# MIT-SPARK/Kimera-Semantics

Hardware: AMD Instinct MI355X
Metric: Mvoxel-updates/s + frames/s, 640×480 @5cm voxels, 1/2/4/8 MI355X (higher is better)
Workload: dtype f32; 1 GPU; bag-replay stand-in: 640x480 depth+label trajectory (room), 'fast' integrator, 5 cm voxels, 5 m rays, trunc 0.2 m, p=0.8; pipeline_frames=12, parallelism=frame-sharded x1, points_per_frame=305657, rays_per_frame=85307, updates_per_frame=502687

## Files before the change

### include/ks_hip.h

```cpp
#ifndef KS_HIP_H_
#define KS_HIP_H_

#include <stddef.h>
#include <stdint.h>

#ifdef __cplusplus
extern "C" {
#endif

#define KS_NUM_LABELS 21

enum {
  KS_OK = 0,
  KS_ERR_INVALID_ARG = -1,
  KS_ERR_LABEL_RANGE = -2,
  KS_ERR_PROBABILITY = -3,
  KS_ERR_HIP = -4,
  KS_ERR_POOL_FULL = -5,
  KS_ERR_INDEX_RANGE = -6,
  KS_ERR_NO_DEVICE = -7,
  KS_ERR_UNSUPPORTED = -8,
  KS_ERR_PEER_FAILED = -9
};

// ... 3 lines not shown
enum { KS_BUNDLE_ORDER_REFERENCE = 0, KS_BUNDLE_ORDER_CANONICAL = 1 };
enum { KS_EARLY_OUT_EXACT = 1 };

typedef struct ks_config {
  float voxel_size;
  int32_t voxels_per_side;
  float truncation_distance;
  float max_weight;
  float min_ray_length_m;
  float max_ray_length_m;
  int32_t voxel_carving_enabled;
  int32_t use_const_weight;
  int32_t allow_clear;
  int32_t use_weight_dropoff;
  int32_t use_sparsity_compensation_factor;
  float sparsity_compensation_factor;
  int32_t enable_anti_grazing;
  float start_voxel_subsampling_factor;
  int32_t max_consecutive_ray_collisions;
  int32_t clear_checks_every_n_frames;
  int32_t integration_order_mode;
  int32_t integrator_threads;
  int32_t method;
  int32_t bundle_order;
  float semantic_measurement_probability;
  int32_t color_mode;
  int32_t n_dynamic_labels;
  uint8_t dynamic_labels[32];
  uint8_t label_rgba[256][4];
  int32_t early_out_phase_growth;
  int32_t device_id;
  uint32_t max_tiles;
  uint32_t max_points;
  int32_t pipeline_frames;
} ks_config;

typedef struct ks_frame_stats {
  uint64_t n_points;
  uint64_t n_valid_points;
  uint64_t n_rays_cast;
  uint64_t n_voxel_updates;
  uint64_t n_blocks_allocated;
} ks_frame_stats;

enum {
  KS_STAGE_POINTS = 0,
  KS_STAGE_SORT_POINTS,
  KS_STAGE_RAYS,
  KS_STAGE_MARCH,
  KS_STAGE_EMIT,
  KS_STAGE_SORT_PAIRS,
  KS_STAGE_APPLY,
  KS_STAGE_APPLY_LONG,
  KS_STAGE_COUNT
};
typedef struct ks_profile {
  double ms[KS_STAGE_COUNT];
  uint64_t launches[KS_STAGE_COUNT];
  uint64_t frames;
  uint64_t updates;
  uint64_t points;
  double apply_kernel_ms;
  uint64_t apply_kernel_launches;
  uint64_t apply_kernel_updates;
  double host_ms;
  double host_wait_ms;
} ks_profile;

typedef struct ks_ctx ks_ctx;

int ks_default_config(ks_config* cfg);
int ks_create(const ks_config* cfg, ks_ctx** out);
void ks_destroy(ks_ctx* ctx);
const char* ks_last_error(ks_ctx* ctx);

int ks_set_color_to_label(ks_ctx* ctx, const uint8_t* rgba_keys, const uint8_t* labels, size_t n);

int ks_integrate_points(ks_ctx* ctx, const float T_G_C[7], const float* xyz, const uint8_t* rgba,
                        const uint8_t* labels, size_t n, int freespace, ks_frame_stats* stats);
int ks_integrate_points_device(ks_ctx* ctx, const float T_G_C[7], const float* d_xyz, const uint8_t* d_rgba,
                               const uint8_t* d_labels, size_t n, int freespace, ks_frame_stats* stats);

int ks_integrate_depth(ks_ctx* ctx, const float T_G_C[7], const void* depth, int depth_fmt, const uint8_t* label_img,
                       const uint8_t* rgba_img, int width, int height, const float K[4], int freespace,
                       ks_frame_stats* stats);
int ks_integrate_depth_device(ks_ctx* ctx, const float T_G_C[7], const void* d_depth, int depth_fmt,
                              const uint8_t* d_label_img, const uint8_t* d_rgba_img, int width, int height,
                              const float K[4], int freespace, ks_frame_stats* stats);

int ks_num_blocks(ks_ctx* ctx, size_t* n);
int ks_get_block_indices(ks_ctx* ctx, int32_t* out_xyz, size_t cap, size_t* n);
int ks_get_updated_block_indices(ks_ctx* ctx, int32_t* out_xyz, size_t cap, size_t* n, int reset);
int ks_download_blocks(ks_ctx* ctx, const int32_t* idx_xyz, size_t n, void* tsdf_out, void* sem_out);
int ks_upload_blocks(ks_ctx* ctx, const int32_t* idx_xyz, size_t n, const void* tsdf_in, const void* sem_in);
#define KS_VOXEL_RECORD_BYTES 120
typedef struct ks_voxel_run {
  int32_t block[3];
  uint32_t first;
  uint32_t count;
} ks_voxel_run;
int ks_count_updated_voxels(ks_ctx* ctx, size_t* n_records, size_t* n_runs );
int ks_download_updated_voxels(ks_ctx* ctx, void* out, size_t cap_records, size_t* n_records, ks_voxel_run* runs,
                               size_t cap_runs, size_t* n_runs);
void* ks_host_alloc(size_t bytes);
void ks_host_free(void* p);

typedef struct ks_mesh_config { float min_weight; int32_t only_stale; } ks_mesh_config;
typedef struct ks_mesh_stats {
  uint64_t blocks_meshed, blocks_total, triangles_total, triangles_changed, degenerate_dropped;
} ks_mesh_stats;
typedef struct ks_mesh_block { int32_t block[3]; uint32_t first_vertex, n_vertices; } ks_mesh_block;
int ks_mesh_default_config(ks_mesh_config* cfg);
int ks_mesh_update(ks_ctx* ctx, const ks_mesh_config* cfg, ks_mesh_stats* stats );
int ks_mesh_size(ks_ctx* ctx, size_t* n_blocks, size_t* n_vertices);
int ks_mesh_download(ks_ctx* ctx, ks_mesh_block* blocks, size_t cap_blocks, float* xyz, float* normals, uint8_t* rgba,
                     uint8_t* labels, size_t cap_vertices);
int ks_mesh_changed_blocks(ks_ctx* ctx, int32_t* out_xyz, size_t cap, size_t* n);

typedef struct ks_esdf_config {
  float min_weight, min_distance_m, max_distance_m;
  int32_t use_region;
  int32_t region_min[3], region_max[3];
  uint64_t max_workspace_bytes;
} ks_esdf_config;
typedef struct ks_esdf_stats { uint64_t voxels_observed, voxels_fixed, voxels_clamped, box_voxels[3], workspace_bytes; } ks_esdf_stats;
#define KS_ESDF_RECORD_BYTES 8
int ks_esdf_default_config(ks_esdf_config* cfg);
int ks_esdf_update(ks_ctx* ctx, const ks_esdf_config* cfg, ks_esdf_stats* stats );
int ks_esdf_download_blocks(ks_ctx* ctx, const int32_t* idx_xyz, size_t n, void* out );
int ks_esdf_query(ks_ctx* ctx, const float* xyz , size_t n, float* distance, uint8_t* flags,
                  uint8_t* label );

#define KS_TILE_BYTES 65536
int ks_get_tile_keys(ks_ctx* ctx, uint64_t* out, size_t cap, size_t* n);
int ks_export_tiles_device(ks_ctx* ctx, const uint32_t* slots, size_t n, void* d_payload);
int ks_merge_tiles_device(ks_ctx* ctx, const uint64_t* keys, size_t n, const void* d_payload);
int ks_clear(ks_ctx* ctx);
int ks_clear_voxels(ks_ctx* ctx);
int ks_reset_tiles(ks_ctx* ctx, const uint32_t* slots, size_t n);
int ks_tile_owner(uint64_t tile_key, int world);
typedef struct ks_reduce_stats {
  uint64_t tiles_sent, tiles_received, tiles_local, bytes_sent;
} ks_reduce_stats;
int ks_reduce(ks_ctx* ctx, void* rccl_comm, int rank, int world, ks_reduce_stats* stats);

typedef struct ks_round_stats {
  uint64_t updates_marched, updates_applied, bytes_sent, origin_voxel_touched, rays_cast;
} ks_round_stats;
int ks_integrate_round_exact(ks_ctx* marcher, ks_ctx* owner, void* rccl_comm, int rank, int world, uint64_t first_frame,
                             const float T_G_C[7], const float* xyz, const uint8_t* rgba, const uint8_t* labels, size_t n,
                             int freespace_points, ks_round_stats* stats);

int ks_debug_radix_sort(ks_ctx* ctx, void* keys, uint32_t* vals, size_t n, int key_bits, unsigned end_bit);

int ks_synchronize(ks_ctx* ctx);
void* ks_stream(ks_ctx* ctx);
int ks_flush(ks_ctx* ctx, ks_frame_stats* stats);
int ks_profile_enable(ks_ctx* ctx, int level);
int ks_early_out_iterations(ks_ctx* ctx, uint64_t* frames, uint64_t* iterations);
int ks_early_out_stats(ks_ctx* ctx, uint64_t out[5]);
int ks_profile_get(ks_ctx* ctx, ks_profile* out, int reset);
int ks_update_stats(ks_ctx* ctx, uint64_t out[4]);
int ks_pipeline_shape(ks_ctx* ctx, int32_t out[4]);
int ks_stream_plan(ks_ctx* ctx, int32_t out[8]);
int ks_seed_launch_shape(int32_t integration_order_mode, int32_t early_out_phase_growth, uint64_t cap_points, uint32_t* out, int32_t max_phases);

#ifdef __cplusplus
}
#endif
#endif
```

### kimera_semantics_amd/binding.py

```python
from __future__ import annotations

import ctypes as C
import os
import subprocess

import numpy as np

_HERE = os.path.dirname(os.path.abspath(__file__))
LIB_PATH = os.environ.get("KS_HIP_LIB") or os.path.join(_HERE, "libks_hip.so")
NUM_LABELS = 21

KS_METHOD_FAST, KS_METHOD_MERGED = 0, 1
KS_COLOR_MODE_COLOR, KS_COLOR_MODE_SEMANTIC, KS_COLOR_MODE_SEMANTIC_PROBABILITY = 0, 1, 2
KS_ORDER_MIXED, KS_ORDER_SORTED, KS_ORDER_MIXED_1024_GROUPS = 0, 1, 2
KS_BUNDLE_ORDER_REFERENCE, KS_BUNDLE_ORDER_CANONICAL = 0, 1
KS_EARLY_OUT_EXACT = 1
KS_ERR_LABEL_RANGE, KS_ERR_PROBABILITY, KS_ERR_POOL_FULL, KS_ERR_NO_DEVICE, KS_ERR_UNSUPPORTED = -2, -3, -5, -7, -8
KS_ERR_INVALID_ARG, KS_ERR_PEER_FAILED = -1, -9

STAGES = ["points", "sort_points", "rays", "march", "emit", "sort_pairs", "apply", "apply_long"]

TSDF_DTYPE = np.dtype([("distance", "<f4"), ("weight", "<f4"), ("color", "u1", (4,))])
SEM_DTYPE = np.dtype([("label", "u1"), ("pad", "u1", (3,)), ("priors", "<f4", (NUM_LABELS,)),
                      ("color", "u1", (4,))])

ABI_SYMBOLS = [
    "ks_default_config", "ks_create", "ks_destroy", "ks_last_error", "ks_set_color_to_label",
    "ks_integrate_points", "ks_integrate_points_device", "ks_integrate_depth", "ks_integrate_depth_device", "ks_num_blocks", "ks_get_block_indices",
    "ks_get_updated_block_indices", "ks_count_updated_voxels", "ks_download_updated_voxels", "ks_download_blocks", "ks_upload_blocks", "ks_host_alloc", "ks_host_free", "ks_get_tile_keys", "ks_export_tiles_device", "ks_merge_tiles_device", "ks_clear", "ks_clear_voxels", "ks_reset_tiles", "ks_tile_owner", "ks_reduce",
    "ks_debug_radix_sort", "ks_synchronize", "ks_flush", "ks_stream",
    "ks_profile_enable", "ks_profile_get", "ks_early_out_iterations", "ks_early_out_stats", "ks_pipeline_shape", "ks_stream_plan", "ks_seed_launch_shape", "ks_update_stats", "ks_integrate_round_exact",
    "ks_mesh_default_config", "ks_mesh_update", "ks_mesh_size", "ks_mesh_download", "ks_mesh_changed_blocks",
    "ks_esdf_default_config", "ks_esdf_update", "ks_esdf_download_blocks", "ks_esdf_query",
]


class KsConfig(C.Structure):
    _fields_ = [
        ("voxel_size", C.c_float), ("voxels_per_side", C.c_int32),
        ("truncation_distance", C.c_float), ("max_weight", C.c_float),
        ("min_ray_length_m", C.c_float), ("max_ray_length_m", C.c_float),
        ("voxel_carving_enabled", C.c_int32), ("use_const_weight", C.c_int32),
        ("allow_clear", C.c_int32), ("use_weight_dropoff", C.c_int32),
        ("use_sparsity_compensation_factor", C.c_int32), ("sparsity_compensation_factor", C.c_float),
        ("enable_anti_grazing", C.c_int32), ("start_voxel_subsampling_factor", C.c_float),
        ("max_consecutive_ray_collisions", C.c_int32), ("clear_checks_every_n_frames", C.c_int32),
        ("integration_order_mode", C.c_int32), ("integrator_threads", C.c_int32),
        ("method", C.c_int32), ("bundle_order", C.c_int32),
        ("semantic_measurement_probability", C.c_float), ("color_mode", C.c_int32),
        ("n_dynamic_labels", C.c_int32), ("dynamic_labels", C.c_uint8 * 32),
        ("label_rgba", (C.c_uint8 * 4) * 256),
        ("early_out_phase_growth", C.c_int32),
        ("device_id", C.c_int32), ("max_tiles", C.c_uint32), ("max_points", C.c_uint32), ("pipeline_frames", C.c_int32),
    ]


class KsRoundStats(C.Structure):
    _fields_ = [("updates_marched", C.c_uint64), ("updates_applied", C.c_uint64), ("bytes_sent", C.c_uint64),
                ("origin_voxel_touched", C.c_uint64), ("rays_cast", C.c_uint64)]


class KsFrameStats(C.Structure):
    _fields_ = [("n_points", C.c_uint64), ("n_valid_points", C.c_uint64), ("n_rays_cast", C.c_uint64),
                ("n_voxel_updates", C.c_uint64), ("n_blocks_allocated", C.c_uint64)]


class KsReduceStats(C.Structure):
    _fields_ = [("tiles_sent", C.c_uint64), ("tiles_received", C.c_uint64), ("tiles_local", C.c_uint64),
                ("bytes_sent", C.c_uint64)]


class KsMeshConfig(C.Structure):
    _fields_ = [("min_weight", C.c_float), ("only_stale", C.c_int32)]


class KsMeshStats(C.Structure):
    _fields_ = [("blocks_meshed", C.c_uint64), ("blocks_total", C.c_uint64), ("triangles_total", C.c_uint64),
                ("triangles_changed", C.c_uint64), ("degenerate_dropped", C.c_uint64)]


MESH_BLOCK_DTYPE = np.dtype([("block", "<i4", (3,)), ("first_vertex", "<u4"), ("n_vertices", "<u4")])


class KsEsdfConfig(C.Structure):
    _fields_ = [("min_weight", C.c_float), ("min_distance_m", C.c_float), ("max_distance_m", C.c_float), ("use_region", C.c_int32),
                ("region_min", C.c_int32 * 3), ("region_max", C.c_int32 * 3), ("max_workspace_bytes", C.c_uint64)]


class KsEsdfStats(C.Structure):
    _fields_ = [("voxels_observed", C.c_uint64), ("voxels_fixed", C.c_uint64), ("voxels_clamped", C.c_uint64),
                ("box_voxels", C.c_uint64 * 3), ("workspace_bytes", C.c_uint64)]


ESDF_DTYPE = np.dtype([("distance", "<f4"), ("flags", "u1"), ("label", "u1"), ("pad", "u1", (2,))])


class KsProfile(C.Structure):
    _fields_ = [("ms", C.c_double * 8), ("launches", C.c_uint64 * 8), ("frames", C.c_uint64),
                ("updates", C.c_uint64), ("points", C.c_uint64), ("apply_kernel_ms", C.c_double),
                ("apply_kernel_launches", C.c_uint64), ("apply_kernel_updates", C.c_uint64),
                ("host_ms", C.c_double), ("host_wait_ms", C.c_double)]


def build(force: bool = False) -> str:
    src_dir = os.path.join(_HERE, "csrc")
    srcs = [os.path.join(src_dir, f) for f in ("ks_hip.hip", "ks_types.h", "ks_k_rays.h", "ks_k_bundle_order.h", "ks_k_march.h", "ks_k_exact.h", "ks_k_apply.h",
                                                "ks_k_apply_xl.h", "ks_k_shard.h", "ks_k_shard_merged.h", "ks_k_io.h", "ks_k_mesh.h", "ks_k_esdf.h", "ks_mc_tri_table.inc", "ks_device_math.h", "ks_radix_sort.h", "ks_owned.h")]
    srcs.append(os.path.join(_HERE, "..", "include", "ks_hip.h"))
    stale = (not os.path.exists(LIB_PATH)) or any(
        os.path.exists(s) and os.path.getmtime(s) > os.path.getmtime(LIB_PATH) for s in srcs)
    if force or stale:
        subprocess.check_call(["make", "-C", src_dir])
    return LIB_PATH


_lib = None


def lib():
    global _lib
    if _lib is None:
        if not os.path.exists(LIB_PATH):
            raise RuntimeError(f"{LIB_PATH} is missing: run `python -c 'import __graft_entry__ as g; g.build()'` "
                               "(the HIP path has no CPU fallback)")
        L = C.CDLL(LIB_PATH)
        vp = C.c_void_p
        L.ks_default_config.argtypes = [C.POINTER(KsConfig)]
        L.ks_create.argtypes = [C.POINTER(KsConfig), C.POINTER(vp)]
        L.ks_destroy.argtypes = [vp]
        L.ks_destroy.restype = None
        L.ks_last_error.argtypes = [vp]
        L.ks_last_error.restype = C.c_char_p
        L.ks_set_color_to_label.argtypes = [vp, vp, vp, C.c_size_t]
        L.ks_integrate_points.argtypes = [vp, vp, vp, vp, vp, C.c_size_t, C.c_int, C.POINTER(KsFrameStats)]
        L.ks_integrate_points_device.argtypes = [vp, vp, vp, vp, vp, C.c_size_t, C.c_int, C.POINTER(KsFrameStats)]
        L.ks_integrate_depth.argtypes = [vp, vp, vp, C.c_int, vp, vp, C.c_int, C.c_int, vp, C.c_int, C.POINTER(KsFrameStats)]
        L.ks_integrate_depth_device.argtypes = [vp, vp, vp, C.c_int, vp, vp, C.c_int, C.c_int, vp, C.c_int, C.POINTER(KsFrameStats)]
        L.ks_num_blocks.argtypes = [vp, C.POINTER(C.c_size_t)]
        L.ks_get_block_indices.argtypes = [vp, vp, C.c_size_t, C.POINTER(C.c_size_t)]
        L.ks_get_updated_block_indices.argtypes = [vp, vp, C.c_size_t, C.POINTER(C.c_size_t), C.c_int]
        L.ks_download_blocks.argtypes = [vp, vp, C.c_size_t, vp, vp]
        L.ks_count_updated_voxels.argtypes = [vp, C.POINTER(C.c_size_t), C.POINTER(C.c_size_t)]
        L.ks_download_updated_voxels.argtypes = [vp, vp, C.c_size_t, C.POINTER(C.c_size_t), vp, C.c_size_t, C.POINTER(C.c_size_t)]
        L.ks_upload_blocks.argtypes = [vp, vp, C.c_size_t, vp, vp]
        L.ks_host_alloc.argtypes = [C.c_size_t]
        L.ks_host_alloc.restype = C.c_void_p
        L.ks_host_free.argtypes = [vp]
        L.ks_host_free.restype = None
        L.ks_get_tile_keys.argtypes = [vp, vp, C.c_size_t, C.POINTER(C.c_size_t)]
        L.ks_export_tiles_device.argtypes = [vp, vp, C.c_size_t, vp]
        L.ks_merge_tiles_device.argtypes = [vp, vp, C.c_size_t, vp]
        L.ks_clear.argtypes = [vp]
        L.ks_clear_voxels.argtypes = [vp]
        L.ks_reset_tiles.argtypes = [vp, vp, C.c_size_t]
        L.ks_tile_owner.argtypes = [C.c_uint64, C.c_int]
        L.ks_reduce.argtypes = [vp, vp, C.c_int, C.c_int, C.POINTER(KsReduceStats)]
        L.ks_debug_radix_sort.argtypes = [vp, vp, vp, C.c_size_t, C.c_int, C.c_uint]
        L.ks_synchronize.argtypes = [vp]
        L.ks_flush.argtypes = [vp, C.POINTER(KsFrameStats)]
        L.ks_stream.argtypes = [vp]
        L.ks_stream.restype = vp
        L.ks_profile_enable.argtypes = [vp, C.c_int]
        L.ks_profile_get.argtypes = [vp, C.POINTER(KsProfile), C.c_int]
        L.ks_early_out_iterations.argtypes = [vp, C.POINTER(C.c_uint64), C.POINTER(C.c_uint64)]
        L.ks_early_out_stats.argtypes = [vp, C.POINTER(C.c_uint64)]
        L.ks_pipeline_shape.argtypes = [vp, C.POINTER(C.c_int32)]
        L.ks_stream_plan.argtypes = [vp, C.POINTER(C.c_int32)]
        L.ks_seed_launch_shape.argtypes = [C.c_int32, C.c_int32, C.c_uint64, C.POINTER(C.c_uint32), C.c_int32]
        L.ks_update_stats.argtypes = [vp, C.POINTER(C.c_uint64)]
        L.ks_integrate_round_exact.argtypes = [vp, vp, vp, C.c_int, C.c_int, C.c_uint64, vp, vp, vp, vp, C.c_size_t, C.c_int, C.POINTER(KsRoundStats)]
        L.ks_mesh_default_config.argtypes = [C.POINTER(KsMeshConfig)]
        L.ks_mesh_update.argtypes = [vp, C.POINTER(KsMeshConfig), C.POINTER(KsMeshStats)]
        L.ks_mesh_size.argtypes = [vp, C.POINTER(C.c_size_t), C.POINTER(C.c_size_t)]
        L.ks_mesh_download.argtypes = [vp, vp, C.c_size_t, vp, vp, vp, vp, C.c_size_t]
        L.ks_mesh_changed_blocks.argtypes = [vp, vp, C.c_size_t, C.POINTER(C.c_size_t)]
        L.ks_esdf_default_config.argtypes = [C.POINTER(KsEsdfConfig)]
        L.ks_esdf_update.argtypes = [vp, C.POINTER(KsEsdfConfig), C.POINTER(KsEsdfStats)]
        L.ks_esdf_download_blocks.argtypes = [vp, vp, C.c_size_t, vp]
        L.ks_esdf_query.argtypes = [vp, vp, C.c_size_t, vp, vp, vp]
        _lib = L
    return _lib


def default_config(**overrides) -> KsConfig:
    cfg = KsConfig()
    lib().ks_default_config(C.byref(cfg))
    apply_overrides(cfg, **overrides)
    return cfg


def apply_overrides(cfg, **overrides):
    for k, v in overrides.items():
        if k == "dynamic_labels":
            cfg.n_dynamic_labels = len(v)
            for i, lab in enumerate(v):
                cfg.dynamic_labels[i] = int(lab)
        elif k == "label_rgba":
            arr = np.ascontiguousarray(np.asarray(v, dtype=np.uint8).reshape(256, 4))
            C.memmove(cfg.label_rgba, arr.ctypes.data, 1024)
        else:
            if not hasattr(cfg, k):
                raise AttributeError(k)
            setattr(cfg, k, v)
    return cfg


class KsError(RuntimeError):
    def __init__(self, code, msg):
        super().__init__(f"ks error {code}: {msg}")
        self.code = code


def _ptr(a):
    return None if a is None else a.ctypes.data


class HipIntegrator:

    def __init__(self, cfg: KsConfig):
        self.cfg = cfg
        self.vps = cfg.voxels_per_side
        self._h = C.c_void_p()
        rc = lib().ks_create(C.byref(cfg), C.byref(self._h))
        if rc != 0:
            raise KsError(rc, lib().ks_last_error(None).decode())

    def _chk(self, rc):
        if rc != 0:
            raise KsError(rc, lib().ks_last_error(self._h).decode())

    def close(self):
        if getattr(self, "_h", None):
            lib().ks_destroy(self._h)
            self._h = C.c_void_p()

    def __del__(self):
        try:
            self.close()
        except Exception:
            pass

    def set_color_to_label(self, rgba_keys, labels):
        k = np.ascontiguousarray(rgba_keys, dtype=np.uint8).reshape(-1, 4)
        l = np.ascontiguousarray(labels, dtype=np.uint8)
        self._chk(lib().ks_set_color_to_label(self._h, _ptr(k), _ptr(l), len(l)))

    def integrate(self, T_G_C, xyz, rgba, labels, freespace=False) -> KsFrameStats:
        T = np.ascontiguousarray(T_G_C, dtype=np.float32)
        xyz = np.ascontiguousarray(xyz, dtype=np.float32)
        labels = None if labels is None else np.ascontiguousarray(labels, dtype=np.uint8)
        rgba = None if rgba is None else np.ascontiguousarray(rgba, dtype=np.uint8)
        st = KsFrameStats()
        self._chk(lib().ks_integrate_points(self._h, _ptr(T), _ptr(xyz), _ptr(rgba), _ptr(labels), xyz.shape[0],
                                            int(freespace), C.byref(st)))
        return st

    def integrate_depth(self, T_G_C, depth, K, label_img=None, rgba_img=None, freespace=False) -> KsFrameStats:
        T = np.ascontiguousarray(T_G_C, dtype=np.float32)
        depth = np.ascontiguousarray(depth)
        fmt = 0 if depth.dtype == np.float32 else 1
        assert depth.dtype in (np.float32, np.uint16)
        Kc = np.ascontiguousarray(K, dtype=np.float32)
        lab = None if label_img is None else np.ascontiguousarray(label_img, dtype=np.uint8)
        col = None if rgba_img is None else np.ascontiguousarray(rgba_img, dtype=np.uint8)
        st = KsFrameStats()
        self._chk(lib().ks_integrate_depth(self._h, _ptr(T), _ptr(depth), fmt, _ptr(lab), _ptr(col), depth.shape[1],
                                           depth.shape[0], _ptr(Kc), int(freespace), C.byref(st)))
        return st

    def integrate_depth_device(self, T_G_C, d_depth: int, fmt: int, d_label_img: int, d_rgba_img: int, width: int,
                               height: int, K, freespace=False) -> KsFrameStats:
        T = np.ascontiguousarray(T_G_C, dtype=np.float32)
        Kc = np.ascontiguousarray(K, dtype=np.float32)
        st = KsFrameStats()
        self._chk(lib().ks_integrate_depth_device(self._h, _ptr(T), d_depth or None, fmt, d_label_img or None,
                                                  d_rgba_img or None, width, height, _ptr(Kc), int(freespace), C.byref(st)))
        return st

    def integrate_device(self, T_G_C, d_xyz: int, d_rgba: int, d_labels: int, n: int, freespace=False) -> KsFrameStats:
        T = np.ascontiguousarray(T_G_C, dtype=np.float32)
        st = KsFrameStats()
        self._chk(lib().ks_integrate_points_device(self._h, _ptr(T), d_xyz or None, d_rgba or None, d_labels or None, n,
                                                   int(freespace), C.byref(st)))
        return st

    def block_indices(self) -> np.ndarray:
        n = C.c_size_t()
        self._chk(lib().ks_get_block_indices(self._h, None, 0, C.byref(n)))
        out = np.zeros((n.value, 3), dtype=np.int32)
        if n.value:
            self._chk(lib().ks_get_block_indices(self._h, _ptr(out), n.value, C.byref(n)))
        return out

    def updated_block_indices(self, reset=True) -> np.ndarray:
        n = C.c_size_t()
        self._chk(lib().ks_get_updated_block_indices(self._h, None, 0, C.byref(n), 0))
        out = np.zeros((n.value, 3), dtype=np.int32)
        self._chk(lib().ks_get_updated_block_indices(self._h, _ptr(out), n.value, C.byref(n), int(reset)))
        return out

    def download(self, indices=None):
        if indices is None:
            indices = self.block_indices()
        indices = np.ascontiguousarray(indices, dtype=np.int32).reshape(-1, 3)
        nv = self.vps ** 3
        t = np.zeros((len(indices), nv), dtype=TSDF_DTYPE)
        s = np.zeros((len(indices), nv), dtype=SEM_DTYPE)
        if len(indices):
            self._chk(lib().ks_download_blocks(self._h, _ptr(indices), len(indices), _ptr(t), _ptr(s)))
        return indices, t, s

    def upload(self, indices, tsdf=None, sem=None):
        indices = np.ascontiguousarray(indices, dtype=np.int32).reshape(-1, 3)
        nv = self.vps ** 3
        tp = sp = None
        if tsdf is not None:
            tsdf = np.ascontiguousarray(tsdf, dtype=TSDF_DTYPE).reshape(len(indices), nv)
            tp = _ptr(tsdf)
        if sem is not None:
            sem = np.ascontiguousarray(sem, dtype=SEM_DTYPE).reshape(len(indices), nv)
            sp = _ptr(sem)
        self._chk(lib().ks_upload_blocks(self._h, _ptr(indices), len(indices), tp, sp))

    def mesh(self, only_stale=False, min_weight=1e-4):
        from .mesh import Mesh
        mc, st = KsMeshConfig(float(min_weight), int(bool(only_stale))), KsMeshStats()
        self._chk(lib().ks_mesh_update(self._h, C.byref(mc), C.byref(st)))
        nb, nv = C.c_size_t(), C.c_size_t()
        self._chk(lib().ks_mesh_size(self._h, C.byref(nb), C.byref(nv)))
        blocks = np.zeros(nb.value, dtype=MESH_BLOCK_DTYPE)
        xyz, normals = np.zeros((nv.value, 3), np.float32), np.zeros((nv.value, 3), np.float32)
        rgba, labels = np.zeros((nv.value, 4), np.uint8), np.zeros(nv.value, np.uint8)
        self._chk(lib().ks_mesh_download(self._h, _ptr(blocks), nb.value, _ptr(xyz), _ptr(normals), _ptr(rgba), _ptr(labels), nv.value))
        return Mesh(blocks, xyz, normals, rgba, labels, {k: int(getattr(st, k)) for k, _ in KsMeshStats._fields_})

    def mesh_changed_blocks(self) -> np.ndarray:
        n = C.c_size_t()
        self._chk(lib().ks_mesh_changed_blocks(self._h, None, 0, C.byref(n)))
        out = np.zeros((n.value, 3), dtype=np.int32)
        if n.value:
            self._chk(lib().ks_mesh_changed_blocks(self._h, _ptr(out), n.value, C.byref(n)))
        return out

    def esdf_update(self, region=None, **cfg) -> dict:
        ec, st = KsEsdfConfig(), KsEsdfStats()
        lib().ks_esdf_default_config(C.byref(ec))
        for k, v in cfg.items():
            if k not in ("min_weight", "min_distance_m", "max_distance_m", "max_workspace_bytes"):
                raise AttributeError(k)
            setattr(ec, k, v)
        if region is not None:
            ec.use_region = 1
            for a in range(3):
                ec.region_min[a], ec.region_max[a] = int(region[0][a]), int(region[1][a])
        rc = lib().ks_esdf_update(self._h, C.byref(ec), C.byref(st))
        stats = {k: ([int(v) for v in getattr(st, k)] if k == "box_voxels" else int(getattr(st, k))) for k, _ in KsEsdfStats._fields_}
        if rc != 0:
            err = KsError(rc, lib().ks_last_error(self._h).decode())
            err.stats = stats
            raise err
        return stats

    def esdf(self, region=None, **cfg):
        stats = self.esdf_update(region=region, **cfg)
        idx = self.block_indices()
        return idx, self.esdf_blocks(idx), stats

    def esdf_blocks(self, indices) -> np.ndarray:
        indices = np.ascontiguousarray(indices, dtype=np.int32).reshape(-1, 3)
        out = np.zeros((len(indices), self.vps ** 3), dtype=ESDF_DTYPE)
        self._chk(lib().ks_esdf_download_blocks(self._h, _ptr(indices), len(indices), _ptr(out)))
        return out

    def esdf_query(self, xyz) -> np.ndarray:
        xyz = np.ascontiguousarray(xyz, dtype=np.float32).reshape(-1, 3)
        n = len(xyz)
        d, f, l = np.zeros(n, np.float32), np.zeros(n, np.uint8), np.zeros(n, np.uint8)
        self._chk(lib().ks_esdf_query(self._h, _ptr(xyz), n, _ptr(d), _ptr(f), _ptr(l)))
        out = np.zeros(n, dtype=ESDF_DTYPE)
        out["distance"], out["flags"], out["label"] = d, f, l
        return out

    TILE_BYTES = 65536

    def tile_keys(self) -> np.ndarray:
        n = C.c_size_t()
        self._chk(lib().ks_get_tile_keys(self._h, None, 0, C.byref(n)))
        out = np.zeros(n.value, dtype=np.uint64)
        if n.value:
            self._chk(lib().ks_get_tile_keys(self._h, _ptr(out), n.value, C.byref(n)))
        return out

    def export_tiles(self, slots: np.ndarray, d_payload: int):
        s = np.ascontiguousarray(slots, dtype=np.uint32)
        self._chk(lib().ks_export_tiles_device(self._h, _ptr(s), len(s), d_payload or None))

    def merge_tiles(self, keys: np.ndarray, d_payload: int):
        k = np.ascontiguousarray(keys, dtype=np.uint64)
        self._chk(lib().ks_merge_tiles_device(self._h, _ptr(k), len(k), d_payload or None))

    def download_updated_voxels(self):
        n, nr = C.c_size_t(), C.c_size_t()
        self._chk(lib().ks_count_updated_voxels(self._h, C.byref(n), C.byref(nr)))
        dt = np.dtype([("block", "<i4", (3,)), ("linear", "<u4"), ("tsdf", TSDF_DTYPE), ("sem", SEM_DTYPE)])
        rdt = np.dtype([("block", "<i4", (3,)), ("first", "<u4"), ("count", "<u4")])
        assert dt.itemsize == 120 and rdt.itemsize == 20
        out = np.zeros(n.value, dtype=dt)
        runs = np.zeros(nr.value, dtype=rdt)
        if n.value:
            m, mr = C.c_size_t(), C.c_size_t()
            self._chk(lib().ks_download_updated_voxels(self._h, _ptr(out), n.value, C.byref(m), _ptr(runs), nr.value, C.byref(mr)))
            assert m.value == n.value and mr.value == nr.value
            assert int(runs["count"].sum()) == n.value
            for r in runs[:: max(1, len(runs) // 16)]:
                if r["count"]:
                    assert (out["block"][r["first"]:r["first"] + r["count"]] == r["block"]).all()
        return out

    def clear(self):
        self._chk(lib().ks_clear(self._h))

    def clear_voxels(self):
        self._chk(lib().ks_clear_voxels(self._h))

    def reset_tiles(self, slots: np.ndarray):
        s = np.ascontiguousarray(slots, dtype=np.uint32)
        self._chk(lib().ks_reset_tiles(self._h, _ptr(s), len(s)))

    def reduce(self, rccl_comm, rank: int, world: int) -> dict:
        st = KsReduceStats()
        self._chk(lib().ks_reduce(self._h, C.c_void_p(rccl_comm) if rccl_comm else None, rank, world, C.byref(st)))
        return {"tiles_sent": st.tiles_sent, "tiles_received": st.tiles_received, "tiles_local": st.tiles_local,
                "bytes_sent": st.bytes_sent}

    def debug_radix_sort(self, keys: np.ndarray, vals=None, end_bit=None):
        keys = np.ascontiguousarray(keys).copy()
        bits = keys.dtype.itemsize * 8
        vals = None if vals is None else np.ascontiguousarray(vals, dtype=np.uint32).copy()
        self._chk(lib().ks_debug_radix_sort(self._h, _ptr(keys), _ptr(vals), keys.shape[0], bits,
                                            bits if end_bit is None else end_bit))
        return keys, vals

    def synchronize(self):
        self._chk(lib().ks_synchronize(self._h))

    @property
    def stream(self) -> int:
        return lib().ks_stream(self._h) or 0

    def profile_enable(self, level=1):
        self._chk(lib().ks_profile_enable(self._h, int(level)))

    def early_out_stats(self):
        out = (C.c_uint64 * 5)()
        self._chk(lib().ks_early_out_stats(self._h, out))
        return dict(frames=int(out[0]), rounds=int(out[1]), fallbacks=int(out[2]), event_driven=bool(out[3]), pipelined=bool(out[4]))

    def integrate_round_exact(self, marcher: "HipIntegrator", rccl_comm, rank: int, world: int, first_frame: int, T_G_C, xyz, rgba, labels,
                              freespace=False) -> dict:
        T = np.ascontiguousarray(T_G_C, dtype=np.float32)
        n = 0 if xyz is None else len(xyz)
        x = None if xyz is None else np.ascontiguousarray(xyz, dtype=np.float32)
        c = None if rgba is None else np.ascontiguousarray(rgba, dtype=np.uint8)
        l = None if labels is None else np.ascontiguousarray(labels, dtype=np.uint8)
        st = KsRoundStats()
        self._chk(lib().ks_integrate_round_exact(marcher._h, self._h, rccl_comm, int(rank), int(world), int(first_frame), _ptr(T),
                                                 _ptr(x) if x is not None else None, _ptr(c) if c is not None else None,
                                                 _ptr(l) if l is not None else None, n, int(bool(freespace)), C.byref(st)))
        return dict(updates_marched=int(st.updates_marched), updates_applied=int(st.updates_applied), bytes_sent=int(st.bytes_sent),
                    origin_voxel_touched=bool(st.origin_voxel_touched), rays_cast=int(st.rays_cast))

    def update_stats(self):
        out = (C.c_uint64 * 4)()
        self._chk(lib().ks_update_stats(self._h, out))
        return dict(walked=int(out[0]), serial=int(out[1]), chunks=int(out[2]), replayed=int(out[3]))

    def pipeline_shape(self):
        out = (C.c_int32 * 4)()
        self._chk(lib().ks_pipeline_shape(self._h, out))
        return dict(lag=int(out[0]), slots=int(out[1]), batch=int(out[2]), march_streams=int(out[3]))

    def stream_plan(self):
        out = (C.c_int32 * 8)()
        self._chk(lib().ks_stream_plan(self._h, out))
        side = {1: "own", 0: "tail", -1: "none"}
        return dict(budget=int(out[0]), streams=int(out[1]), march_streams=int(out[2]), long=side[int(out[3])], xlong=side[int(out[4])],
                    march="own" if out[5] else "A", tail="own" if out[6] else "A", streams_held=int(out[7]))

    def early_out_iterations(self):
        f, it = C.c_uint64(), C.c_uint64()
        self._chk(lib().ks_early_out_iterations(self._h, C.byref(f), C.byref(it)))
        return f.value, it.value

    def flush(self) -> KsFrameStats:
        st = KsFrameStats()
        self._chk(lib().ks_flush(self._h, C.byref(st)))
        return st

    def profile(self, reset=False) -> dict:
        p = KsProfile()
        self._chk(lib().ks_profile_get(self._h, C.byref(p), int(reset)))
        return {"ms": {STAGES[i]: p.ms[i] for i in range(8)}, "launches": {STAGES[i]: p.launches[i] for i in range(8)},
                "frames": p.frames, "updates": p.updates, "points": p.points,
                "apply_kernel_ms": p.apply_kernel_ms, "apply_kernel_launches": p.apply_kernel_launches,
                "apply_kernel_updates": p.apply_kernel_updates, "host_ms": p.host_ms, "host_wait_ms": p.host_wait_ms}
```

### kimera_semantics_amd/csrc/ks_hip.hip

```cpp

#include <atomic>
#include <chrono>
#include <condition_variable>
#include <mutex>
#include <thread>
#include <cstring>
#include <string.h>

#include <dlfcn.h>
#include <hip/hip_runtime.h>
#include <hip/hip_ext.h>
#include <rccl/rccl.h>

#include <algorithm>
#include <iterator>
#include <cmath>
#include <cstdio>
#include <cstring>
#include <set>
#include <string>
#include <tuple>
#include <unordered_map>
#include <vector>

#include "../../include/ks_hip.h"
#include "ks_device_math.h"
#include "ks_owned.h"
#include "ks_radix_sort.h"

using namespace ksd;

#include "ks_types.h"
#include "ks_k_bundle_order.h"
#include "ks_k_rays.h"
#include "ks_k_march.h"
#include "ks_k_exact.h"
#include "ks_k_apply.h"
#include "ks_k_apply_xl.h"
#include "ks_k_shard.h"
#include "ks_k_shard_merged.h"
#include "ks_k_io.h"
#include "ks_k_mesh.h"
#include "ks_k_esdf.h"

using namespace ksk;

namespace {

std::string g_create_error;

const char* dbg_env(const char* name) {
  const char* g = getenv("KS_DEBUG");
  return (g && g[0] == '1') ? getenv(name) : nullptr;
}

}

constexpr int kMaxLag = 16;
constexpr int kSlots = kMaxLag + 8;
constexpr int kMarchStreams = 8;
constexpr int kObsTables = 16;
struct HostSnap {
  Counters c;
  uint32_t n_tiles;
  uint32_t pad[7];
};
struct FrameSlot {
  int index = 0;
  DevBuf<RayDesc> d_rays;
  DevBuf<float> d_deltas;
  DevBuf<uint64_t> d_pairs;
  DevBuf<uint32_t> d_cnt;
  DevBuf<uint32_t> d_lp;
  DevBuf<unsigned long long> d_bt;
  DevBuf<uint8_t> d_live;
  DevBuf<uint32_t> d_seed_gen, d_seed_items, d_seed_n;
  bool wide = false;
  DevBuf<FrameParams> d_F;
  DevBuf<uint64_t> d_gkeys, d_rkeys;
  struct GraphSet {
    hipGraphExec_t g1 = nullptr, g2 = nullptr, g3 = nullptr;
    uint64_t key = 0;
    GraphSet() = default;
    GraphSet(const GraphSet&) = delete;
    GraphSet& operator=(const GraphSet&) = delete;
    ~GraphSet() { reset(); }
    void reset() {
      for (hipGraphExec_t* g : {&g1, &g2, &g3}) {
        if (*g) (void)hipGraphExecDestroy(*g);
        *g = nullptr;
      }
      key = 0;
    }
  } b_graphs[2];
  DevBuf<uint64_t> d_eo_keys[2];
  DevBuf<uint32_t> d_eo_vals[2];
  size_t eo_cap_marks = 0;
  DevBuf<uint4> d_eo_tab;
  DevBuf<unsigned long long> d_eo_xnode;
  DevBuf<uint32_t> d_eo_cnt_b, d_eo_ux, d_eo_dirty, d_eo_list[2], d_eo_chg, d_eo_consulted, d_eo_lp;
  DevBuf<unsigned long long> d_eo_bt;
  DevBuf<EoCtl> d_eo_ctl;
  DevBuf<uint32_t> d_eo_sort_ws;
  DevBuf<uint32_t> d_eo_hseq, d_eo_where;
  DevBuf<uint4> d_eo_rinfo, d_eo_ckpt;
  DevBuf<uint8_t> d_eo_hitb;
  DevBuf<unsigned long long> d_eo_bits_a, d_eo_bits_b;
  DevBuf<unsigned long long> d_eo_btp;
  Event eo_committed;
  Counters* d_counters = nullptr;
  DevBuf<uint32_t> d_ray_list;
  PinnedBuf<HostSnap> h_snap;
  Event a_done;
  Event ready;
  Event tail_done;
  Event fork, join;
  Event join_x;
  Event found;
  bool tail_recorded = false;
  bool join_recorded = false;
  bool b_launched = false;
  size_t steps_max = 0;
  uint64_t frame_no = 0;
  FrameParams F{};
  size_t n = 0;
  int prof_set = -1;
  bool pending = false;
  const Counters& counters() const { return h_snap->c; }
  uint32_t n_tiles() const { return h_snap->n_tiles; }
};

constexpr int kProfSets = 32;
constexpr int kStageEvents = KS_STAGE_COUNT + 3;
struct ProfSet {
  Event ev[kStageEvents];
  Event k0, k1;
  bool used = false, complete = false, stages = false, apply = false, applied = false;
  uint64_t n_pairs = 0, n_points = 0;
};

struct StreamPlanIn {
  bool uses_early_out = false;
  bool exact_early_out = false;
  bool frames_independent = true;
  int pipeline_frames = 0;
  int batch = 1;
  bool xlong = true;
  int budget = 4;
};
struct StreamPlan {
  int budget = 4;
  int n_march = 1;
  bool march_own = false;
  bool tail_own = false;
  bool long_own = true;
  bool xlong_own = true;
  int distinct = 1;
};
inline StreamPlan stream_plan(const StreamPlanIn& in) {
  StreamPlan p;
  p.budget = in.budget;
  if (in.pipeline_frames) {
    p.n_march = (!in.frames_independent || in.batch > 1) ? 1 : std::min(kMarchStreams, std::max(4, in.pipeline_frames));
    if (in.exact_early_out && p.n_march > 4) p.n_march = 4;
    if (in.exact_early_out && in.batch > 1) p.n_march = 2;
    if (!in.uses_early_out) p.n_march = 1;
    p.march_own = in.uses_early_out;
    p.tail_own = true;
  }
  p.long_own = true;
  p.xlong_own = in.xlong;
  auto count = [&p] { return 1 + (p.march_own ? p.n_march : 0) + (p.tail_own ? 1 : 0) + (p.long_own ? 1 : 0) + (p.xlong_own ? 1 : 0); };
  if (p.budget < 8 && count() > p.budget) p.xlong_own = false;
  if (p.budget < 8 && count() > p.budget) p.long_own = false;
  p.distinct = count();
  return p;
}
inline int hw_queue_budget() {
  auto number = [](const char* s, int* out) {
    if (!s) return false;
    char* end = nullptr;
    const long v = strtol(s, &end, 10);
    if (end == s) return false;
    *out = (int)std::min<long>(32, std::max<long>(1, v));
    return true;
  };
  int b = 4;
  number(getenv("GPU_MAX_HW_QUEUES"), &b);
  number(dbg_env("KS_HW_QUEUES"), &b);
  return b;
}

struct ks_ctx {
  Stream streams[kMarchStreams + 4];
  int n_streams = 0;
  ks_config cfg{};
  std::string err;
  hipStream_t stream = nullptr;
  hipStream_t stream_march_[kMarchStreams] = {};
  int n_march = 1;
  int batch = 1;
  std::vector<FrameSlot*> batch_slots;
  hipStream_t prof_march_stream = nullptr;
  hipStream_t stream_tail = nullptr;
  hipStream_t stream_long = nullptr;
  hipStream_t stream_xlong = nullptr;
  StreamPlan plan;
  bool xlong = true;
  float voxel_size_inv = 0.f, log_match = 0.f, log_non_match = 0.f;
  int vps_shift = 1;

  TileTable table{};
  Pool pool{};
  DevBuf<TileEntry> table_ent;
  DevBuf<uint64_t> table_slot_keys;
  DevBuf<uint4> pool_vox;
  DevBuf<uint8_t> pool_updated, pool_dirty;
  DevBuf<uint64_t> d_start_set;
  DevBuf<uint64_t> d_observed_[kObsTables];
  int n_obs = 1;
  uint64_t start_offset = 0, observed_offset = 0;
  int64_t reset_counter = 0;
  uint32_t obs_tag = 0, obs_tag_lo = 1;
  DevBuf<Counters> d_retry_counters;
  std::atomic<size_t> pairs_hint{0};
  bool uses_early_out = false;
  std::vector<SeedPhase> seed_phases;
  DevBuf<SeedPhase> d_seed_phases;
  size_t seed_cap_items = 0;
  std::thread tail_thread;
  std::mutex tail_mu;
  std::mutex capture_mu;
  std::condition_variable tail_cv;
  FrameSlot* tail_job = nullptr;
  bool tail_busy = false, tail_quit = false;
  int tail_rc = KS_OK;
  bool use_tail_thread = false;
  bool use_graphs = true;
  bool test_overlap = true;
  std::atomic<uint64_t> buffers_epoch{1};
  DevBuf<uint8_t> d_color_lut;
  DevBuf<uint32_t> d_label_lut;
  uint32_t tiles_initialised = 0;

  size_t cap_points = 0;
  DevBuf<float> d_xyz;
  DevBuf<uint8_t> d_rgba;
  DevBuf<uint8_t> d_labels;
  DevBuf<uint32_t> d_hash;
  DevBuf<uint32_t> d_skeys32, d_skeys32b;
  DevBuf<float4> d_gpw;
  DevBuf<uint64_t> d_ray_keys;
  DevBuf<uint2> d_glc;
  DevBuf<unsigned long long> d_long_list_[2];
  DevBuf<uint32_t> d_blong;
  std::atomic<uint32_t> bo_hint{~0u};
  bool bo_hint_fixed = false;
  DevBuf<uint64_t> d_key_overflow;
  uint32_t key_overflow_mask = 0;
  uint32_t key_bits = 0;
  DevBuf<uint64_t> d_pkeys, d_pkeys2;
  DevBuf<uint32_t> d_pvals, d_pvals2;
  DevBuf<uint32_t> d_order;
  DevBuf<uint32_t> d_inv_order;
  DevBuf<uint32_t> d_okeys, d_okeys2, d_ovals;
  size_t cap_pairs = 0;
  DevBuf<uint64_t> d_pairs2_[2];
  hipEvent_t pending_join = nullptr;
  ksrs::Workspace sort_ws, sort_ws_tail;
  bool exact_early_out = false;
  DevBuf<uint64_t> d_eo_keys[2];
  DevBuf<uint32_t> d_eo_vals[2];
  size_t cap_marks = 0;
  DevBuf<uint2> d_eo_range;
  DevBuf<uint64_t> d_eo_plain;
  DevBuf<uint32_t> d_eo_lp;
  DevBuf<unsigned long long> d_eo_bt;
  DevBuf<EoState> d_eo_state;
  PinnedBuf<EoState> h_eo_state;
  uint64_t eo_iterations = 0, eo_frames = 0;
  bool eo_device = false;
  int eo_bulk_rounds = 6;
  static constexpr int eo_sweeps = 12;
  int eo_sweep_chunks = 16;
  std::atomic<int> eo_want_bulk{0};
  DevBuf<uint32_t> d_eo_committed;
  uint32_t eo_frame_no = 0;
  hipEvent_t eo_last_commit = nullptr;
  std::atomic<size_t> eo_want_marks{0}, eo_want_x{0};
  size_t eo_cap_marks = 0, eo_cap_x = 0;
  std::atomic<uint64_t> eo_fallbacks{0};
  uint64_t eo_fallbacks_seen = 0;
  std::atomic<int> eo_hopeless{0};
  bool eo_device_off = false;
  bool use_bundle_rank = false;
  BoCtx bo{};
  BoSchedule bo_sched{};
  DevBuf<uint8_t> d_bo_slab;
  int bo_epochs = 0;
  DevBuf<int32_t> d_rx_counts;
  DevBuf<uint64_t> d_tx_keys, d_rx_keys;
  DevBuf<uint32_t> d_tx_slots;
  DevBuf<uint8_t> d_tx_payload, d_rx_payload;
  size_t cap_tx = 0, cap_rx = 0;
  DevBuf<uint32_t> d_xchg_u32;
  DevBuf<uint64_t> d_xchg_u64;
  DevBuf<uint8_t> d_state;
  FrameSlot slot[kSlots];
  int n_slots = 1;
  uint64_t frame_no = 0;
  ks_frame_stats owed{};
  DevBuf<int32_t> d_block_idx;
  DevBuf<uint8_t> d_tsdf_out, d_sem_out;
  DevBuf<uint8_t> d_vox_out;
  size_t cap_out_blocks = 0;

  DevBuf<uint32_t> d_depth_blocks;
  DevBuf<uint8_t> d_img_depth;
  DevBuf<uint8_t> d_img_aux;

  int profiling = 0;
  unsigned long long apply_runs_min_pairs = 1ull << 20;
  bool xl_parallel = true;
  unsigned long long xl_min_pairs = 1ull << 23;
  DevBuf<XlRun> d_xl_runs;
  DevBuf<XlHeader> d_xl_hdr;
  DevBuf<XlChunk> d_xl_chunks;
  DevBuf<uint32_t> d_xl_idx;
  bool shard_export = false;
  int shard_world = 1;
  uint64_t shard_frames_seen = 0;
  DevBuf<uint64_t> d_sh_okey[2];
  DevBuf<uint64_t> d_sh_gkey[2];
  DevBuf<uint32_t> d_sh_seq[2];
  DevBuf<float> d_sh_sdf[2];
  DevBuf<float> d_sh_uw[2];
  DevBuf<uint32_t> d_sh_counts;
  size_t cap_sh = 0;
  uint32_t sh_counts[65] = {0};
  uint64_t sh_exported = 0;
  DevBuf<uint64_t> d_sh_tk;
  DevBuf<uint64_t> d_sh_pairs[2];
  DevBuf<uint32_t> d_sh_vals[2];
  size_t cap_sh_rx = 0;
  DevBuf<uint32_t> d_shm_bno;
  DevBuf<float2> d_shm_btab;
  DevBuf<uint32_t> d_shm_mpos;
  DevBuf<uint32_t> d_shm_cnt;
  size_t cap_shm_n = 0;
  DevBuf<float> d_shm_mixed;
  uint32_t shm_counts[2] = {0, 0};
  DevBuf<float2> d_shm_rx_btab;
  DevBuf<float> d_shm_rx_mixed;
  DevBuf<float4> d_shm_ops;
  DevBuf<uint32_t> d_shm_long;
  size_t cap_shm_ops = 0;
  bool long_lanes = true;
  unsigned long long long_lanes_min_pairs = 1ull << 24;
  DevBuf<unsigned long long> d_long_sorted_[2];
  DevBuf<LongHdr> d_long_hdr_[2];
  DevBuf<unsigned long long> d_xl_fb;
  uint32_t cap_xl_chunks = 1u << 17;
  MeshArena mesh_arena[2] = {};
  DevBuf<float> mesh_xyz[2], mesh_nrm[2];
  DevBuf<uint32_t> mesh_rgba[2];
  DevBuf<uint8_t> mesh_label[2];
  size_t mesh_cap[2] = {0, 0};
  int mesh_cur = 0;
  bool mesh_valid = false;
  float mesh_min_weight = 0.f;
  std::vector<uint64_t> mesh_blocks;
  uint32_t mesh_tiles_seen = 0;
  std::vector<ks_mesh_block> mesh_dir;
  std::vector<int32_t> mesh_changed;
  DevBuf<uint8_t> d_mesh_buf[10];
  DevBuf<EsdfRecord> esdf_store;
  DevBuf<uint64_t> esdf_keys[2];
  DevBuf<uint32_t> esdf_slots;
  DevBuf<unsigned long long> esdf_counters;
  DevBuf<EsdfRecord> esdf_out;
  DevBuf<int32_t> esdf_idx;
  DevBuf<float> esdf_xyz;
  bool esdf_valid = false;
  uint32_t esdf_tiles = 0;
  ks_profile prof{};
  ProfSet pset[kProfSets];
  bool fatal = false;
};

#define HIPCHK(ctx, expr)                                                                         \
  do {                                                                                            \
    hipError_t e_ = (expr);                                                                       \
    if (e_ != hipSuccess) {                                                                       \
      (ctx)->err = std::string(#expr) + ": " + hipGetErrorString(e_);                             \
      return KS_ERR_HIP;                                                                          \
    }                                                                                             \
  } while (0)

int ks_hip_failed(ks_ctx* ctx, const char* what, hipError_t e) {
  ctx->err = std::string(what) + ": " + hipGetErrorString(e);
  return KS_ERR_HIP;
}

namespace {

inline hipStream_t march_stream(ks_ctx* c, uint64_t frame_no) { return c->stream_march_[frame_no % (uint64_t)c->n_march]; }
inline uint64_t* observed_table(ks_ctx* c, uint64_t frame_no) { return c->d_observed_[frame_no % (uint64_t)c->n_obs]; }
int sync_march(ks_ctx* c) {
  for (int i = 0; i < c->n_march; ++i)
    if (c->stream_march_[i] != c->stream) HIPCHK(c, hipStreamSynchronize(c->stream_march_[i]));
  return KS_OK;
}

void probe_rehash_schedule(size_t n_max, BoSchedule* out) {
  static std::mutex mu;
  static std::vector<uint32_t> t, b;
  static size_t probed = 0;
  std::lock_guard<std::mutex> lk(mu);
  if (probed < n_max) {
    t.clear();
    b.clear();
    std::unordered_map<uint32_t, char> m;
    size_t bc = m.bucket_count();
    for (uint32_t i = 0; i < n_max; ++i) {
      m.emplace(i, 0);
      if (m.bucket_count() != bc) {
        bc = m.bucket_count();
        t.push_back(i);
        b.push_back((uint32_t)bc);
      }
    }
    probed = n_max;
  }
  *out = BoSchedule{};
  uint32_t off = 0;
  int e = 0;
  for (; e < (int)t.size() && e < kBoMaxEpochs && t[e] < n_max; ++e) {
    out->t[e] = t[e];
    out->b[e] = b[e];
    out->head_off[e] = off;
    off += b[e];
  }
  out->n_epochs = (uint32_t)e;
  out->t[e] = UINT32_MAX;
}

int ensure_bundle_order(ks_ctx* c, size_t cap) {
  probe_rehash_schedule(cap, &c->bo_sched);
  const BoSchedule& S = c->bo_sched;
  {
    static const uint32_t kLibstdcxxBuckets[] = {13, 29, 59, 127, 257, 541, 1109, 2357, 5087, 10273, 20753, 42043, 85229, 172933};
    for (uint32_t e = 0; e < S.n_epochs && e < sizeof(kLibstdcxxBuckets) / sizeof(uint32_t); ++e)
      if (S.b[e] != kLibstdcxxBuckets[e] || (e > 0 && S.t[e] != kLibstdcxxBuckets[e - 1])) {
        c->err = "bundle_order = KS_BUNDLE_ORDER_REFERENCE needs libstdc++'s unordered_map rehash schedule (13, 29, 59, ...): this build's standard "
                 "library differs; use KS_BUNDLE_ORDER_CANONICAL";
        return KS_ERR_UNSUPPORTED;
      }
  }
  c->bo_epochs = (int)S.n_epochs;
  size_t heads = 0;
  for (uint32_t e = 0; e < S.n_epochs; ++e) heads += S.b[e];
  const size_t nbt = cap / kBoBlock + 2, nfbt = 2 * cap / kBoBlock + 2;
  auto al = [](size_t words) { return (words * 4 + 255) & ~(size_t)255; };
  const size_t per_map = 11 * al(cap) + al(nbt) + al(heads);
  const size_t total = 2 * per_map + al(2) + al((sizeof(BoSchedule) + 3) / 4) + 2 * al(2 * cap) + al(nfbt) + al(cap);
  if (int rc = c->d_bo_slab.alloc(c, total)) return rc;
  uint8_t* p = c->d_bo_slab;
  auto take = [&](size_t words) { uint32_t* r = (uint32_t*)p; p += al(words); return r; };
  for (int m = 0; m < 2; ++m) {
    BoMap& M = c->bo.m[m];
    M.H = take(cap); M.rank = take(cap);
    M.next[0] = take(cap); M.next[1] = take(cap);
    M.idj[0] = take(cap); M.idj[1] = take(cap);
    M.kj[0] = take(cap); M.kj[1] = take(cap);
    M.lp = take(cap); M.gm = take(cap); M.cj = take(cap);
    M.bt = take(nbt);
    M.head = take(heads);
    HIPCHK(c, hipMemsetAsync(M.head, 0xff, heads * 4, c->stream));
  }
  c->bo.B = take(2);
  BoSchedule* d_sched = (BoSchedule*)take((sizeof(BoSchedule) + 3) / 4);
  c->bo.sched = d_sched;
  c->bo.flag = take(2 * cap);
  c->bo.flag_lp = take(2 * cap);
  c->bo.flag_bt = take(nfbt);
  c->bo.t_of_head = take(cap);
  HIPCHK(c, hipMemcpyAsync(d_sched, &c->bo_sched, sizeof(BoSchedule), hipMemcpyHostToDevice, c->stream));
  HIPCHK(c, hipStreamSynchronize(c->stream));
  return KS_OK;
}

inline uint32_t order_chains(int order_mode, size_t n) {
  const size_t q = n / kOrderStep;
  return (order_mode == KS_ORDER_MIXED && q >= 1) ? (uint32_t)q : kOrderStep;
}
inline uint32_t order_chains_cap(int order_mode, size_t cap) { return std::max(order_chains(order_mode, cap), order_mode == KS_ORDER_MIXED ? kOrderStep : 0u); }
inline uint32_t order_generations_cap(int order_mode, size_t cap) {
  if (order_mode == KS_ORDER_MIXED) return cap >= kOrderStep ? 2u * kOrderStep - 1u : 1u;
  return (uint32_t)((cap + kOrderStep - 1) / kOrderStep);
}
std::vector<uint32_t> phase_bounds(uint32_t n_gen, int growth) {
  std::vector<uint32_t> b{0};
  for (;;) {
    const uint64_t inc = std::max<uint64_t>(1, (uint64_t)b.back() * (uint64_t)(growth - 16) / 16);
    if (b.back() + inc >= n_gen) break;
    b.push_back((uint32_t)(b.back() + inc));
  }
  return b;
}
inline uint64_t seed_items_of(int order_mode, size_t n, uint32_t g0, uint32_t g1) {
  if (n == 0) return 0;
  const uint64_t chains = order_chains(order_mode, n), full = n / chains, part = n % chains;
  auto subs = [&](uint64_t gens) -> uint64_t {
    const uint64_t hi = std::min<uint64_t>(g1, gens);
    return hi > g0 ? (hi - g0 + kSubRun - 1) / kSubRun : 0;
  };
  return (chains - part) * subs(full) + part * subs(full + 1);
}
std::vector<SeedPhase> seed_launch_shape(int order_mode, int growth, size_t cap) {
  const uint32_t n_gen = order_generations_cap(order_mode, cap);
  const std::vector<uint32_t> B = phase_bounds(n_gen, growth);
  std::vector<SeedPhase> out;
  uint64_t off = 0;
  for (size_t j = 0; j < B.size(); ++j) {
    const uint32_t g0 = B[j], g1 = (j + 1 < B.size()) ? B[j + 1] : n_gen;
    uint64_t m = 0;
    if (order_mode == KS_ORDER_MIXED) {
      m = seed_items_of(order_mode, std::min<size_t>(cap, kOrderStep - 1), g0, g1);
      for (size_t q = 1; q <= cap / kOrderStep; ++q) m = std::max(m, seed_items_of(order_mode, std::min<size_t>(cap, q * kOrderStep + kOrderStep - 1), g0, g1));
    } else {
      m = seed_items_of(order_mode, cap, g0, g1);
    }
    out.push_back(SeedPhase{g0, g1, (uint32_t)off, (uint32_t)m});
    off += m;
  }
  return out;
}

size_t steps_max_of(const ks_config& cfg, float voxel_size_inv) {
  const double max_len = (double)cfg.max_ray_length_m + 2.0 * (double)cfg.truncation_distance;
  return (size_t)std::ceil(1.7321 * max_len * (double)voxel_size_inv) + 8;
}
int ensure_exact_points(ks_ctx* c, size_t cap);
int ensure_points(ks_ctx* c, size_t n) {
  if (n <= c->cap_points) return KS_OK;
  const size_t cap = std::max<size_t>(c->cap_points ? n + n / 8 : n, 1024);
  c->cap_points = 0;
  int rc;
  if ((rc = c->d_xyz.alloc(c, cap * 3))) return rc;
  if ((rc = c->d_rgba.alloc(c, cap * 4))) return rc;
  if ((rc = c->d_labels.alloc(c, cap))) return rc;
  ++c->buffers_epoch;
  const size_t scan_cap = (c->cfg.method == KS_METHOD_MERGED ? 2 : 1) * cap;
  size_t seed_items = 0;
  if (c->uses_early_out) {
    c->seed_phases = seed_launch_shape(c->cfg.integration_order_mode, c->cfg.early_out_phase_growth, cap);
    uint32_t off = 0;
    for (SeedPhase& P : c->seed_phases) {
      if ((P.g1 - P.g0 + kSubRun - 1) / kSubRun > (1u << kSeedSubBits) || order_chains_cap(c->cfg.integration_order_mode, cap) > (1u << kSeedChainBits)) {
        c->err = "point cloud too large for the early-out's work list";
        return KS_ERR_INVALID_ARG;
      }
      if (c->seed_cap_items) P.item_cap = (uint32_t)std::min<size_t>(P.item_cap, c->seed_cap_items);
      P.item_off = off;
      off += P.item_cap;
    }
    seed_items = off;
    if ((rc = c->d_seed_phases.alloc(c, c->seed_phases.size()))) return rc;
    HIPCHK(c, hipMemcpyAsync(c->d_seed_phases, c->seed_phases.data(), c->seed_phases.size() * sizeof(SeedPhase), hipMemcpyHostToDevice, c->stream));
    HIPCHK(c, hipStreamSynchronize(c->stream));
  }
  for (int i = 0; i < (c->cfg.pipeline_frames ? c->n_slots : 1); ++i) {
    if (c->uses_early_out) {
      if ((rc = c->slot[i].d_seed_gen.alloc(c, cap + order_chains_cap(c->cfg.integration_order_mode, cap)))) return rc;
      if ((rc = c->slot[i].d_seed_items.alloc(c, seed_items))) return rc;
      if ((rc = c->slot[i].d_seed_n.alloc(c, c->seed_phases.size()))) return rc;
    }
    if ((rc = c->slot[i].d_rays.alloc(c, cap))) return rc;
    if ((rc = c->slot[i].d_ray_list.alloc(c, cap))) return rc;
    if ((rc = c->slot[i].d_cnt.alloc(c, scan_cap))) return rc;
    if ((rc = c->slot[i].d_lp.alloc(c, scan_cap))) return rc;
    if ((rc = c->slot[i].d_bt.alloc(c, scan_cap / kScanBlock + 2))) return rc;
    if (c->cfg.method == KS_METHOD_FAST && (rc = c->slot[i].d_live.alloc(c, cap))) return rc;
    if (c->cfg.enable_anti_grazing && c->cfg.method == KS_METHOD_MERGED) {
      if ((rc = c->slot[i].d_gkeys.alloc(c, cap))) return rc;
      if ((rc = c->slot[i].d_rkeys.alloc(c, cap))) return rc;
    }
    if (c->cfg.method == KS_METHOD_MERGED && (rc = c->slot[i].d_deltas.alloc(c, cap * kNumLabels))) return rc;
  }
  if ((rc = c->d_hash.alloc(c, cap))) return rc;
  if ((rc = c->d_skeys32.alloc(c, cap))) return rc;
  if ((rc = c->d_skeys32b.alloc(c, cap))) return rc;
  if ((rc = c->d_pkeys.alloc(c, cap))) return rc;
  if ((rc = c->d_pkeys2.alloc(c, cap))) return rc;
  if ((rc = c->d_pvals.alloc(c, cap))) return rc;
  if ((rc = c->d_pvals2.alloc(c, cap))) return rc;
  if ((rc = c->d_order.alloc(c, cap))) return rc;
  if ((rc = c->d_inv_order.alloc(c, cap))) return rc;
  if ((rc = c->d_okeys.alloc(c, cap))) return rc;
  if ((rc = c->d_okeys2.alloc(c, cap))) return rc;
  if ((rc = c->d_ovals.alloc(c, cap))) return rc;
  if (c->cfg.method == KS_METHOD_MERGED) {
    if ((rc = c->d_gpw.alloc(c, cap))) return rc;
    if ((rc = c->d_glc.alloc(c, cap))) return rc;
    if ((rc = c->d_ray_keys.alloc(c, cap))) return rc;
    if ((rc = c->d_blong.alloc(c, cap / kLongRun + 64))) return rc;
    if (c->key_bits) {
      size_t slots = 1024;
      while (slots < 2 * cap) slots <<= 1;
      if ((rc = c->d_key_overflow.alloc(c, slots))) return rc;
      HIPCHK(c, hipMemsetAsync(c->d_key_overflow, 0, slots * sizeof(uint64_t), c->stream));
      c->key_overflow_mask = (uint32_t)(slots - 1);
    }
  }
  if (c->use_bundle_rank && (rc = ensure_bundle_order(c, cap))) return rc;
  if (c->exact_early_out) {
    if ((rc = c->d_eo_lp.alloc(c, cap))) return rc;
    if ((rc = c->d_eo_bt.alloc(c, cap / kScanBlock + 2))) return rc;
    if ((rc = ensure_exact_points(c, cap))) return rc;
  }
  c->cap_points = cap;
  return KS_OK;
}

int ensure_pairs_in(ks_ctx* c, FrameSlot& S, size_t bound) {
  if (bound <= S.d_pairs.size()) return KS_OK;
  if (int rc = S.d_pairs.alloc(c, std::max<size_t>(bound, 1 << 20))) return rc;
  ++c->buffers_epoch;
  return KS_OK;
}
int ensure_pairs_out(ks_ctx* c, size_t n) {
  if (n <= c->cap_pairs) return KS_OK;
  const size_t cap = std::max<size_t>(n + n / 4, 1 << 20);
  c->cap_pairs = 0;
  int rc;
  HIPCHK(c, hipStreamSynchronize(c->stream_long));
  if (c->stream_xlong) HIPCHK(c, hipStreamSynchronize(c->stream_xlong));
  if (c->stream_tail) HIPCHK(c, hipStreamSynchronize(c->stream_tail));
  for (int b = 0; b < 2; ++b) {
    if ((rc = c->d_pairs2_[b].alloc(c, cap))) return rc;
    if ((rc = c->d_long_list_[b].alloc(c, cap / kLongRunLanes + 64 + cap / kXLongRun + 64))) return rc;
    if (c->long_lanes && (rc = c->d_long_sorted_[b].alloc(c, cap / kLongRunLanes + 64))) return rc;
  }
  if (c->d_xl_hdr && (rc = c->d_xl_fb.alloc(c, cap / kXLongRun + 64))) return rc;
  c->cap_pairs = cap;
  return KS_OK;
}

template <typename K>
int sort_keys(ks_ctx* c, K* a, K* b, size_t n, unsigned end_bit, K** result, unsigned begin_bit = 0, bool tail = false) {
  HIPCHK(c, (ksrs::sort<K, false>(tail ? c->sort_ws_tail : c->sort_ws, a, b, nullptr, nullptr, n, end_bit,
                                  tail ? c->stream_tail : c->stream, result, nullptr, begin_bit)));
  return KS_OK;
}
template <typename K>
int sort_pairs(ks_ctx* c, K* ka, K* kb, uint32_t* va, uint32_t* vb, size_t n, unsigned end_bit, K** kres,
               uint32_t** vres) {
  HIPCHK(c, (ksrs::sort<K, true>(c->sort_ws, ka, kb, va, vb, n, end_bit, c->stream, kres, vres)));
  return KS_OK;
}

inline unsigned bits_for(uint64_t n) {
  unsigned b = 1;
  while (b < 64 && (1ull << b) < n) ++b;
  return b;
}

int launch_batch(ks_ctx* c);
int quiesce(ks_ctx* c);
int reset_set(ks_ctx* c, uint64_t* d_set0, uint64_t* offset, bool observed) {
  const bool full = ++(*offset) >= kFullResetThreshold;
  const bool retag = observed && !full && c->obs_tag + (uint32_t)c->cfg.clear_checks_every_n_frames + 2u >= kObsMaxTag;
  if (full || retag) {
    if (int rc = launch_batch(c)) return rc;
    if (full && c->exact_early_out) {
      if (int rc = quiesce(c)) return rc;
    }
    if (int rc = sync_march(c)) return rc;
    if (full) *offset = 0;
    for (int t = 0; t < (observed ? c->n_obs : 1); ++t) {
      uint64_t* d_set = observed ? c->d_observed_[t] : d_set0;
      if (full) {
        HIPCHK(c, hipMemsetAsync(d_set, 0, (observed ? 2 : 1) * (sizeof(uint64_t) << kSetBits), c->stream));
        const uint64_t poison = observed ? kObsPoison : ~0ull;
        HIPCHK(c, hipMemcpyAsync(d_set, &poison, sizeof(poison), hipMemcpyHostToDevice, c->stream));
      } else {
        hipLaunchKernelGGL(k_obs_retag, dim3((2u << kSetBits) / 256), dim3(256), 0, c->stream, d_set);
      }
    }
    if (observed && full && c->d_eo_plain) {
      HIPCHK(c, hipMemsetAsync(c->d_eo_plain, 0, sizeof(uint64_t) << kSetBits, c->stream));
      const uint64_t poison = ~0ull;
      HIPCHK(c, hipMemcpyAsync(c->d_eo_plain, &poison, sizeof(poison), hipMemcpyHostToDevice, c->stream));
    }
    HIPCHK(c, hipStreamSynchronize(c->stream));
    if (observed) c->obs_tag = 0;
  }
  if (observed) c->obs_tag_lo = c->obs_tag + 1;
  return KS_OK;
}

inline void stage_mark(ks_ctx* c, int set, int ev) {
  if (set >= 0 && c->pset[set].stages)
    (void)hipEventRecord(c->pset[set].ev[ev], ev <= 3 ? c->stream : ev <= 5 ? c->prof_march_stream : c->stream_tail);
}

void resolve_prof(ks_ctx* c, int set) {
  ProfSet& P = c->pset[set];
  if (!P.used || !P.complete) return;
  (void)hipEventSynchronize(P.ev[kStageEvents - 1]);
  if (P.stages) {
    for (int s = 0; s < KS_STAGE_COUNT; ++s) {
      float ms = 0.f;
      const int a = s < 3 ? s : s == 3 ? 4 : s + 2;
      if (hipEventElapsedTime(&ms, P.ev[a], P.ev[a + 1]) == hipSuccess) {
        c->prof.ms[s] += ms;
        c->prof.launches[s] += 1;
      }
    }
  }
  if (P.applied) {
    float kms = 0.f;
    if (hipEventElapsedTime(&kms, P.k0, P.k1) == hipSuccess) {
      c->prof.apply_kernel_ms += kms;
      c->prof.apply_kernel_launches += 1;
      c->prof.apply_kernel_updates += P.n_pairs;
    }
  }
  c->prof.frames += 1;
  c->prof.updates += P.n_pairs;
  c->prof.points += P.n_points;
  P.used = P.complete = P.applied = false;
}

SlotView slot_view(const FrameSlot& S, Counters* counters = nullptr) {
  SlotView v{};
  v.F = S.d_F;
  v.rays = S.d_rays;
  v.cnt = S.d_cnt;
  v.lp = S.d_lp;
  v.bt = S.d_bt;
  v.ray_list = S.d_ray_list;
  v.pairs = S.d_pairs;
  v.pairs_cap = (unsigned long long)S.d_pairs.size();
  v.C = counters ? counters : S.d_counters;
  v.host_snap = (uint32_t*)S.h_snap.get();
  v.eo_stats = S.d_eo_ctl ? &S.d_eo_ctl->n_x : nullptr;
  v.seed_gen = S.d_seed_gen;
  v.seed_items = S.d_seed_items;
  v.seed_n = S.d_seed_n;
  return v;
}

void launch_emit(ks_ctx* c, const BatchView& V, uint32_t nb, bool wide, hipStream_t st) {
  const size_t n = c->cap_points;
  const size_t lds = ((2 * n + kScanBlock - 1) / kScanBlock) * sizeof(unsigned long long);
  if (!(c->cfg.method == KS_METHOD_MERGED && c->cfg.enable_anti_grazing)) {
    if (wide || c->cfg.method == KS_METHOD_MERGED || !c->uses_early_out) {
      hipLaunchKernelGGL(k_emit_lane<8>, dim3((uint32_t)((n + 31) / 32), nb), dim3(256), lds, st, V, c->table, c->pool);
    } else {
      hipLaunchKernelGGL(k_emit_lane<16>, dim3((uint32_t)((n + 63) / 64), nb), dim3(256), lds, st, V, c->table, c->pool);
    }
  } else if (wide) {
    hipLaunchKernelGGL(k_emit<64>, dim3((uint32_t)((n + 3) / 4), nb), dim3(256), lds, st, V, c->table, c->pool);
  } else {
    hipLaunchKernelGGL(k_emit<16>, dim3((uint32_t)((n + 15) / 16), nb), dim3(256), lds, st, V, c->table, c->pool);
  }
}

void enqueue_stage_b(ks_ctx* c, const BatchView& V, uint32_t nb, bool wide, hipStream_t sm, size_t steps_max, int part = 0) {
  const ks_config& cfg = c->cfg;
  const size_t n = c->cap_points;
  if (c->uses_early_out && part != 2) {
    for (size_t j = 0; j < c->seed_phases.size(); ++j) {
      const SeedPhase& P = c->seed_phases[j];
      if (P.item_cap == 0) continue;
      const uint32_t steps_cap = (uint32_t)((steps_max + 3) & ~(size_t)3);
      const size_t lds_wave = (size_t)test_lds_words64(steps_cap) * sizeof(unsigned long long);
      const uint32_t wpb = lds_wave * 4 <= 60 * 1024 ? 4u : lds_wave * 2 <= 60 * 1024 ? 2u : 1u;
      const dim3 grid((P.item_cap + wpb - 1) / wpb, nb), block(64 * wpb);
      if (c->test_overlap) hipLaunchKernelGGL(k_test<true>, grid, block, lds_wave * wpb, sm, V, P.g0, P.g1, (uint32_t)j, P.item_off, P.item_cap, steps_cap);
      else hipLaunchKernelGGL(k_test<false>, grid, block, lds_wave * wpb, sm, V, P.g0, P.g1, (uint32_t)j, P.item_off, P.item_cap, steps_cap);
    }
  }
  if (part == 1) return;
  if (cfg.method == KS_METHOD_MERGED && cfg.enable_anti_grazing)
    hipLaunchKernelGGL(k_count_grazing<16>, dim3((uint32_t)((n + 15) / 16), nb), dim3(256), 0, sm, V);
  hipLaunchKernelGGL(k_scan_local, dim3((uint32_t)(((cfg.method == KS_METHOD_MERGED ? 2 : 1) * n + kScanBlock - 1) / kScanBlock), nb),
                     dim3(1024), 0, sm, V);
  launch_emit(c, V, nb, wide, sm);
  hipLaunchKernelGGL(k_publish, dim3(nb), dim3(64), 0, sm, V, (const uint32_t*)c->table.n_tiles);
}

int ensure_marks(ks_ctx* c, size_t n) {
  if (n <= c->cap_marks) return KS_OK;
  const size_t cap = std::max<size_t>(n + n / 4, 1 << 20);
  c->cap_marks = 0;
  int rc;
  for (int b = 0; b < 2; ++b) {
    if ((rc = c->d_eo_keys[b].alloc(c, cap))) return rc;
    if ((rc = c->d_eo_vals[b].alloc(c, cap))) return rc;
  }
  c->cap_marks = cap;
  return KS_OK;
}
constexpr int kEoMaxIterations = 4096;
int exact_early_out(ks_ctx* c, FrameSlot& S, hipStream_t st, Counters* counters = nullptr) {
  const size_t n = S.n;
  Counters* const d_counters = counters ? counters : S.d_counters;
  const FrameParams* dF = S.d_F;
  EoState* hs = c->h_eo_state;
  HIPCHK(c, hipMemsetAsync(c->d_eo_state, 0, sizeof(EoState), st));
  hipLaunchKernelGGL(k_eo_total, dim3((uint32_t)std::min<size_t>((n + 255) / 256, 1024)), dim3(256), 0, st, dF,
                     (const uint32_t*)S.d_cnt, c->d_eo_state);
  HIPCHK(c, hipMemcpyAsync(hs, c->d_eo_state, sizeof(EoState), hipMemcpyDeviceToHost, st));
  HIPCHK(c, hipStreamSynchronize(st));
  const uint32_t nb4k = (uint32_t)((n + kScanBlock - 1) / kScanBlock);
  const size_t lds = (size_t)nb4k * sizeof(unsigned long long);
  uint64_t* kres = nullptr;
  uint32_t* vres = nullptr;
  unsigned long long n_marks = hs->n_marks_next;
  bool converged = n_marks == 0;
  int it = 0;
  for (; !converged && it < kEoMaxIterations; ++it) {
    int rc;
    if ((rc = ensure_marks(c, n_marks))) return rc;
    HIPCHK(c, hipMemsetAsync(c->d_eo_range, 0, sizeof(uint2) << kSetBits, st));
    hipLaunchKernelGGL(k_eo_scan, dim3(nb4k), dim3(1024), 0, st, dF, (const uint32_t*)S.d_cnt, c->d_eo_lp, c->d_eo_bt, c->d_eo_state);
    if (S.wide)
      hipLaunchKernelGGL(k_eo_emit<8>, dim3((uint32_t)((n + 31) / 32)), dim3(256), lds, st, dF, S.d_ray_list, S.d_rays, S.d_cnt,
                         c->d_eo_lp, c->d_eo_bt, c->d_eo_keys[0], c->d_eo_vals[0], (unsigned long long)c->cap_marks, d_counters,
                         c->d_eo_state);
    else
      hipLaunchKernelGGL(k_eo_emit<64>, dim3((uint32_t)((n + 255) / 256)), dim3(256), lds, st, dF, S.d_ray_list, S.d_rays, S.d_cnt,
                         c->d_eo_lp, c->d_eo_bt, c->d_eo_keys[0], c->d_eo_vals[0], (unsigned long long)c->cap_marks, d_counters,
                         c->d_eo_state);
    HIPCHK(c, (ksrs::sort<uint64_t, true>(counters ? c->sort_ws_tail : c->sort_ws, c->d_eo_keys[0], c->d_eo_keys[1], c->d_eo_vals[0], c->d_eo_vals[1],
                                          (size_t)n_marks, 64, st, &kres, &vres, 44)));
    hipLaunchKernelGGL(k_eo_index, dim3((uint32_t)((n_marks + 255) / 256)), dim3(256), 0, st, n_marks, (const uint64_t*)kres,
                       c->d_eo_range);
    EoBuf E{kres, vres, c->d_eo_range, c->d_eo_plain};
    if (S.wide)
      hipLaunchKernelGGL(k_eo_eval<8>, dim3((uint32_t)((n + 31) / 32)), dim3(256), 0, st, dF, S.d_ray_list, S.d_rays, S.d_cnt, E,
                         d_counters, c->d_eo_state);
    else
      hipLaunchKernelGGL(k_eo_eval<16>, dim3((uint32_t)((n + 63) / 64)), dim3(256), 0, st, dF, S.d_ray_list, S.d_rays, S.d_cnt, E,
                         d_counters, c->d_eo_state);
    HIPCHK(c, hipMemcpyAsync(hs, c->d_eo_state, sizeof(EoState), hipMemcpyDeviceToHost, st));
    HIPCHK(c, hipStreamSynchronize(st));
    if (hs->n_marks != n_marks) {
      c->err = "exact early-out: mark count mismatch";
      return KS_ERR_HIP;
    }
    if (hs->changed == 0) converged = true;
    else n_marks = hs->n_marks_next;
  }
  if (!converged) {
    c->err = "exact early-out: no fixed point within the iteration limit";
    return KS_ERR_UNSUPPORTED;
  }
  c->eo_iterations += (uint64_t)it;
  if (!counters) c->eo_frames += 1;
  if (n_marks)
    hipLaunchKernelGGL(k_eo_commit, dim3((uint32_t)((n_marks + 255) / 256)), dim3(256), 0, st, n_marks, (const uint64_t*)kres,
                       (const uint32_t*)vres, c->d_eo_plain);
  return KS_OK;
}

int ensure_exact_slots(ks_ctx* c, size_t cap_marks, size_t cap_x) {
  if (!c->eo_device) return KS_OK;
  int rc;
  const int n_slots = c->cfg.pipeline_frames ? c->n_slots : 1;
  for (int i = 0; i < n_slots; ++i) {
    FrameSlot& S = c->slot[i];
    if (!S.d_eo_ctl) {
      if ((rc = S.d_eo_ctl.alloc(c, 1))) return rc;
      if ((rc = S.d_eo_tab.alloc(c, (size_t)1 << kSetBits))) return rc;
      HIPCHK(c, hipMemsetAsync(S.d_eo_tab, 0, sizeof(uint4) << kSetBits, c->stream));
      if ((rc = S.eo_committed.create(c, hipEventDisableTiming))) return rc;
    }
    if (S.eo_cap_marks < cap_marks) {
      S.eo_cap_marks = 0;
      for (int b = 0; b < 2; ++b) {
        if ((rc = S.d_eo_keys[b].alloc(c, cap_marks))) return rc;
        if ((rc = S.d_eo_vals[b].alloc(c, cap_marks))) return rc;
      }
      if ((rc = S.d_eo_sort_ws.alloc(c, ksrs::ws_words_dev(cap_marks, 3)))) return rc;
      if ((rc = S.d_eo_hitb.alloc(c, cap_marks))) return rc;
      if ((rc = S.d_eo_hseq.alloc(c, cap_marks))) return rc;
      if ((rc = S.d_eo_where.alloc(c, cap_marks))) return rc;
      if ((rc = S.d_eo_bits_a.alloc(c, cap_marks / 64 + 2))) return rc;
      if ((rc = S.d_eo_bits_b.alloc(c, cap_marks / 64 + 2))) return rc;
      S.eo_cap_marks = cap_marks;
    }
    if ((rc = S.d_eo_xnode.reserve(c, 2 * cap_x, 2 * cap_x))) return rc;
  }
  c->eo_cap_marks = cap_marks;
  c->eo_cap_x = cap_x;
  ++c->buffers_epoch;
  HIPCHK(c, hipStreamSynchronize(c->stream));
  return KS_OK;
}
int ensure_exact_points(ks_ctx* c, size_t cap) {
  if (!c->eo_device) return KS_OK;
  int rc;
  for (int i = 0; i < (c->cfg.pipeline_frames ? c->n_slots : 1); ++i) {
    FrameSlot& S = c->slot[i];
    for (DevBuf<uint32_t>* p : {&S.d_eo_cnt_b, &S.d_eo_ux, &S.d_eo_dirty, &S.d_eo_list[0], &S.d_eo_list[1], &S.d_eo_chg, &S.d_eo_consulted, &S.d_eo_lp})
      if ((rc = p->alloc(c, cap))) return rc;
    if ((rc = S.d_eo_bt.alloc(c, cap / kScanBlock + 2))) return rc;
    if ((rc = S.d_eo_btp.alloc(c, cap / kScanBlock + 2))) return rc;
    if ((rc = S.d_eo_rinfo.alloc(c, cap))) return rc;
    if ((rc = S.d_eo_ckpt.alloc(c, 3 * cap))) return rc;
  }
  return KS_OK;
}
EoView eo_view(ks_ctx* c, const FrameSlot& S) {
  EoView E{};
  E.F = S.d_F;
  E.ray_list = S.d_ray_list;
  E.rays = S.d_rays;
  E.C = S.d_counters;
  E.cnt_a = S.d_cnt;
  E.cnt_b = S.d_eo_cnt_b;
  E.ux = S.d_eo_ux;
  E.dirty = S.d_eo_dirty;
  E.keys = S.d_eo_keys[1];
  E.vals = S.d_eo_vals[1];
  E.bits_a = S.d_eo_bits_a;
  E.bits_b = S.d_eo_bits_b;
  E.lp = S.d_eo_lp;
  E.bt = S.d_eo_bt;
  E.btp = S.d_eo_btp;
  E.keys0 = S.d_eo_keys[0];
  E.vals0 = S.d_eo_vals[0];
  E.cap_marks = (unsigned long long)S.eo_cap_marks;
  E.hitb = S.d_eo_hitb;
  E.hseq_w = S.d_eo_hseq;
  E.wide = S.wide ? 1u : 0u;
  E.live = S.d_live;
  E.hseq = S.d_eo_hseq;
  E.where = S.d_eo_where;
  E.rinfo = S.d_eo_rinfo;
  E.ckpt = S.d_eo_ckpt;
  E.tab = S.d_eo_tab;
  E.xnode = S.d_eo_xnode;
  E.cap_x = (uint32_t)(S.d_eo_xnode.size() / 2);
  E.list[0] = S.d_eo_list[0];
  E.list[1] = S.d_eo_list[1];
  E.chg = S.d_eo_chg;
  E.consulted = S.d_eo_consulted;
  E.plain = c->d_eo_plain;
  E.committed = c->d_eo_committed;
  E.ctl = S.d_eo_ctl;
  return E;
}
void enqueue_sweeps(ks_ctx* c, const EoBatch& Bt, uint32_t nb, int count, hipStream_t st) {
  const size_t n = c->cap_points;
  const size_t waves = (size_t)order_chains_cap(c->cfg.integration_order_mode, n) *
                       ((order_generations_cap(c->cfg.integration_order_mode, n) + kEoSweepSegment - 1) / kEoSweepSegment);
  const uint32_t grid = (uint32_t)std::min<size_t>((waves + 3) / 4, 1 << 16);
  for (int i = 0; i < count; ++i) {
    hipLaunchKernelGGL(k_eo2_sweep, dim3(grid, nb), dim3(256), 0, st, Bt);
    hipLaunchKernelGGL(k_eo2_sweep_next, dim3(nb), dim3(64), 0, st, Bt);
  }
}
int enqueue_exact_rounds(ks_ctx* c, FrameSlot* const* slots, uint32_t nb, hipStream_t st) {
  const size_t n = c->cap_points;
  const uint32_t nb4k = (uint32_t)((n + kScanBlock - 1) / kScanBlock);
  const size_t lds = (size_t)nb4k * sizeof(unsigned long long);
  EoBatch Bt{};
  ksrs::DevBatch<uint64_t> Rs{};
  const FrameSlot& S0 = *slots[0];
  for (uint32_t k = 0; k < nb; ++k) {
    const FrameSlot& S = *slots[k];
    Bt.v[k] = eo_view(c, S);
    Rs.keys_a[k] = S.d_eo_keys[0];
    Rs.keys_b[k] = S.d_eo_keys[1];
    Rs.vals_a[k] = S.d_eo_vals[0];
    Rs.vals_b[k] = S.d_eo_vals[1];
    Rs.n_dev[k] = (const unsigned long long*)&S.d_eo_ctl->st.n_marks;
    Rs.ws[k] = S.d_eo_sort_ws;
  }
  hipLaunchKernelGGL(k_eo2_begin, dim3(nb), dim3(64), 0, st, Bt);
  const uint32_t gm = (uint32_t)std::min<size_t>((S0.eo_cap_marks + 255) / 256, 2048);
  const uint32_t gn = (uint32_t)std::min<size_t>((n + 255) / 256, 2048);
  if (S0.wide) {
    hipLaunchKernelGGL(k_eo2_full, dim3(gn, nb), dim3(256), 0, st, Bt);
    hipLaunchKernelGGL(k_eo2_scan, dim3(nb4k, nb), dim3(1024), 0, st, Bt);
    hipLaunchKernelGGL(k_eo2_emit<8>, dim3((uint32_t)((n + 31) / 32), nb), dim3(256), lds, st, Bt);
    HIPCHK(c, ksrs::sort_dev_batch<uint64_t>(Rs, (int)nb, S0.d_eo_sort_ws.size(), S0.eo_cap_marks, 44, 64, st));
    hipLaunchKernelGGL(k_eo2_bits, dim3(gm, nb), dim3(256), 0, st, Bt, 0u);
    hipLaunchKernelGGL(k_eo2_where, dim3(gm, nb), dim3(256), 0, st, Bt);
    enqueue_sweeps(c, Bt, nb, c->eo_sweeps, st);
    return KS_OK;
  } else {
    hipLaunchKernelGGL(k_eo2_scan, dim3(nb4k, nb), dim3(1024), 0, st, Bt);
    hipLaunchKernelGGL(k_eo2_emit<64>, dim3((uint32_t)((n + 255) / 256), nb), dim3(256), lds, st, Bt);
    HIPCHK(c, ksrs::sort_dev_batch<uint64_t>(Rs, (int)nb, S0.d_eo_sort_ws.size(), S0.eo_cap_marks, 44, 64, st));
    hipLaunchKernelGGL(k_eo2_hits, dim3(gm, nb), dim3(256), 0, st, Bt);
    hipLaunchKernelGGL(k_eo2_stop0, dim3(gn, nb), dim3(256), 0, st, Bt);
    hipLaunchKernelGGL(k_eo2_bits, dim3(gm, nb), dim3(256), 0, st, Bt, 1u);
  }
  const uint32_t gr = (uint32_t)std::min<size_t>((n + 3) / 4, 2048);
  for (int r = 1; r <= c->eo_bulk_rounds; ++r) {
    const uint32_t g = S0.wide ? gr : std::min(gr, r == 1 ? 2048u : r == 2 ? 1024u : r <= 4 ? 512u : 256u);
    hipLaunchKernelGGL(k_eo2_eval, dim3(g, nb), dim3(256), 0, st, Bt, (uint32_t)r);
    hipLaunchKernelGGL(k_eo2_propagate, dim3(g, nb), dim3(256), 0, st, Bt, (uint32_t)r);
  }
  return KS_OK;
}
void enqueue_exact_finish(ks_ctx* c, FrameSlot& S, hipStream_t st) {
  const EoView E = eo_view(c, S);
  hipLaunchKernelGGL(k_eo2_finish, dim3(1), dim3(kEoFinishThreads), 0, st, E, (uint32_t)c->eo_bulk_rounds + 1u, 1u);
  hipLaunchKernelGGL(k_eo2_commit, dim3(1024), dim3(256), 0, st, E);
}

template <typename Enqueue> hipGraphExec_t capture_graph(hipStream_t sm, Enqueue enqueue) {
  hipGraph_t g = nullptr;
  hipGraphExec_t out = nullptr;
  bool ok = hipStreamBeginCapture(sm, hipStreamCaptureModeRelaxed) == hipSuccess;
  if (ok) {
    const int rc = enqueue();
    ok = hipStreamEndCapture(sm, &g) == hipSuccess && g != nullptr && rc == KS_OK;
  }
  if (ok) ok = hipGraphInstantiate(&out, g, nullptr, nullptr, 0) == hipSuccess;
  if (g) (void)hipGraphDestroy(g);
  return ok ? out : nullptr;
}
struct BatchLaunch {
  ks_ctx* c;
  FrameSlot* const* slots;
  uint32_t nb;
  FrameSlot& S0;
  hipStream_t sm;
  const BatchView& V;
  size_t steps_max;
  uint64_t key;
  FrameSlot::GraphSet& G;
  int sweeps_host_driven() const {
    EoBatch Bt{};
    for (uint32_t k = 0; k < nb; ++k) Bt.v[k] = eo_view(c, *slots[k]);
    for (int chunk = 1;; ++chunk) {
      bool going = false;
      for (uint32_t k = 0; k < nb; ++k) {
        uint32_t w[2] = {0u, 0u};
        HIPCHK(c, hipMemcpyAsync(&w[0], &slots[k]->d_eo_ctl->sw_prev, sizeof(uint32_t), hipMemcpyDeviceToHost, sm));
        HIPCHK(c, hipMemcpyAsync(&w[1], &slots[k]->d_eo_ctl->fail, sizeof(uint32_t), hipMemcpyDeviceToHost, sm));
        HIPCHK(c, hipStreamSynchronize(sm));
        going = going || (w[0] != 0u && w[1] == 0u);
      }
      if (!going || chunk >= c->eo_sweep_chunks) break;
      enqueue_sweeps(c, Bt, nb, c->eo_sweeps, sm);
    }
    hipLaunchKernelGGL(k_eo2_sweep_done, dim3(nb), dim3(64), 0, sm, Bt);
    return KS_OK;
  }
  int exact_device() const {
    int rc;
    auto seed_and_rounds = [&] {
      enqueue_stage_b(c, V, nb, S0.wide, sm, steps_max, 1);
      return enqueue_exact_rounds(c, slots, nb, sm);
    };
    auto finish = [&] {
      for (uint32_t k = 0; k < nb; ++k) enqueue_exact_finish(c, *slots[k], sm);
      return KS_OK;
    };
    auto emission = [&] { return enqueue_stage_b(c, V, nb, S0.wide, sm, steps_max, 2), KS_OK; };
    bool graphs = c->use_graphs && !S0.wide;
    if (graphs && (G.key != key || !G.g1 || !G.g2 || !G.g3)) {
      std::lock_guard<std::mutex> cap(c->capture_mu);
      G.reset();
      if ((G.g1 = capture_graph(sm, seed_and_rounds)) && (G.g2 = capture_graph(sm, finish)) && (G.g3 = capture_graph(sm, emission))) {
        G.key = key;
      } else {
        (void)hipGetLastError();
        G.reset();
        c->use_graphs = graphs = false;
      }
    }
    if (graphs) HIPCHK(c, hipGraphLaunch(G.g1, sm));
    else if ((rc = seed_and_rounds()) || (S0.wide && (rc = sweeps_host_driven()))) return rc;
    if (c->eo_last_commit && c->eo_last_commit != S0.eo_committed) HIPCHK(c, hipStreamWaitEvent(sm, c->eo_last_commit, 0));
    if (graphs) HIPCHK(c, hipGraphLaunch(G.g2, sm));
    else finish();
    HIPCHK(c, hipEventRecord(S0.eo_committed, sm));
    c->eo_last_commit = S0.eo_committed;
    if (graphs) HIPCHK(c, hipGraphLaunch(G.g3, sm));
    else emission();
    return KS_OK;
  }
  int exact_host() const {
    enqueue_stage_b(c, V, nb, S0.wide, sm, steps_max, 1);
    if (int rc = exact_early_out(c, S0, sm)) return rc;
    enqueue_stage_b(c, V, nb, S0.wide, sm, steps_max, 2);
    return KS_OK;
  }
  int plain_or_replayed() const {
    if (c->use_graphs && (G.key != key || !G.g1)) {
      std::lock_guard<std::mutex> cap(c->capture_mu);
      G.reset();
      if ((G.g1 = capture_graph(sm, [&] { return enqueue_stage_b(c, V, nb, S0.wide, sm, steps_max), KS_OK; }))) {
        G.key = key;
      } else {
        (void)hipGetLastError();
        c->use_graphs = false;
      }
    }
    if (c->use_graphs && G.g1) HIPCHK(c, hipGraphLaunch(G.g1, sm));
    else enqueue_stage_b(c, V, nb, S0.wide, sm, steps_max);
    return KS_OK;
  }
};

int launch_batch(ks_ctx* c) {
  if (c->batch_slots.empty()) return KS_OK;
  std::vector<FrameSlot*> slots;
  slots.swap(c->batch_slots);
  const uint32_t nb = (uint32_t)slots.size();
  FrameSlot& S0 = *slots[0];
  hipStream_t sm = c->batch > 1 ? c->stream_march_[(S0.frame_no / (uint64_t)c->batch) % (uint64_t)c->n_march] : march_stream(c, S0.frame_no);
  c->prof_march_stream = sm;
  if (sm != c->stream) HIPCHK(c, hipStreamWaitEvent(sm, slots[nb - 1]->a_done, 0));
  const bool stage_events = nb == 1 && S0.prof_set >= 0 && c->pset[S0.prof_set].stages;
  if (stage_events) (void)hipEventRecord(c->pset[S0.prof_set].ev[4], sm);
  BatchView V{};
  size_t steps_max = 0;
  ParamsBatch PB{};
  for (uint32_t k = 0; k < nb; ++k) {
    FrameSlot& S = *slots[k];
    S.F.observed = observed_table(c, S.frame_no);
    if (c->exact_early_out) S.F.eo_frame = c->eo_frame_no++;
    PB.F[k] = S.F;
    PB.out[k] = S.d_F;
    V.s[k] = slot_view(S);
    steps_max = std::max(steps_max, S.steps_max);
  }
  if (nb == 1) hipLaunchKernelGGL(k_set_params, dim3(1), dim3(64), 0, sm, slots[0]->F, slots[0]->d_F);
  else hipLaunchKernelGGL(k_set_params_batch, dim3(nb), dim3(64), 0, sm, PB);
  const uint64_t key = ((uint64_t)c->cap_points << 24) ^ (c->buffers_epoch.load() << 4) ^ (S0.wide ? 1u : 0u) ^ ((uint64_t)nb << 1);
  const BatchLaunch B{c, slots.data(), nb, S0, sm, V, steps_max, key, S0.b_graphs[nb == (uint32_t)c->batch ? 0 : 1]};
  if (int rc = !c->exact_early_out ? B.plain_or_replayed() : c->eo_device && !c->eo_device_off ? B.exact_device() : B.exact_host()) return rc;
  for (uint32_t k = 0; k < nb; ++k) {
    HIPCHK(c, hipEventRecord(slots[k]->ready, sm));
    slots[k]->b_launched = true;
  }
  if (stage_events) (void)hipEventRecord(c->pset[S0.prof_set].ev[5], sm);
  return KS_OK;
}

void fill_frame_params(ks_ctx* c, FrameParams& F, const float Tq[7], size_t n, int freespace) {
  const ks_config& cfg = c->cfg;
  F = FrameParams{};
  F.T.w = Tq[0];
  F.T.v = {Tq[1], Tq[2], Tq[3]};
  F.T.t = {Tq[4], Tq[5], Tq[6]};
  F.voxel_size_inv = c->voxel_size_inv;
  F.min_ray = cfg.min_ray_length_m;
  F.max_ray = cfg.max_ray_length_m;
  F.trunc = cfg.truncation_distance;
  F.start_inv = cfg.start_voxel_subsampling_factor * c->voxel_size_inv;
  F.log_match = c->log_match;
  F.log_non_match = c->log_non_match;
  F.tsdf.voxel_size = cfg.voxel_size;
  F.tsdf.trunc = cfg.truncation_distance;
  F.tsdf.max_weight = cfg.max_weight;
  F.tsdf.dropoff_denominator = cfg.truncation_distance - cfg.voxel_size;
  F.tsdf.sparsity_factor = cfg.sparsity_compensation_factor;
  F.tsdf.use_dropoff = cfg.use_weight_dropoff;
  F.tsdf.use_sparsity = cfg.use_sparsity_compensation_factor;
  F.start_offset = c->start_offset;
  F.observed_offset = c->observed_offset;
  F.obs_tag = c->obs_tag;
  F.obs_tag_lo = c->obs_tag_lo;
  F.max_collisions = cfg.max_consecutive_ray_collisions;
  F.n = (uint32_t)n;
  const uint32_t q = (uint32_t)(n / kOrderStep);
  const bool by_1024 = cfg.integration_order_mode == KS_ORDER_MIXED_1024_GROUPS;
  F.order_groups = q == 0 ? 1u : by_1024 ? kOrderStep : q;
  F.order_per = q == 0 ? 0u : by_1024 ? q : kOrderStep;
  F.chains = order_chains(cfg.integration_order_mode, n);
  F.carving = cfg.voxel_carving_enabled;
  F.allow_clear = cfg.allow_clear;
  F.freespace = freespace;
  F.use_const_weight = cfg.use_const_weight;
  F.method = cfg.method;
  F.color_mode = cfg.color_mode;
  F.sorted_order = cfg.integration_order_mode == KS_ORDER_SORTED;
  F.n_dynamic = cfg.n_dynamic_labels;
  const unsigned pb = bits_for(n);
  F.point_mask = (1u << pb) - 1u;
  F.clear_bit = (cfg.method == KS_METHOD_MERGED) ? (1u << pb) : 0u;
  F.seq_bits = pb + (cfg.method == KS_METHOD_MERGED ? 1u : 0u);
  F.inv_order = F.sorted_order ? c->d_inv_order : nullptr;
  std::memcpy(F.dynamic_labels, cfg.dynamic_labels, 32);
  F.early_out = c->uses_early_out;
}
void begin_prof_set(ks_ctx* c, FrameSlot& S, size_t n) {
  const int set = (int)(c->frame_no % kProfSets);
  resolve_prof(c, set);
  ProfSet& P = c->pset[set];
  P.used = true;
  P.complete = P.applied = false;
  P.stages = c->profiling == 1;
  P.apply = c->profiling == 1 || (c->frame_no % 4) == 0;
  P.n_points = n;
  P.n_pairs = 0;
  S.prof_set = set;
}
int stage_a_fast(ks_ctx* c, FrameSlot& S, const float* d_xyz, const uint8_t* d_rgba, const uint8_t* d_labels, size_t n) {
  const FrameParams& F = S.F;
  hipStream_t st = c->stream;
  const uint32_t nb1k = (uint32_t)((n + 1023) / 1024);
  hipLaunchKernelGGL(k_points_fast, dim3(nb1k), dim3(1024), 0, st, F, d_xyz, d_rgba, d_labels, c->d_color_lut,
                     S.d_rays, c->d_hash, c->d_skeys32, c->d_pvals, S.d_cnt, S.d_live, S.d_counters);
  stage_mark(c, S.prof_set, 1);
  uint32_t *sk = nullptr, *sv = nullptr;
  if (int rc = sort_pairs(c, c->d_skeys32.get(), c->d_skeys32b.get(), c->d_pvals.get(), c->d_pvals2.get(), n, kSetBits + 1, &sk, &sv)) return rc;
  stage_mark(c, S.prof_set, 2);
  hipLaunchKernelGGL(k_dedup, dim3(nb1k), dim3(1024), 0, st, F, sk, sv, c->d_hash, c->d_start_set, S.d_ray_list, S.d_rays, S.d_cnt, S.d_live, S.d_counters);
  if (c->uses_early_out && n > 0) {
    const uint32_t n_gen = (uint32_t)((n + F.chains - 1) / F.chains);
    uint32_t n_ph = 0;
    while (n_ph < c->seed_phases.size() && c->seed_phases[n_ph].g0 < n_gen) ++n_ph;
    HIPCHK(c, hipMemsetAsync(S.d_seed_n, 0, c->seed_phases.size() * sizeof(uint32_t), st));
    hipLaunchKernelGGL(k_seed_list, dim3((F.chains + 63u) / 64u, n_ph), dim3(64 * kSeedSegs), 0, st, F, (const SeedPhase*)c->d_seed_phases,
                       (const uint8_t*)S.d_live, S.d_seed_gen, S.d_seed_items, S.d_seed_n, S.d_counters);
  }
  hipLaunchKernelGGL(k_dedup_commit, dim3(nb1k), dim3(1024), 0, st, F, sk, sv, c->d_hash, c->d_start_set, S.d_counters);
  return KS_OK;
}
void enqueue_bundle_order(ks_ctx* c, hipStream_t st, size_t n, const uint64_t* sk, const uint32_t* sv) {
  const uint32_t capb = (uint32_t)((c->cap_points + kBoBlock - 1) / kBoBlock);
  const size_t lds_f = (2 * c->cap_points / kBoBlock + 3) * sizeof(uint32_t), lds_e = ((size_t)capb + 2) * sizeof(uint32_t);
  hipLaunchKernelGGL(k_bo_scan_flags, dim3((uint32_t)((2 * n + kBoBlock - 1) / kBoBlock)), dim3(kBoBlock), 0, st, (uint32_t)n, c->bo);
  hipLaunchKernelGGL(k_bo_init, dim3((uint32_t)((n + kBoBlock - 1) / kBoBlock)), dim3(kBoBlock), lds_f, st, (uint32_t)n, sk, sv, c->bo);
  const uint32_t nbb = (uint32_t)((n + kBoBlock - 1) / kBoBlock);
  int e_small = 0;
  while (e_small < c->bo_epochs && c->bo_sched.b[e_small] <= kBoSmallBuckets) ++e_small;
  if (e_small > 0) hipLaunchKernelGGL(k_bo_small, dim3(2), dim3(kBoBlock), 0, st, c->bo, e_small);
  const size_t nh_floor = c->bo_hint_fixed ? (e_small > 0 ? (size_t)c->bo_sched.t[e_small - 1] + 1 : 1) : 2 * (size_t)kBoSmallBuckets;
  const size_t nh = std::min<size_t>(n, std::max<size_t>(c->bo_hint.load(std::memory_order_relaxed), nh_floor));
  int e_last = -1;
  for (int e = e_small; e <= c->bo_epochs; ++e) {
    if (e > 0 && c->bo_sched.t[e - 1] >= nh) break;
    hipLaunchKernelGGL(k_bo_link, dim3(nbb, 2), dim3(kBoBlock), lds_e, st, c->bo, e, (e == e_small && e_small > 0) ? 1 : 0);
    if (e < c->bo_epochs && c->bo_sched.t[e] < nh)
      hipLaunchKernelGGL(k_bo_walk, dim3(nbb, 2), dim3(kBoBlock), 0, st, c->bo, e);
    else
      e_last = e;
  }
  if (nh < n && e_last >= 0 && e_last < c->bo_epochs) hipLaunchKernelGGL(k_bo_rest, dim3(2), dim3(kBoBlock), lds_e, st, c->bo, e_last);
}
int stage_a_merged(ks_ctx* c, FrameSlot& S, const float* d_xyz, const uint8_t* d_rgba, const uint8_t* d_labels, size_t n, const uint32_t* order_ptr) {
  const ks_config& cfg = c->cfg;
  FrameParams& F = S.F;
  hipStream_t st = c->stream;
  const uint32_t nb = (uint32_t)((n + 255) / 256);
  const uint32_t nb1k = (uint32_t)((n + 1023) / 1024);
  if (c->key_bits) {
    const float reach = cfg.max_ray_length_m + 2.0f * cfg.voxel_size;
    const float tq[3] = {F.T.t.x, F.T.t.y, F.T.t.z};
    for (int a = 0; a < 3; ++a) {
      const float lo = std::floor((tq[a] - reach) * c->voxel_size_inv) - 2.0f;
      F.key_base[a] = (int32_t)std::min(std::max(lo, -2.0e9f), 2.0e9f);
    }
    F.key_bits = c->key_bits;
  }
  hipLaunchKernelGGL(k_points_merged, dim3(nb1k), dim3(1024), 0, st, F, d_xyz, d_rgba, d_labels, c->d_color_lut, c->d_pkeys, c->d_skeys32, c->d_pvals,
                     S.d_cnt, c->use_bundle_rank ? c->bo.flag : nullptr, c->d_key_overflow, c->key_overflow_mask, S.d_counters);
  stage_mark(c, S.prof_set, 1);
  uint64_t* sk = nullptr;
  uint32_t *sk32 = nullptr, *sv = nullptr;
  if (c->key_bits) {
    if (int rc = sort_pairs(c, c->d_skeys32.get(), c->d_skeys32b.get(), c->d_pvals.get(), c->d_pvals2.get(), n, 32, &sk32, &sv)) return rc;
    sk = c->d_pkeys;
  } else {
    if (int rc = sort_pairs(c, c->d_pkeys.get(), c->d_pkeys2.get(), c->d_pvals.get(), c->d_pvals2.get(), n, 64, &sk, &sv)) return rc;
  }
  stage_mark(c, S.prof_set, 2);
  hipLaunchKernelGGL(k_gather_sorted, dim3(nb), dim3(256), 0, st, F, d_xyz, d_rgba, d_labels, c->d_color_lut,
                     order_ptr, (const uint64_t*)sk, (const uint32_t*)sk32, sk, sv, c->d_gpw, c->d_glc, c->use_bundle_rank ? c->bo.flag : nullptr, c->d_blong,
                     c->d_key_overflow, S.d_counters);
  if (c->use_bundle_rank) enqueue_bundle_order(c, st, n, sk, sv);
  uint64_t* ray_keys = cfg.enable_anti_grazing ? S.d_rkeys : nullptr;
  if (cfg.enable_anti_grazing) HIPCHK(c, hipMemcpyAsync(S.d_gkeys, sk, n * sizeof(uint64_t), hipMemcpyDeviceToDevice, st));
  const uint32_t n_long_blocks = (uint32_t)std::min<size_t>(n / kLongRun + 1, 512);
  hipLaunchKernelGGL(k_bundles_all, dim3(n_long_blocks + (uint32_t)((n + 127) / 128)), dim3(128), 0, st, F, sk, sv, c->d_gpw, c->d_glc, c->d_blong,
                     S.d_rays, S.d_deltas, S.d_ray_list, ray_keys, S.d_cnt, c->bo, c->use_bundle_rank, S.d_counters, n_long_blocks);
  if (cfg.enable_anti_grazing) {
    F.grazing_keys = S.d_gkeys;
    F.ray_keys = S.d_rkeys;
  }
  return KS_OK;
}
int frame_front(ks_ctx* c, FrameSlot& S, const float Tq[7], const float* d_xyz, const uint8_t* d_rgba, const uint8_t* d_labels, size_t n, int freespace) {
  int rc;
  FrameParams& F = S.F;
  fill_frame_params(c, F, Tq, n, freespace);
  const size_t steps_max = steps_max_of(c->cfg, c->voxel_size_inv);
  S.wide = steps_max > 400;
  const size_t hint = c->pairs_hint.load(std::memory_order_relaxed);
  if ((rc = ensure_pairs_in(c, S, std::max<size_t>(hint + hint / 4, 1 << 20)))) return rc;
  hipStream_t st = c->stream;
  if (S.tail_recorded && c->stream_tail != c->stream) HIPCHK(c, hipStreamWaitEvent(st, S.tail_done, 0));
  if (S.join_recorded) HIPCHK(c, hipStreamWaitEvent(st, S.join, 0));
  S.n = n;
  S.prof_set = -1;
  if (c->profiling) begin_prof_set(c, S, n);
  S.frame_no = c->frame_no++;
  const uint32_t nb = (uint32_t)((n + 255) / 256);
  const uint32_t* order_ptr = nullptr;
  stage_mark(c, S.prof_set, 0);
  if (F.sorted_order) {
    hipLaunchKernelGGL(k_sqnorm, dim3(nb), dim3(256), 0, st, (uint32_t)n, d_xyz, c->d_okeys, c->d_ovals);
    uint32_t *ok = nullptr, *ov = nullptr;
    if ((rc = sort_pairs(c, c->d_okeys.get(), c->d_okeys2.get(), c->d_ovals.get(), c->d_order.get(), n, 32, &ok, &ov))) return rc;
    order_ptr = ov;
    hipLaunchKernelGGL(k_invert, dim3(nb), dim3(256), 0, st, (uint32_t)n, order_ptr, c->d_inv_order);
    F.order = order_ptr;
  }
  if ((rc = c->cfg.method == KS_METHOD_FAST ? stage_a_fast(c, S, d_xyz, d_rgba, d_labels, n) : stage_a_merged(c, S, d_xyz, d_rgba, d_labels, n, order_ptr)))
    return rc;
  stage_mark(c, S.prof_set, 3);
  if (c->stream_march_[0] != st) HIPCHK(c, hipEventRecord(S.a_done, st));
  S.steps_max = steps_max;
  S.b_launched = false;
  S.pending = true;
  c->batch_slots.push_back(&S);
  if ((int)c->batch_slots.size() >= c->batch || c->profiling == 1) return launch_batch(c);
  return KS_OK;
}

int shard_export_frame(ks_ctx* c, FrameSlot& S, unsigned long long n_pairs, hipStream_t st) {
  const int world = c->shard_world;
  int rc;
  if (n_pairs > c->cap_sh) {
    const size_t cap = std::max<size_t>(n_pairs + n_pairs / 4, 1 << 20);
    c->cap_sh = 0;
    for (int b = 0; b < 2; ++b) {
      if ((rc = c->d_sh_okey[b].alloc(c, cap))) return rc;
      if ((rc = c->d_sh_gkey[b].alloc(c, cap))) return rc;
      if ((rc = c->d_sh_seq[b].alloc(c, cap))) return rc;
      if ((rc = c->d_sh_sdf[b].alloc(c, cap))) return rc;
      if ((rc = c->d_sh_uw[b].alloc(c, cap))) return rc;
    }
    c->cap_sh = cap;
  }
  if (!c->d_sh_counts && (rc = c->d_sh_counts.alloc(c, 128))) return rc;
  const bool merged = c->cfg.method == KS_METHOD_MERGED;
  c->shm_counts[0] = c->shm_counts[1] = 0;
  if (merged && (S.n > c->cap_shm_n || !c->d_shm_cnt)) {
    const size_t cap = std::max<size_t>(S.n, 1 << 16);
    c->cap_shm_n = 0;
    if ((rc = c->d_shm_bno.alloc(c, cap))) return rc;
    if ((rc = c->d_shm_btab.alloc(c, cap))) return rc;
    if ((rc = c->d_shm_mpos.alloc(c, cap))) return rc;
    if ((rc = c->d_shm_cnt.alloc(c, 2))) return rc;
    c->cap_shm_n = cap;
  }
  HIPCHK(c, hipMemsetAsync(c->d_sh_counts, 0, 128 * sizeof(uint32_t), st));
  std::memset(c->sh_counts, 0, sizeof(c->sh_counts));
  c->sh_exported = n_pairs;
  if (n_pairs) {
    const uint32_t nb = (uint32_t)((n_pairs + 255) / 256);
    hipLaunchKernelGGL(k_shard_export, dim3(nb), dim3(256), 0, st, S.F, n_pairs, (const uint64_t*)S.d_pairs, (const RayDesc*)S.d_rays,
                       (const uint64_t*)c->table.slot_keys, (uint32_t)world, c->d_sh_okey[0], c->d_sh_gkey[0], c->d_sh_seq[0],
                       c->d_sh_sdf[0], c->d_sh_uw[0], c->d_sh_counts);
    uint64_t* sorted = nullptr;
    HIPCHK(c, (ksrs::sort<uint64_t, false>(c->sort_ws_tail, c->d_sh_okey[0], c->d_sh_okey[1], nullptr, nullptr, (size_t)n_pairs, 64, st,
                                           &sorted, nullptr, 56)));
    if (merged) {
      HIPCHK(c, hipMemsetAsync(c->d_shm_bno, 0, (size_t)S.n * sizeof(uint32_t), st));
      HIPCHK(c, hipMemsetAsync(c->d_shm_cnt, 0, 2 * sizeof(uint32_t), st));
      hipLaunchKernelGGL(k_shard_mark_bundles, dim3(nb), dim3(256), 0, st, n_pairs, (const uint32_t*)c->d_sh_seq[0], c->d_shm_bno);
      hipLaunchKernelGGL(k_shard_bundle_table, dim3((uint32_t)((S.n + 255) / 256)), dim3(256), 0, st, (uint32_t)S.n, (const RayDesc*)S.d_rays,
                         c->d_shm_bno, c->d_shm_btab, c->d_shm_mpos, c->d_shm_cnt);
      hipLaunchKernelGGL(k_shard_gather_merged, dim3(nb), dim3(256), 0, st, n_pairs, (const uint64_t*)sorted, (const uint64_t*)c->d_sh_gkey[0],
                         (const uint32_t*)c->d_sh_seq[0], (const float*)c->d_sh_sdf[0], (const float*)c->d_sh_uw[0], (const uint32_t*)c->d_shm_bno,
                         c->d_sh_gkey[1], c->d_sh_seq[1], c->d_sh_sdf[1], c->d_sh_uw[1]);
      HIPCHK(c, hipMemcpyAsync(c->shm_counts, c->d_shm_cnt, 2 * sizeof(uint32_t), hipMemcpyDeviceToHost, st));
    } else {
      hipLaunchKernelGGL(k_shard_gather, dim3(nb), dim3(256), 0, st, n_pairs, (const uint64_t*)sorted, (const uint64_t*)c->d_sh_gkey[0],
                         (const uint32_t*)c->d_sh_seq[0], (const float*)c->d_sh_sdf[0], (const float*)c->d_sh_uw[0], c->d_sh_gkey[1],
                         c->d_sh_seq[1], c->d_sh_sdf[1], c->d_sh_uw[1]);
    }
    HIPCHK(c, hipMemcpyAsync(c->sh_counts, c->d_sh_counts, 65 * sizeof(uint32_t), hipMemcpyDeviceToHost, st));
  }
  HIPCHK(c, hipStreamSynchronize(st));
  if (merged && c->shm_counts[1]) {
    const size_t nm = c->shm_counts[1];
    if ((rc = c->d_shm_mixed.reserve(c, nm * kNumLabels, std::max<size_t>(nm + nm / 2, 1024) * kNumLabels))) return rc;
    hipLaunchKernelGGL(k_shard_mixed_rows, dim3((uint32_t)((nm * kNumLabels + 255) / 256)), dim3(256), 0, st, (uint32_t)nm,
                       (const uint32_t*)c->d_shm_mpos, (const float*)S.d_deltas, c->d_shm_mixed);
    HIPCHK(c, hipStreamSynchronize(st));
  }
  return KS_OK;
}

inline void skip_update_stages(ks_ctx* c, int set) {
  for (int e = 7; e < kStageEvents - 1; ++e) stage_mark(c, set, e);
}
inline void finish_prof(ks_ctx* c, int set, hipStream_t st, uint64_t n_pairs) {
  if (set < 0) return;
  ProfSet& P = c->pset[set];
  P.n_pairs = n_pairs;
  (void)hipEventRecord(P.ev[kStageEvents - 1], st);
  P.complete = true;
}
inline void owe_stats(ks_ctx* c, const FrameSlot& S, const Counters& cnt, unsigned long long n_pairs, uint32_t n_blocks) {
  c->owed.n_points += S.n;
  c->owed.n_valid_points += cnt.n_valid;
  c->owed.n_rays_cast += cnt.n_rays;
  c->owed.n_voxel_updates += n_pairs;
  c->owed.n_blocks_allocated += n_blocks;
}
void eo_grow_after_fallback(ks_ctx* c, const EoCtl& hctl) {
  auto want_at_least = [](auto& w, auto v) {
    auto cur = w.load(std::memory_order_relaxed);
    while (cur < v && !w.compare_exchange_weak(cur, v, std::memory_order_relaxed)) {}
  };
  if (hctl.fail & kEoFailMarks) want_at_least(c->eo_want_marks, std::max<size_t>(2 * c->eo_cap_marks, (size_t)hctl.st.n_marks + (size_t)hctl.st.n_marks / 4));
  const bool x_dense = (hctl.fail & kEoFailX) && (size_t)hctl.n_x > (size_t)hctl.st.n_marks / 8;
  const bool more_bulk = (hctl.fail & kEoFailRounds) && !x_dense && c->eo_bulk_rounds < (int)kEoBulkMax;
  if (more_bulk) want_at_least(c->eo_want_bulk, std::min((int)kEoBulkMax, c->eo_bulk_rounds + std::max(4, c->eo_bulk_rounds / 2)));
  const bool dense = x_dense || ((hctl.fail & kEoFailRounds) && !more_bulk);
  if ((hctl.fail & kEoFailX) && !dense) want_at_least(c->eo_want_x, std::max<size_t>(16 * c->eo_cap_x, 8 * (size_t)hctl.n_x));
  if (dense) c->eo_hopeless.fetch_add(1, std::memory_order_relaxed);
  else if (!(hctl.fail & kEoFailChain)) c->eo_hopeless.store(0, std::memory_order_relaxed);
}
int repeat_emission(ks_ctx* c, FrameSlot& S, hipStream_t st, bool fix_point_first, Counters* cnt, uint32_t* new_tiles) {
  Counters rcnt{};
  rcnt.n_rays = cnt->n_rays;
  HIPCHK(c, hipMemcpyAsync(c->d_retry_counters, &rcnt, sizeof(rcnt), hipMemcpyHostToDevice, st));
  BatchView V{};
  V.s[0] = slot_view(S, c->d_retry_counters);
  if (fix_point_first) {
    if (int rc = exact_early_out(c, S, st, c->d_retry_counters)) return rc;
    HIPCHK(c, hipMemsetD32Async((hipDeviceptr_t)c->d_eo_committed, (int)(S.F.eo_frame + 1u), 1, st));
    hipLaunchKernelGGL(k_scan_local, dim3((uint32_t)((c->cap_points + kScanBlock - 1) / kScanBlock), 1), dim3(1024), 0, st, V);
  }
  launch_emit(c, V, 1, S.wide, st);
  HIPCHK(c, hipMemcpyAsync(&rcnt, c->d_retry_counters, sizeof(rcnt), hipMemcpyDeviceToHost, st));
  uint32_t nt = 0;
  HIPCHK(c, hipMemcpyAsync(&nt, c->table.n_tiles, sizeof(nt), hipMemcpyDeviceToHost, st));
  HIPCHK(c, hipStreamSynchronize(st));
  cnt->err = rcnt.err;
  cnt->n_pairs = rcnt.n_pairs;
  *new_tiles = std::min(nt, c->cfg.max_tiles);
  return KS_OK;
}
int repair_after_fallback(ks_ctx* c, FrameSlot& S, hipStream_t st, Counters* cnt, uint32_t* new_tiles) {
  HIPCHK(c, hipStreamSynchronize(st));
  EoCtl hctl;
  HIPCHK(c, hipMemcpy(&hctl, S.d_eo_ctl, sizeof(hctl), hipMemcpyDeviceToHost));
  eo_grow_after_fallback(c, hctl);
  c->eo_fallbacks.fetch_add(1, std::memory_order_relaxed);
  return repeat_emission(c, S, st, true, cnt, new_tiles);
}
int repair_after_overflow(ks_ctx* c, FrameSlot& S, hipStream_t st, Counters* cnt, uint32_t* new_tiles) {
  HIPCHK(c, hipStreamSynchronize(st));
  if (int rc = ensure_pairs_in(c, S, (size_t)cnt->n_pairs + (size_t)cnt->n_pairs / 4)) return rc;
  return repeat_emission(c, S, st, false, cnt, new_tiles);
}
int take_error_exits(ks_ctx* c, int set, hipStream_t st, uint32_t err) {
  skip_update_stages(c, set);
  finish_prof(c, set, st, 0);
  if (err & kErrLabel) {
    c->err = "semantic label >= 21 (CHECK_LT in the reference)";
    return KS_ERR_LABEL_RANGE;
  }
  c->fatal = true;
  c->err = (err & kErrPool) ? "voxel tile pool exhausted: raise ks_config.max_tiles" : "voxel index out of the packed range / tile table full";
  return (err & kErrPool) ? KS_ERR_POOL_FULL : KS_ERR_INDEX_RANGE;
}
#define KS_LAUNCH_TIMED_IF(timed, ev0, ev1, kernel, grid, block, stream, ...)                 \
  if (timed) hipExtLaunchKernelGGL(kernel, grid, block, 0, stream, ev0, ev1, 0, __VA_ARGS__); \
  else hipLaunchKernelGGL(kernel, grid, block, 0, stream, __VA_ARGS__)
// ... 1395 lines not shown
  if ((rc = c->esdf_out.reserve(c, m_max * nv, m_max * nv))) return rc;
  if ((rc = c->esdf_idx.reserve(c, m_max * 3, m_max * 3))) return rc;
  for (size_t off = 0; off < n; off += m_max) {
    const size_t m = std::min(m_max, n - off);
    HIPCHK(c, hipMemcpyAsync(c->esdf_idx, idx + 3 * off, m * 3 * sizeof(int32_t), hipMemcpyHostToDevice, c->stream));
    hipLaunchKernelGGL(k_esdf_download, dim3((uint32_t)((nv + 255) / 256), (uint32_t)m), dim3(256), 0, c->stream, c->table,
                       (const EsdfRecord*)c->esdf_store.get(), c->esdf_tiles, (const int32_t*)c->esdf_idx.get(), vps, c->esdf_out.get());
    HIPCHK(c, hipMemcpyAsync((uint8_t*)out + off * nv * sizeof(EsdfRecord), c->esdf_out, m * nv * sizeof(EsdfRecord), hipMemcpyDeviceToHost, c->stream));
    HIPCHK(c, hipStreamSynchronize(c->stream));
  }
  HIPCHK(c, hipGetLastError());
  return KS_OK;
}

int ks_esdf_query(ks_ctx* c, const float* xyz, size_t n, float* distance, uint8_t* flags, uint8_t* label) {
  if (!c || (n && !xyz)) return KS_ERR_INVALID_ARG;
  if (int rc = esdf_ready(c, "ks_esdf_query")) return rc;
  if (n == 0) return KS_OK;
  if (int rc = quiesce(c)) return rc;
  const size_t chunk = size_t(1) << 22;
  const size_t m_max = std::min(chunk, n);
  int rc;
  if ((rc = c->esdf_out.reserve(c, m_max, m_max))) return rc;
  if ((rc = c->esdf_xyz.reserve(c, m_max * 3, m_max * 3))) return rc;
  std::vector<EsdfRecord> rec(m_max);
  for (size_t off = 0; off < n; off += m_max) {
    const size_t m = std::min(m_max, n - off);
    HIPCHK(c, hipMemcpyAsync(c->esdf_xyz, xyz + 3 * off, m * 3 * sizeof(float), hipMemcpyHostToDevice, c->stream));
    hipLaunchKernelGGL(k_esdf_query, dim3((uint32_t)((m + 255) / 256)), dim3(256), 0, c->stream, c->table, (const EsdfRecord*)c->esdf_store.get(),
                       c->esdf_tiles, (const float*)c->esdf_xyz.get(), m, c->voxel_size_inv, c->esdf_out.get());
    HIPCHK(c, hipMemcpyAsync(rec.data(), c->esdf_out, m * sizeof(EsdfRecord), hipMemcpyDeviceToHost, c->stream));
    HIPCHK(c, hipStreamSynchronize(c->stream));
    for (size_t i = 0; i < m; ++i) {
      if (distance) distance[off + i] = rec[i].distance;
      if (flags) flags[off + i] = (uint8_t)(rec[i].tail & 0xffu);
      if (label) label[off + i] = (uint8_t)((rec[i].tail >> 8) & 0xffu);
    }
  }
  HIPCHK(c, hipGetLastError());
  return KS_OK;
}

static void* device_view_of_pinned(void* p) {
  hipPointerAttribute_t a;
  if (hipPointerGetAttributes(&a, p) != hipSuccess) {
    (void)hipGetLastError();
    return nullptr;
  }
  return a.type == hipMemoryTypeHost ? a.devicePointer : nullptr;
}

static int updated_voxels_impl(ks_ctx* c, void* out, size_t cap, size_t* n, bool count_only, ks_voxel_run* runs, size_t cap_runs,
                               size_t* n_runs) {
  if (!c || !n) return KS_ERR_INVALID_ARG;
  *n = 0;
  if (n_runs) *n_runs = 0;
  if (int rc = quiesce(c)) return rc;
  const uint32_t nt = c->tiles_initialised;
  if (nt == 0) return KS_OK;
  int rc;
  if ((rc = ensure_exchange(c, (size_t)nt + 8))) return rc;
  uint32_t* d_cnt = c->d_xchg_u32;
  uint32_t* d_list = c->d_xchg_u32 + 8;
  hipStream_t st = c->stream;
  HIPCHK(c, hipMemsetAsync(d_cnt, 0, 8 * sizeof(uint32_t), st));
  hipLaunchKernelGGL(k_list_updated_tiles, dim3((nt + 255) / 256), dim3(256), 0, st, c->pool, nt, d_list, d_cnt);
  uint32_t h_cnt[2] = {0, 0};
  HIPCHK(c, hipMemcpyAsync(h_cnt, d_cnt, sizeof(uint32_t), hipMemcpyDeviceToHost, st));
  HIPCHK(c, hipStreamSynchronize(st));
  const uint32_t n_list = h_cnt[0];
  if (n_list == 0) return KS_OK;
  if (n_runs) *n_runs = n_list;
  hipLaunchKernelGGL(k_export_dirty, dim3(n_list), dim3(512), 0, st, c->table, c->pool, (const uint32_t*)d_list,
                     (const uint32_t*)c->d_label_lut, c->vps_shift, 1, d_cnt, (uint8_t*)nullptr, (uint32_t*)nullptr);
  HIPCHK(c, hipMemcpyAsync(h_cnt, d_cnt, 2 * sizeof(uint32_t), hipMemcpyDeviceToHost, st));
  HIPCHK(c, hipStreamSynchronize(st));
  *n = h_cnt[1];
  if (count_only || h_cnt[1] == 0) return KS_OK;
  if ((size_t)h_cnt[1] > cap) {
    c->err = "ks_download_updated_voxels: output buffer too small (call ks_count_updated_voxels first)";
    return KS_ERR_INVALID_ARG;
  }
  if (runs && (size_t)n_list > cap_runs) {
    c->err = "ks_download_updated_voxels: run buffer too small";
    return KS_ERR_INVALID_ARG;
  }
  uint8_t* rec_direct = (uint8_t*)device_view_of_pinned(out);
  uint32_t* run_direct = runs ? (uint32_t*)device_view_of_pinned(runs) : nullptr;
  const size_t bytes = (size_t)h_cnt[1] * kVoxRecBytes;
  const size_t run_bytes = (size_t)n_list * sizeof(ks_voxel_run);
  const size_t need = (rec_direct ? 0 : bytes + bytes / 4) + (run_direct ? 0 : 2 * run_bytes) + 64;
  if ((!rec_direct || (runs && !run_direct)) && (rc = c->d_vox_out.reserve(c, need, need))) return rc;
  uint8_t* d_rec = rec_direct ? rec_direct : c->d_vox_out;
  uint32_t* d_runs = run_direct ? run_direct : (uint32_t*)(c->d_vox_out.get() + (rec_direct ? 0 : ((bytes + 15) & ~(size_t)15)));
  HIPCHK(c, hipMemsetAsync(d_cnt + 1, 0, sizeof(uint32_t), st));
  hipLaunchKernelGGL(k_export_dirty, dim3(n_list), dim3(512), 0, st, c->table, c->pool, (const uint32_t*)d_list,
                     (const uint32_t*)c->d_label_lut, c->vps_shift, 0, d_cnt, d_rec, runs ? d_runs : (uint32_t*)nullptr);
  if (!rec_direct) HIPCHK(c, hipMemcpyAsync(out, c->d_vox_out, bytes, hipMemcpyDeviceToHost, st));
  if (runs && !run_direct) HIPCHK(c, hipMemcpyAsync(runs, d_runs, run_bytes, hipMemcpyDeviceToHost, st));
  HIPCHK(c, hipStreamSynchronize(st));
  HIPCHK(c, hipGetLastError());
  return KS_OK;
}

int ks_count_updated_voxels(ks_ctx* c, size_t* n, size_t* n_runs) {
  return updated_voxels_impl(c, nullptr, 0, n, true, nullptr, 0, n_runs);
}
int ks_download_updated_voxels(ks_ctx* c, void* out, size_t cap, size_t* n, ks_voxel_run* runs, size_t cap_runs, size_t* n_runs) {
  if (!out && cap) return KS_ERR_INVALID_ARG;
  static_assert(sizeof(ks_voxel_run) == 20, "run record layout");
  return updated_voxels_impl(c, out, cap, n, false, runs, cap_runs, n_runs);
}

void* ks_host_alloc(size_t bytes) {
  void* p = nullptr;
  if (hipHostMalloc(&p, std::max<size_t>(bytes, 1), hipHostMallocDefault) != hipSuccess) return nullptr;
  return p;
}

void ks_host_free(void* p) {
  if (p) (void)hipHostFree(p);
}

int ks_debug_radix_sort(ks_ctx* c, void* keys, uint32_t* vals, size_t n, int key_bits, unsigned end_bit) {
  if (!c || (n && !keys) || (key_bits != 32 && key_bits != 64)) return KS_ERR_INVALID_ARG;
  if (n == 0) return KS_OK;
  const size_t kb = key_bits / 8;
  DevBuf<uint8_t> ka, kbuf;
  DevBuf<uint32_t> va, vb;
  int rc;
  if ((rc = ka.alloc(c, n * kb)) || (rc = kbuf.alloc(c, n * kb))) return rc;
  HIPCHK(c, hipMemcpy(ka, keys, n * kb, hipMemcpyHostToDevice));
  if (vals) {
    if ((rc = va.alloc(c, n)) || (rc = vb.alloc(c, n))) return rc;
    HIPCHK(c, hipMemcpy(va, vals, n * 4, hipMemcpyHostToDevice));
  }
  void* kres = nullptr;
  uint32_t* vres = nullptr;
  if (key_bits == 32) {
    uint32_t* r = nullptr;
    rc = vals ? sort_pairs(c, (uint32_t*)ka.get(), (uint32_t*)kbuf.get(), va.get(), vb.get(), n, end_bit, &r, &vres)
              : sort_keys(c, (uint32_t*)ka.get(), (uint32_t*)kbuf.get(), n, end_bit, &r);
    kres = r;
  } else {
    uint64_t* r = nullptr;
    rc = vals ? sort_pairs(c, (uint64_t*)ka.get(), (uint64_t*)kbuf.get(), va.get(), vb.get(), n, end_bit, &r, &vres)
              : sort_keys(c, (uint64_t*)ka.get(), (uint64_t*)kbuf.get(), n, end_bit, &r);
    kres = r;
  }
  if (rc) return rc;
  HIPCHK(c, hipStreamSynchronize(c->stream));
  HIPCHK(c, hipMemcpy(keys, kres, n * kb, hipMemcpyDeviceToHost));
  if (vals) HIPCHK(c, hipMemcpy(vals, vres, n * 4, hipMemcpyDeviceToHost));
  return KS_OK;
}

int ks_get_tile_keys(ks_ctx* c, uint64_t* out, size_t cap, size_t* n) {
  if (!c || !n) return KS_ERR_INVALID_ARG;
  if (int rc = quiesce(c)) return rc;
  HIPCHK(c, hipStreamSynchronize(c->stream));
  *n = c->tiles_initialised;
  const size_t m = std::min<size_t>(cap, *n);
  if (out && m) HIPCHK(c, hipMemcpy(out, c->table.slot_keys, m * sizeof(uint64_t), hipMemcpyDeviceToHost));
  return KS_OK;
}

int ks_export_tiles_device(ks_ctx* c, const uint32_t* slots, size_t n, void* d_payload) {
  if (!c || (n && (!slots || !d_payload))) return KS_ERR_INVALID_ARG;
  if (n == 0) return KS_OK;
  if (int rc = quiesce(c)) return rc;
  for (size_t i = 0; i < n; ++i)
    if (slots[i] >= c->tiles_initialised) return KS_ERR_INVALID_ARG;
  if (int rc = ensure_exchange(c, n)) return rc;
  HIPCHK(c, hipMemcpyAsync(c->d_xchg_u32, slots, n * sizeof(uint32_t), hipMemcpyHostToDevice, c->stream));
  hipLaunchKernelGGL(k_export_tiles, dim3((uint32_t)n), dim3(512), 0, c->stream, c->pool, c->d_xchg_u32, (uint4*)d_payload);
  HIPCHK(c, hipStreamSynchronize(c->stream));
  return KS_OK;
}

int ks_merge_tiles_device(ks_ctx* c, const uint64_t* keys, size_t n, const void* d_payload) {
  if (!c || (n && (!keys || !d_payload))) return KS_ERR_INVALID_ARG;
  if (n == 0) return KS_OK;
  if (c->fatal) return KS_ERR_INVALID_ARG;
  std::vector<uint32_t> order(n);
  for (size_t i = 0; i < n; ++i) order[i] = (uint32_t)i;
  std::stable_sort(order.begin(), order.end(), [&](uint32_t a, uint32_t b) { return keys[a] < keys[b]; });
  std::vector<uint64_t> ukeys;
  std::vector<uint32_t> offs;
  for (size_t i = 0; i < n; ++i) {
    if (i == 0 || keys[order[i]] != keys[order[i - 1]]) {
      ukeys.push_back(keys[order[i]]);
      offs.push_back((uint32_t)i);
    }
  }
  offs.push_back((uint32_t)n);
  const size_t nu = ukeys.size();
  int rc;
  if ((rc = quiesce(c))) return rc;
  if ((rc = ensure_exchange(c, n + 1))) return rc;
  uint32_t* d_offs = c->d_xchg_u32;
  uint32_t* d_idx = c->d_xchg_u32 + (nu + 1);
  HIPCHK(c, hipMemcpyAsync(c->d_xchg_u64, ukeys.data(), nu * sizeof(uint64_t), hipMemcpyHostToDevice, c->stream));
  HIPCHK(c, hipMemcpyAsync(d_offs, offs.data(), (nu + 1) * sizeof(uint32_t), hipMemcpyHostToDevice, c->stream));
  HIPCHK(c, hipMemcpyAsync(d_idx, order.data(), n * sizeof(uint32_t), hipMemcpyHostToDevice, c->stream));
  if ((rc = insert_tiles(c, c->d_xchg_u64, nu))) return rc;
  switch (c->cfg.color_mode) {
    case KS_COLOR_MODE_COLOR:
      hipLaunchKernelGGL(k_merge_tiles<KS_COLOR_MODE_COLOR>, dim3((uint32_t)nu), dim3(512), 0, c->stream, c->table, c->pool,
                         c->d_xchg_u64, d_offs, d_idx, (const uint4*)d_payload, c->cfg.max_weight, c->d_label_lut);
      break;
    case KS_COLOR_MODE_SEMANTIC:
      hipLaunchKernelGGL(k_merge_tiles<KS_COLOR_MODE_SEMANTIC>, dim3((uint32_t)nu), dim3(512), 0, c->stream, c->table,
                         c->pool, c->d_xchg_u64, d_offs, d_idx, (const uint4*)d_payload, c->cfg.max_weight, c->d_label_lut);
      break;
    default:
      hipLaunchKernelGGL(k_merge_tiles<KS_COLOR_MODE_SEMANTIC_PROBABILITY>, dim3((uint32_t)nu), dim3(512), 0, c->stream,
                         c->table, c->pool, c->d_xchg_u64, d_offs, d_idx, (const uint4*)d_payload, c->cfg.max_weight,
                         c->d_label_lut);
      break;
  }
  HIPCHK(c, hipStreamSynchronize(c->stream));
  HIPCHK(c, hipGetLastError());
  return KS_OK;
}

int ks_reset_tiles(ks_ctx* c, const uint32_t* slots, size_t n) {
  if (!c || (n && !slots)) return KS_ERR_INVALID_ARG;
  if (n == 0) return KS_OK;
  if (int rc = quiesce(c)) return rc;
  for (size_t i = 0; i < n; ++i)
    if (slots[i] >= c->tiles_initialised) return KS_ERR_INVALID_ARG;
  if (int rc = ensure_exchange(c, n)) return rc;
  HIPCHK(c, hipMemcpyAsync(c->d_xchg_u32, slots, n * sizeof(uint32_t), hipMemcpyHostToDevice, c->stream));
  hipLaunchKernelGGL(k_reset_tiles, dim3((uint32_t)n), dim3(512), 0, c->stream, c->pool, c->d_xchg_u32);
  HIPCHK(c, hipStreamSynchronize(c->stream));
  return KS_OK;
}

namespace {
struct RcclApi {
  void* h = nullptr;
  decltype(&ncclAllGather) all_gather = nullptr;
  decltype(&ncclSend) send = nullptr;
  decltype(&ncclRecv) recv = nullptr;
  decltype(&ncclGroupStart) group_start = nullptr;
  decltype(&ncclGroupEnd) group_end = nullptr;
  decltype(&ncclGetErrorString) err_string = nullptr;
  bool load(std::string* why) {
    if (h) return true;
    const char* env = getenv("KS_RCCL_LIB");
    const char* names[] = {env, "librccl.so.1", "librccl.so", "/opt/rocm/lib/librccl.so.1"};
    for (const char* nm : names) {
      if (!nm) continue;
      h = dlopen(nm, RTLD_NOW | RTLD_LOCAL);
      if (h) break;
    }
    if (!h) { *why = "librccl not found (set KS_RCCL_LIB)"; return false; }
    all_gather = (decltype(all_gather))dlsym(h, "ncclAllGather");
    send = (decltype(send))dlsym(h, "ncclSend");
    recv = (decltype(recv))dlsym(h, "ncclRecv");
    group_start = (decltype(group_start))dlsym(h, "ncclGroupStart");
    group_end = (decltype(group_end))dlsym(h, "ncclGroupEnd");
    err_string = (decltype(err_string))dlsym(h, "ncclGetErrorString");
    if (!all_gather || !send || !recv || !group_start || !group_end) { *why = "librccl lacks a required symbol"; h = nullptr; return false; }
    return true;
  }
};
RcclApi g_rccl;

inline uint64_t splitmix64(uint64_t x) {
  x += 0x9E3779B97F4A7C15ull;
  x = (x ^ (x >> 30)) * 0xBF58476D1CE4E5B9ull;
  x = (x ^ (x >> 27)) * 0x94D049BB133111EBull;
  return x ^ (x >> 31);
}
}

#define NCCLCHK(ctx, expr)                                                                                    \
  do {                                                                                                        \
    ncclResult_t r_ = (expr);                                                                                 \
    if (r_ != ncclSuccess) {                                                                                  \
      (ctx)->err = std::string(#expr) + ": " + (g_rccl.err_string ? g_rccl.err_string(r_) : "rccl error");    \
      return KS_ERR_HIP;                                                                                      \
    }                                                                                                         \
  } while (0)

int ks_tile_owner(uint64_t tile_key, int world) { return world > 0 ? (int)(splitmix64(tile_key) % (uint64_t)world) : 0; }

static int ensure_reduce_scratch(ks_ctx* c, size_t n_send, size_t n_recv, int world) {
  int rc;
  if ((rc = c->d_rx_counts.reserve(c, (size_t)(world + 3) * world, (size_t)(world + 3) * world))) return rc;
  if (n_send > c->cap_tx) {
    const size_t cap = std::max<size_t>(n_send + n_send / 2, 64);
    c->cap_tx = 0;
    if ((rc = c->d_tx_keys.alloc(c, cap))) return rc;
    if ((rc = c->d_tx_slots.alloc(c, cap))) return rc;
    if ((rc = c->d_tx_payload.alloc(c, cap * (size_t)KS_TILE_BYTES))) return rc;
    c->cap_tx = cap;
  }
  if (n_recv > c->cap_rx) {
    const size_t cap = std::max<size_t>(n_recv + n_recv / 2, 64);
    c->cap_rx = 0;
    if ((rc = c->d_rx_keys.alloc(c, cap))) return rc;
    if ((rc = c->d_rx_payload.alloc(c, cap * (size_t)KS_TILE_BYTES))) return rc;
    c->cap_rx = cap;
  }
// ... 553 lines not shown
```

### kimera_semantics_amd/csrc/ks_k_march.h

```cpp
#pragma once
#include "ks_types.h"

namespace ksk {

constexpr uint64_t kObsPoison = 0x00000000ffffffffull;
constexpr uint64_t kObsRetired = 0x00000000fffffffeull;
constexpr uint32_t kObsMaxTag = 1023;
constexpr uint32_t kObsMaxPoints = (1u << 22) - 2;

__device__ __forceinline__ uint64_t obs_entry(uint32_t tag, uint32_t pos, uint32_t hash) {
  return ((uint64_t)tag << 54) | ((uint64_t)(pos + 1u) << 32) | (uint64_t)hash;
}
__device__ __forceinline__ bool obs_match(uint64_t e, uint32_t h, uint32_t tag_lo, uint32_t tag) {
  const uint32_t posf = (uint32_t)(e >> 32) & 0x3fffffu, t = (uint32_t)(e >> 54);
  return posf != 0u && t >= tag_lo && t <= tag && (uint32_t)e == h;
}

__global__ void __launch_bounds__(256) k_obs_retag(uint64_t* __restrict__ set) {
  const uint32_t i = blockIdx.x * blockDim.x + threadIdx.x;
  if (i < (2u << kSetBits)) {
    const uint64_t e = set[i];
    if (e != 0ull) set[i] = kObsRetired;
  }
}
// ... 38 lines not shown
  return d.sx != 0 && d.sy != 0 && d.sz != 0 && isfinite(d.tx) && isfinite(d.ty) && isfinite(d.tz) && isfinite(d.dx) &&
         isfinite(d.dy) && isfinite(d.dz);
}
template <bool LE>
__device__ __forceinline__ int sorted_count(const float* e, float v) {
  int base = 0;
#pragma unroll
  for (int h = 32; h >= 1; h >>= 1) {
    const float x = e[base + h - 1];
    base += (LE ? (x <= v) : (x < v)) ? h : 0;
  }
  const float x = e[base];
  return base + ((LE ? (x <= v) : (x < v)) ? 1 : 0);
}
template <typename Visit>
__device__ __forceinline__ void dda_round64(Dda& st, float* E, uint32_t lane, Visit&& visit) {
  float tx0 = st.tx, ty0 = st.ty, tz0 = st.tz, dx0 = st.dx, dy0 = st.dy, dz0 = st.dz;
  KS_VALUE_BARRIER(tx0); KS_VALUE_BARRIER(ty0); KS_VALUE_BARRIER(tz0);
  KS_VALUE_BARRIER(dx0); KS_VALUE_BARRIER(dy0); KS_VALUE_BARRIER(dz0);
  if (lane < 3) {
    float t = lane == 0 ? tx0 : lane == 1 ? ty0 : tz0;
    const float d = lane == 0 ? dx0 : lane == 1 ? dy0 : dz0;
    float* e = E + lane * kES;
    for (int i = 0; i < 65; ++i) {
      e[i] = t;
      t = t + d;
    }
  }
  KS_WAVE_LDS_ORDER();
  const float *Ex = E, *Ey = E + kES, *Ez = E + 2 * kES;
  const float ex = Ex[lane], ey = Ey[lane], ez = Ez[lane];
  const int cyx = sorted_count<false>(Ey, ex), czx = sorted_count<false>(Ez, ex);
  const int cxy = sorted_count<true>(Ex, ey), czy = sorted_count<false>(Ez, ey);
  const int cxz = sorted_count<true>(Ex, ez), cyz = sorted_count<true>(Ey, ez);
  const int rx = (int)lane + cyx + czx, ry = (int)lane + cxy + czy, rz = (int)lane + cxz + cyz;
  if (rx < 64) visit((uint32_t)rx, st.cx + st.sx * (int)lane, st.cy + st.sy * cyx, st.cz + st.sz * czx);
  if (ry < 64) visit((uint32_t)ry, st.cx + st.sx * cxy, st.cy + st.sy * (int)lane, st.cz + st.sz * czy);
  if (rz < 64) visit((uint32_t)rz, st.cx + st.sx * cxz, st.cy + st.sy * cyz, st.cz + st.sz * (int)lane);
  const int nx = (int)__popcll(__ballot(rx < 64)), ny = (int)__popcll(__ballot(ry < 64)), nz = (int)__popcll(__ballot(rz < 64));
  const float ntx = Ex[nx], nty = Ey[ny], ntz = Ez[nz];
  st.cx += st.sx * nx;
  st.cy += st.sy * ny;
  st.cz += st.sz * nz;
  st.tx = ntx;
  st.ty = nty;
  st.tz = ntz;
}
__device__ __forceinline__ Dda dda_bcast(const Dda& d, int src) {
  Dda r;
  r.cx = __shfl(d.cx, src); r.cy = __shfl(d.cy, src); r.cz = __shfl(d.cz, src);
  r.sx = __shfl(d.sx, src); r.sy = __shfl(d.sy, src); r.sz = __shfl(d.sz, src);
  r.tx = __shfl(d.tx, src); r.ty = __shfl(d.ty, src); r.tz = __shfl(d.tz, src);
  r.dx = __shfl(d.dx, src); r.dy = __shfl(d.dy, src); r.dz = __shfl(d.dz, src);
  r.steps = __shfl(d.steps, src);
  r.in_range = true;
  return r;
}

constexpr int kBatchMax = 8;
struct SlotView {
  const FrameParams* F;
  const RayDesc* rays;
  uint32_t* cnt;
  uint32_t* lp;
  unsigned long long* bt;
  const uint32_t* ray_list;
  uint64_t* pairs;
  unsigned long long pairs_cap;
  Counters* C;
  uint32_t* host_snap;
  const uint32_t* eo_stats;
  const uint32_t* seed_gen;
  const uint32_t* seed_items;
  const uint32_t* seed_n;
};
struct BatchView {
  SlotView s[kBatchMax];
};

constexpr uint32_t kOrderStep = 1024;
constexpr uint32_t kPrivSlots = 1024;
constexpr uint32_t kCntBroke = 1u << 31;

typedef unsigned long long obs_u64x2 __attribute__((ext_vector_type(2)));
typedef __attribute__((address_space(1))) unsigned long long obs_global_u64;
typedef __attribute__((address_space(1))) obs_u64x2 obs_global_u64x2;
__device__ __forceinline__ void obs_atomic_max(obs_global_u64* p, unsigned long long v) {
  (void)__hip_atomic_fetch_max(p, v, __ATOMIC_RELAXED, __HIP_MEMORY_SCOPE_AGENT);
}
__device__ __forceinline__ ulonglong2 obs_load2(const obs_global_u64* observed, uint32_t slot) {
  const obs_u64x2 e = ((const obs_global_u64x2*)observed)[slot];
  return make_ulonglong2(e.x, e.y);
}
constexpr int kTestThreads = 256;
constexpr uint32_t kSubRun = 16;
#ifdef KS_STATS
__device__ unsigned long long g_test_stats[16];
#define KS_STAT_ADD(i, v) do { if (lane_id() == 0) atomicAdd(&g_test_stats[i], (unsigned long long)(v)); } while (0)
#define KS_STAT_MAX(i, v) do { if (lane_id() == 0) atomicMax(&g_test_stats[i], (unsigned long long)(v)); } while (0)
#else
#define KS_STAT_ADD(i, v)
#define KS_STAT_MAX(i, v)
#endif

__device__ __forceinline__ int early_out_stop(uint64_t hits, uint64_t valids, int lim, int& c) {
  const int nv = valids == ~0ull ? 64 : (int)__ffsll((long long)~valids) - 1;
  if (lim >= 0 && lim <= 6 && c <= lim && nv + c <= 64) {
    const uint64_t hh = (c ? ((hits << c) | ((1ull << c) - 1ull)) : hits);
    uint64_t run = hh;
    for (int k = 1; k <= lim; ++k) run &= hh >> k;
    if (run != 0ull) {
      const int stop = (int)__ffsll((long long)run) - 1 + lim - c;
      if (stop < nv) return stop;
    }
    if (nv == 0) return -1;
    const uint64_t top = nv + c == 64 ? hh : (hh | (~0ull << (nv + c)));
    const uint64_t inv = ~top;
    const int last_zero = inv == 0ull ? -1 : 63 - (int)__clzll((long long)inv);
    c = nv + c - 1 - last_zero;
    return -1;
  }
  int stop = -1;
  for (int i = 0; i < nv; ++i) {
    c = ((hits >> i) & 1ull) ? c + 1 : 0;
    if (c > lim) {
      stop = i;
      break;
    }
  }
  return stop;
}
__device__ __forceinline__ unsigned long long priv_key(uint32_t gen, uint32_t s, uint32_t slot, uint32_t h) {
  return ((unsigned long long)gen << 52) | ((unsigned long long)(s < 1023u ? s : 1023u) << 42) |
         ((unsigned long long)(slot >> 10) << 32) | (unsigned long long)h;
}
__device__ __forceinline__ bool priv_lookup(const unsigned long long* priv, uint32_t slot, uint32_t h, bool& hit) {
  const unsigned long long pe = priv[slot & (kPrivSlots - 1u)];
  if (pe != 0ull && (uint32_t)((pe >> 32) & 1023ull) == (slot >> 10)) {
    hit = (uint32_t)pe == h;
    return true;
  }
  return false;
}

__host__ __device__ inline uint32_t test_lds_words64(uint32_t steps_cap) { return kPrivSlots + 256u + steps_cap + 16u + (3u * kES + 1u) / 2u; }

struct SeedPhase {
  uint32_t g0, g1;
  uint32_t item_off;
  uint32_t item_cap;
};
constexpr uint32_t kSeedChainBits = 16, kSeedSubBits = 11;
constexpr uint32_t kSeedSegs = 4;
__global__ void __launch_bounds__(64 * kSeedSegs) k_seed_list(FrameParams F, const SeedPhase* __restrict__ phases,
                                                              const uint8_t* __restrict__ live, uint32_t* __restrict__ gens,
                                                              uint32_t* __restrict__ items, uint32_t* __restrict__ n_items, Counters* C) {
  __shared__ uint32_t s_cnt[kSeedSegs][64];
  const SeedPhase P = phases[blockIdx.y];
  const uint32_t n = F.n, n_chains = F.chains;
  const uint32_t n_gen = (n + n_chains - 1u) / n_chains;
  const uint32_t g0 = P.g0, g1 = P.g1 < n_gen ? P.g1 : n_gen;
  if (g0 >= g1 || blockIdx.x * 64u >= n_chains) return;
  const uint32_t lane = lane_id(), seg = threadIdx.x >> 6, chain = blockIdx.x * 64u + lane;
  const uint32_t len = g1 - g0, seg_len = (len + kSeedSegs - 1u) / kSeedSegs;
  const uint32_t a = g0 + seg * seg_len < g1 ? g0 + seg * seg_len : g1, b = a + seg_len < g1 ? a + seg_len : g1;
  auto flag = [&](uint32_t g) -> bool {
    const uint32_t p = g * n_chains + chain;
    const bool in = chain < n_chains && p < n;
    return live[in ? p : 0u] != 0 && in;
  };
  uint32_t mine = 0;
#pragma unroll 8
  for (uint32_t g = a; g < b; ++g) mine += flag(g) ? 1u : 0u;
  s_cnt[seg][lane] = mine;
  __syncthreads();
  uint32_t rank = 0, total = 0;
  for (uint32_t s = 0; s < kSeedSegs; ++s) {
    const uint32_t v = s_cnt[s][lane];
    rank += s < seg ? v : 0u;
    total += v;
  }
  uint32_t* __restrict__ mine_out = gens + (size_t)g0 * n_chains + (size_t)chain * len;
#pragma unroll 8
  for (uint32_t g = a; g < b; ++g)
    if (flag(g)) mine_out[rank++] = g;
  if (seg != 0) return;
  const uint32_t n_it = (total + kSubRun - 1u) / kSubRun;
  uint32_t x = n_it;
#pragma unroll
  for (int o = 1; o < 64; o <<= 1) {
    const uint32_t y = __shfl_up(x, o);
    if (lane >= (uint32_t)o) x += y;
  }
  const uint32_t wave_total = __shfl(x, 63);
  uint32_t base = 0;
  if (lane == 0 && wave_total) base = atomicAdd(&n_items[blockIdx.y], wave_total);
  base = __shfl(base, 0) + x - n_it;
  for (uint32_t s = 0; s < n_it; ++s) {
    const uint32_t left = total - s * kSubRun;
    if (base + s < P.item_cap) items[P.item_off + base + s] = chain | (s << kSeedChainBits) | (((left < kSubRun ? left : kSubRun) - 1u) << (kSeedChainBits + kSeedSubBits));
    else atomicOr(&C->err, kErrIndex);
  }
}
typedef __attribute__((address_space(1))) const uint32_t seed_global_u32;

template <bool OVERLAP>
__global__ void __launch_bounds__(kTestThreads) k_test(BatchView V, uint32_t g0, uint32_t g1, uint32_t phase, uint32_t item_off, uint32_t item_cap,
                                                       uint32_t steps_cap) {
  const SlotView& sv = V.s[blockIdx.y];
  const RayDesc* __restrict__ rays = sv.rays;
  uint32_t* __restrict__ cnt = sv.cnt;
  const Counters* C = sv.C;
  const FrameParams F = *sv.F;
  obs_global_u64* observed = (obs_global_u64*)(unsigned long long*)F.observed;
  const uint32_t n_chains = F.chains;
  const uint32_t phase_pos0 = g0 * n_chains;
  bool my_save = false;
  auto snapshot_look = [&](const ulonglong2 e, uint32_t h, bool& save) -> bool {
    unsigned long long content = e.x;
    const bool current = (uint32_t)(e.x >> 54) == F.obs_tag && ((uint32_t)(e.x >> 32) & 0x3fffffu) > phase_pos0;
    if (current) content = e.y;
    save = !current && e.x != 0ull && e.x != e.y;
    return obs_match(content, h, F.obs_tag_lo, F.obs_tag);
  };
  auto snapshot_save = [&](const ulonglong2 e, uint32_t slot) {
    obs_atomic_max(&observed[2u * slot + 1u], e.x);
    my_save = true;
  };
  auto snapshot_decide = [&](const ulonglong2 e, uint32_t slot, uint32_t h) -> bool {
    bool save;
    const bool hit = snapshot_look(e, h, save);
    if (save) snapshot_save(e, slot);
    return hit;
  };
  auto snapshot_hit = [&](uint32_t slot, uint32_t h) -> bool { return snapshot_decide(obs_load2(observed, slot), slot, h); };
  extern __shared__ unsigned long long s_test[];
  const uint32_t lane = lane_id(), wave = threadIdx.x >> 6;
  unsigned long long* priv = s_test + (size_t)wave * test_lds_words64(steps_cap);
  unsigned long long* keys = priv + kPrivSlots;
  unsigned long long* lkeys = keys + 256;
  uint32_t* rinfo = (uint32_t*)(lkeys + steps_cap);
  float* escr = (float*)(rinfo + 32);
  const uint32_t frame_err = __hip_atomic_load(&C->err, __ATOMIC_RELAXED, __HIP_MEMORY_SCOPE_AGENT);
  const uint32_t w = blockIdx.x * (blockDim.x >> 6) + wave;
  uint32_t n_items = ((seed_global_u32*)sv.seed_n)[phase];
  const uint32_t item = ((seed_global_u32*)sv.seed_items)[item_off + (w < item_cap ? w : item_cap - 1u)];
  if (n_items > item_cap) n_items = item_cap;
  if (w >= n_items) return;
  const uint32_t chain = item & ((1u << kSeedChainBits) - 1u), sub = (item >> kSeedChainBits) & ((1u << kSeedSubBits) - 1u);
  const uint32_t n_mine = (item >> (kSeedChainBits + kSeedSubBits)) + 1u;
  {
    const uint32_t n_gen = (F.n + n_chains - 1u) / n_chains;
    if (g1 > n_gen) g1 = n_gen;
  }
  uint32_t my_gen = ~0u;
  if (lane < n_mine) my_gen = ((seed_global_u32*)sv.seed_gen)[g0 * n_chains + chain * (g1 - g0) + sub * kSubRun + lane];
  if (__ballot(my_gen != ~0u) == 0ull || (frame_err & (kErrLabel | kErrIndex))) return;
  const int lim = F.max_collisions;
#ifdef KS_STATS
  const unsigned long long t_begin = __builtin_readcyclecounter();
  uint32_t st_long = 0, st_rounds = 0;
#endif

  Dda dda{};
  int my_steps = -1;
  {
    const uint64_t p = (uint64_t)my_gen * n_chains + chain;
    const bool is_live = my_gen != ~0u;
    if (is_live) {
      const RayDesc d = rays[ray_index(F, (uint32_t)p)];
      dda.setup(F.T.t, {d.px, d.py, d.pz}, ((d.info >> 10) & 1u) != 0, F.carving != 0, F.max_ray, F.voxel_size_inv, F.trunc,
                false);
      my_steps = dda.steps;
    }
    for (int s = 0; s < 16; ++s) {
      if (s <= my_steps) {
        const uint32_t h = index_hash(dda.cx, dda.cy, dda.cz);
        const uint32_t slot = (uint32_t)(((uint64_t)h + F.observed_offset) & kSetMask);
        keys[lane * 16 + s] = ((unsigned long long)slot << 32) | h;
      }
      dda.advance(s < my_steps);
    }
    if (lane < 16) rinfo[lane] = (uint32_t)my_steps;
  }
  const uint32_t live_mask = (uint32_t)(__ballot(my_steps >= 0) & 0xffffull);
  if (live_mask == 0u) return;
  {
    const uint32_t grp = lane >> 4, l = lane & 15u;
    bool hit[4];
    unsigned long long kk[4];
    ulonglong2 ee[4];
#pragma unroll
    for (int b = 0; b < 4; ++b) {
      const uint32_t r = (uint32_t)b * 4u + grp;
      const bool on = ((live_mask >> r) & 1u) && (int)l <= (int)rinfo[r];
      kk[b] = on ? keys[r * 16 + l] : ~0ull;
      ee[b] = on ? obs_load2(observed, (uint32_t)(kk[b] >> 32)) : make_ulonglong2(0ull, 0ull);
    }
    for (uint32_t i = lane; i < kPrivSlots; i += 64) priv[i] = 0ull;
    KS_WAIT_LOADS();
    bool sv4[4];
#pragma unroll
    for (int b = 0; b < 4; ++b) {
      sv4[b] = false;
      hit[b] = kk[b] != ~0ull && snapshot_look(ee[b], (uint32_t)kk[b], sv4[b]);
    }
#pragma unroll
    for (int b = 0; b < 4; ++b)
      if (kk[b] != ~0ull && sv4[b]) snapshot_save(ee[b], (uint32_t)(kk[b] >> 32));
#pragma unroll
    for (int b = 0; b < 4; ++b) {
      const unsigned long long m = __ballot(hit[b]);
// ... 482 lines not shown
```

### kimera_semantics_amd/csrc/ks_radix_sort.h

```cpp
#pragma once
#include <hip/hip_runtime.h>
#include <stdint.h>
#include <algorithm>
#include <stdlib.h>

#include "ks_owned.h"

namespace ksrs {

constexpr int kMaxPasses = 8;
constexpr int kMaxBins = 2048;
constexpr size_t kHistBlocks = 2048;
constexpr uint32_t kFlagLocal = 1u << 30, kFlagPrefix = 2u << 30, kCountMask = (1u << 30) - 1u;

template <int RB, typename K>
__device__ __forceinline__ uint32_t digit_of(K key, int shift) {
  return (uint32_t)(key >> shift) & (uint32_t)((1 << RB) - 1);
}

template <int RB>
__device__ __forceinline__ unsigned long long match_digit(uint32_t d, unsigned long long active) {
  unsigned long long peers = active;
#pragma unroll
  for (int b = 0; b < RB; ++b) {
    const bool bit = (d >> b) & 1u;
    const unsigned long long bal = __ballot(bit);
    peers &= bit ? bal : ~bal;
  }
  return peers;
}

template <typename K, int RB>
__device__ __forceinline__ void rs_hist_body(const K* __restrict__ keys, uint32_t n, int passes, int begin_bit,
                                             uint32_t* __restrict__ hist, uint32_t* __restrict__ zero_ptr,
                                             uint32_t zero_words, const unsigned long long* __restrict__ n_dev, uint32_t* s_hist) {
  constexpr int kBins = 1 << RB;
  const uint32_t tid = threadIdx.x, lane = tid & 63u;
  if (n_dev) n = (uint32_t)(*n_dev < (unsigned long long)n ? *n_dev : (unsigned long long)n);
  for (uint32_t i = blockIdx.x * 256u + tid; i < zero_words / 4u; i += gridDim.x * 256u)
    ((uint4*)zero_ptr)[i] = make_uint4(0u, 0u, 0u, 0u);
  for (int i = tid; i < passes * kBins; i += 256) s_hist[i] = 0;
  __syncthreads();
  const uint32_t n_slices = (n + 2047u) / 2048u;
  for (uint32_t slice = blockIdx.x; slice < n_slices; slice += gridDim.x) {
    const uint32_t base = slice * 2048u;
#pragma unroll
    for (int i = 0; i < 8; ++i) {
      const uint32_t idx = base + i * 256 + tid;
      const bool valid = idx < n;
      const K key = valid ? keys[idx] : (K)0;
      const unsigned long long active = __ballot(valid);
      for (int p = 0; p < passes; ++p) {
        const uint32_t d = digit_of<RB>(key, begin_bit + p * RB);
        const uint32_t d0 = (uint32_t)__builtin_amdgcn_readfirstlane((int)d);
        if (__ballot(valid && d != d0) == 0ull) {
          if (active && lane == (uint32_t)(__ffsll((long long)active) - 1))
            atomicAdd(&s_hist[p * kBins + d0], (uint32_t)__popcll(active));
        } else {
          const uint32_t dp = __shfl_up(d, 1);
          const unsigned long long lead = __ballot(valid && (lane == 0u || d != dp));
          if (valid && ((lead >> lane) & 1ull)) {
            const unsigned long long rest = (lane < 63u) ? (lead >> (lane + 1u)) : 0ull;
            const uint32_t stop = rest ? lane + (uint32_t)__ffsll((long long)rest) : 64u;
            const unsigned long long in_run = (stop < 64u ? ((1ull << stop) - 1ull) : ~0ull) & ~((1ull << lane) - 1ull);
            atomicAdd(&s_hist[p * kBins + d], (uint32_t)__popcll(in_run & active));
          }
        }
      }
    }
  }
  __syncthreads();
  for (int i = tid; i < passes * kBins; i += 256) {
    const uint32_t c = s_hist[i];
    if (c) atomicAdd(&hist[(i / kBins) * kMaxBins + (i % kBins)], c);
  }
}
template <typename K, int RB>
__global__ void __launch_bounds__(256) k_rs_hist(const K* __restrict__ keys, uint32_t n, int passes, int begin_bit,
                                                 uint32_t* __restrict__ hist, uint32_t* __restrict__ zero_ptr,
                                                 uint32_t zero_words, const unsigned long long* __restrict__ n_dev = nullptr) {
  extern __shared__ uint32_t s_hist[];
  rs_hist_body<K, RB>(keys, n, passes, begin_bit, hist, zero_ptr, zero_words, n_dev, s_hist);
}
constexpr int kRsBatch = 8;
template <typename K>
struct DevBatch {
  K* keys_a[kRsBatch];
  K* keys_b[kRsBatch];
  uint32_t* vals_a[kRsBatch];
  uint32_t* vals_b[kRsBatch];
  const unsigned long long* n_dev[kRsBatch];
  uint32_t* ws[kRsBatch];
};
template <typename K, int RB>
__global__ void __launch_bounds__(256) k_rs_hist_b(DevBatch<K> B, uint32_t cap, int passes, int begin_bit) {
  extern __shared__ uint32_t s_hist[];
  rs_hist_body<K, RB>(B.keys_a[blockIdx.y], cap, passes, begin_bit, B.ws[blockIdx.y], nullptr, 0u, B.n_dev[blockIdx.y], s_hist);
}

template <typename K, bool HAS_VALUES, int THREADS, int ITEMS, int RB, bool REORDER = false>
__device__ __forceinline__ void rs_pass_body(const K* __restrict__ keys_in, K* __restrict__ keys_out,
                                             const uint32_t* __restrict__ vals_in,
                                             uint32_t* __restrict__ vals_out, uint32_t n, int shift,
                                             const uint32_t* __restrict__ bin_hist,
                                             uint32_t* __restrict__ status, uint32_t* __restrict__ ticket,
                                             const unsigned long long* __restrict__ n_dev) {
  constexpr int kBins = 1 << RB;
  constexpr int kChunks = kBins / 64;
  constexpr int kWaves = THREADS / 64;
  constexpr int kTile = THREADS * ITEMS;
  if (n_dev) n = (uint32_t)(*n_dev < (unsigned long long)n ? *n_dev : (unsigned long long)n);
  __shared__ uint32_t s_cnt[kWaves][kBins];
  __shared__ uint32_t s_off[kBins];
  __shared__ uint32_t s_chunk[kChunks];
  __shared__ uint32_t s_tile;
  __shared__ K s_keys[REORDER ? kTile : 1];
  __shared__ uint32_t s_loc[REORDER ? kBins : 1];
  static_assert(!REORDER || (!HAS_VALUES && kBins <= THREADS), "reorder variant: keys only");
  const uint32_t tid = threadIdx.x, lane = tid & 63u, wave = tid >> 6;
  if (tid == 0) s_tile = ticket ? atomicAdd(ticket, 1u) : blockIdx.x;
  for (int i = tid; i < kWaves * kBins; i += THREADS) (&s_cnt[0][0])[i] = 0;
  __syncthreads();
  const uint32_t tile = s_tile;
  if (n_dev && (unsigned long long)tile * kTile >= (unsigned long long)n) return;
  const uint32_t wbase = tile * kTile + wave * (ITEMS * 64);

  K key[ITEMS];
  uint32_t rd[ITEMS];
#pragma unroll
  for (int i = 0; i < ITEMS; ++i) {
    const uint32_t idx = wbase + i * 64 + lane;
    key[i] = (idx < n) ? keys_in[idx] : (K)0;
  }
#pragma unroll
  for (int i = 0; i < ITEMS; ++i) {
    const uint32_t idx = wbase + i * 64 + lane;
    const bool valid = idx < n;
    const uint32_t d = digit_of<RB>(key[i], shift);
    const unsigned long long peers = match_digit<RB>(d, __ballot(valid));
    const uint32_t prev = s_cnt[wave][d];
    rd[i] = (prev + (uint32_t)__popcll(peers & ((1ull << lane) - 1ull))) | (d << 20);
    __builtin_amdgcn_wave_barrier();
    if (valid && (peers & ((1ull << lane) - 1ull)) == 0ull) s_cnt[wave][d] = prev + (uint32_t)__popcll(peers);
    __builtin_amdgcn_wave_barrier();
  }
  __syncthreads();

  for (int d = tid; d < kBins; d += THREADS) {
    uint32_t total = 0;
#pragma unroll
    for (int w = 0; w < kWaves; ++w) {
      const uint32_t c = s_cnt[w][d];
      s_cnt[w][d] = total;
      total += c;
    }
    if (REORDER) s_loc[d] = total;
    uint32_t* st = status + d;
    uint32_t prefix = 0;
    __hip_atomic_store(st + (size_t)tile * kBins, total | kFlagLocal, __ATOMIC_RELAXED, __HIP_MEMORY_SCOPE_AGENT);
    constexpr int kWindow = 8;
    int t = (int)tile - 1;
    bool done = false;
    while (!done) {
      uint32_t s[kWindow];
#pragma unroll
      for (int j = 0; j < kWindow; ++j)
        s[j] = (t - j >= 0) ? __hip_atomic_load(st + (size_t)(t - j) * kBins, __ATOMIC_RELAXED, __HIP_MEMORY_SCOPE_AGENT)
                            : kFlagPrefix;
      int consumed = 0;
#pragma unroll
      for (int j = 0; j < kWindow; ++j) {
        if (done || consumed != j) continue;
        const uint32_t flag = s[j] >> 30;
        if (flag == 0u) continue;
        prefix += s[j] & kCountMask;
        ++consumed;
        if (flag == 2u) done = true;
      }
      t -= consumed;
    }
    __hip_atomic_store(st + (size_t)tile * kBins, (prefix + total) | kFlagPrefix, __ATOMIC_RELAXED,
                       __HIP_MEMORY_SCOPE_AGENT);
    s_off[d] = prefix;
  }
  __syncthreads();
  for (int c = wave; c < kChunks; c += kWaves) {
    const uint32_t hv = bin_hist[c * 64 + lane];
    uint32_t x = hv;
#pragma unroll
    for (int o = 1; o < 64; o <<= 1) {
      const uint32_t y = __shfl_up(x, o);
      if (lane >= (uint32_t)o) x += y;
    }
    if (lane == 63) s_chunk[c] = x;
    s_off[c * 64 + lane] += x - hv;
  }
  __syncthreads();
  for (int d = tid; d < kBins; d += THREADS) {
    uint32_t add = 0;
    for (int cc = 0; cc < d / 64; ++cc) add += s_chunk[cc];
    s_off[d] += add;
  }
  __syncthreads();

  if (REORDER) {
    __shared__ uint32_t s_lchunk[kChunks];
    for (int c = wave; c < kChunks; c += kWaves) {
      const uint32_t tv = s_loc[c * 64 + lane];
      uint32_t x = tv;
#pragma unroll
      for (int o = 1; o < 64; o <<= 1) {
        const uint32_t y = __shfl_up(x, o);
        if (lane >= (uint32_t)o) x += y;
      }
      if (lane == 63) s_lchunk[c] = x;
      s_loc[c * 64 + lane] = x - tv;
    }
    __syncthreads();
    for (int d = tid; d < kBins; d += THREADS) {
      uint32_t add = 0;
      for (int cc = 0; cc < d / 64; ++cc) add += s_lchunk[cc];
      s_loc[d] += add;
    }
    __syncthreads();
#pragma unroll
    for (int i = 0; i < ITEMS; ++i) {
      const uint32_t idx = wbase + i * 64 + lane;
      if (idx < n) {
        const uint32_t d = rd[i] >> 20;
        s_keys[s_loc[d] + s_cnt[wave][d] + (rd[i] & 0xfffffu)] = key[i];
      }
    }
    __syncthreads();
    const uint32_t t0 = tile * (uint32_t)kTile;
    const uint32_t count = (n - t0 < (uint32_t)kTile) ? n - t0 : (uint32_t)kTile;
    for (uint32_t j = tid; j < count; j += THREADS) {
      const K k = s_keys[j];
      const uint32_t d = digit_of<RB>(k, shift);
      keys_out[s_off[d] + (j - s_loc[d])] = k;
    }
    return;
  }
#pragma unroll
  for (int i = 0; i < ITEMS; ++i) {
    const uint32_t idx = wbase + i * 64 + lane;
    if (idx < n) {
      const uint32_t d = rd[i] >> 20;
      const uint32_t pos = s_off[d] + s_cnt[wave][d] + (rd[i] & 0xfffffu);
      keys_out[pos] = key[i];
      if (HAS_VALUES) vals_out[pos] = vals_in[idx];
    }
  }
}

template <typename K, bool HAS_VALUES, int THREADS, int ITEMS, int RB, bool REORDER = false>
__global__ void __launch_bounds__(THREADS) k_rs_pass(const K* __restrict__ keys_in, K* __restrict__ keys_out,
                                                     const uint32_t* __restrict__ vals_in,
                                                     uint32_t* __restrict__ vals_out, uint32_t n, int shift,
                                                     const uint32_t* __restrict__ bin_hist,
                                                     uint32_t* __restrict__ status, uint32_t* __restrict__ ticket,
                                                     const unsigned long long* __restrict__ n_dev = nullptr) {
  rs_pass_body<K, HAS_VALUES, THREADS, ITEMS, RB, REORDER>(keys_in, keys_out, vals_in, vals_out, n, shift, bin_hist, status, ticket, n_dev);
}
template <typename K, int THREADS, int ITEMS, int RB>
__global__ void __launch_bounds__(THREADS) k_rs_pass_b(DevBatch<K> B, uint32_t cap, int begin_bit, int p, uint32_t tiles) {
  const uint32_t y = blockIdx.y;
  uint32_t* ws = B.ws[y];
  const bool odd = (p & 1) != 0;
  rs_pass_body<K, true, THREADS, ITEMS, RB, false>(odd ? B.keys_b[y] : B.keys_a[y], odd ? B.keys_a[y] : B.keys_b[y], odd ? B.vals_b[y] : B.vals_a[y],
                                                   odd ? B.vals_a[y] : B.vals_b[y], cap, begin_bit + p * RB, ws + (size_t)p * kMaxBins,
                                                   ws + ((size_t)kMaxPasses * kMaxBins + kMaxPasses) + (size_t)p * tiles * (1 << RB),
                                                   ws + (size_t)kMaxPasses * kMaxBins + p, B.n_dev[y]);
}

struct Workspace {
  DevBuf<uint32_t> d_ws;
  size_t words = 0;
  int cur = 0;
  size_t dirty[2] = {0, 0};
};
constexpr size_t kHeadWords = (size_t)kMaxPasses * kMaxBins + kMaxPasses;

inline hipError_t ensure(Workspace& w, size_t words, hipStream_t stream) {
  if (words <= w.words) return hipSuccess;
  w.words = 0;
  const size_t cap = ((words + words / 4) + 3) & ~(size_t)3;
  hipError_t e = w.d_ws.try_alloc(2 * cap);
  if (e != hipSuccess) return e;
  e = hipMemsetAsync(w.d_ws, 0, 2 * cap * sizeof(uint32_t), stream);
  if (e != hipSuccess) return e;
  w.words = cap;
  w.cur = 0;
  w.dirty[0] = w.dirty[1] = 0;
  return hipSuccess;
}

template <typename K, bool HAS_VALUES, int THREADS, int ITEMS, int RB, bool REORDER = false>
inline void launch_passes(Workspace& w, K*& kin, K*& kout, uint32_t*& vin, uint32_t*& vout, size_t n, int passes,
                          uint32_t tiles, unsigned begin_bit, hipStream_t stream) {
  constexpr int kBins = 1 << RB;
  uint32_t* base = w.d_ws + (size_t)w.cur * w.words;
  uint32_t* hist = base;
  uint32_t* tickets = base + (size_t)kMaxPasses * kMaxBins;
  uint32_t* status = base + kHeadWords;
  for (int p = 0; p < passes; ++p) {
    hipLaunchKernelGGL((k_rs_pass<K, HAS_VALUES, THREADS, ITEMS, RB, REORDER>), dim3(tiles), dim3(THREADS), 0, stream, kin, kout,
                       vin, vout, (uint32_t)n, (int)begin_bit + p * RB, hist + (size_t)p * kMaxBins,
                       status + (size_t)p * tiles * kBins, tickets + p);
    K* tk = kin; kin = kout; kout = tk;
    uint32_t* tv = vin; vin = vout; vout = tv;
  }
}

template <typename K, bool HAS_VALUES, int RB>
inline hipError_t sort_rb(Workspace& w, K* keys_a, K* keys_b, uint32_t* vals_a, uint32_t* vals_b, size_t n,
                          unsigned begin_bit, unsigned end_bit, hipStream_t stream, K** keys_result,
                          uint32_t** vals_result) {
  constexpr int kBins = 1 << RB;
  const int passes = (int)((end_bit - begin_bit + RB - 1) / RB);
  const bool reorder = !HAS_VALUES && n > (1u << 20);
  const int tile = (n <= (1u << 20)) ? 2048 : (reorder || n <= (1u << 24)) ? 8192 : 16384;
  const uint32_t tiles = (uint32_t)((n + tile - 1) / tile);
  const size_t words = kHeadWords + (size_t)passes * tiles * kBins;
  hipError_t e = ensure(w, words, stream);
  if (e != hipSuccess) return e;
  const int h = w.cur ^ 1;
  hipLaunchKernelGGL((k_rs_hist<K, RB>), dim3((uint32_t)std::min<size_t>((n + 2047) / 2048, kHistBlocks)), dim3(256),
                     (size_t)passes * kBins * sizeof(uint32_t), stream, keys_a, (uint32_t)n, passes, (int)begin_bit,
                     w.d_ws + (size_t)h * w.words, w.d_ws + (size_t)(h ^ 1) * w.words,
                     (uint32_t)((w.dirty[h ^ 1] + 3) & ~(size_t)3));
  w.dirty[h ^ 1] = 0;
  w.dirty[h] = words;
  w.cur = h;
  K* kin = keys_a;
  K* kout = keys_b;
  uint32_t* vin = vals_a;
  uint32_t* vout = vals_b;
  if (tile == 2048) launch_passes<K, HAS_VALUES, 256, 8, RB>(w, kin, kout, vin, vout, n, passes, tiles, begin_bit, stream);
  else if (tile == 8192 && reorder) {
    if constexpr (!HAS_VALUES) launch_passes<K, false, 512, 16, RB, true>(w, kin, kout, vin, vout, n, passes, tiles, begin_bit, stream);
  } else if (tile == 8192) launch_passes<K, HAS_VALUES, 512, 16, RB>(w, kin, kout, vin, vout, n, passes, tiles, begin_bit, stream);
  else launch_passes<K, HAS_VALUES, 512, 32, RB>(w, kin, kout, vin, vout, n, passes, tiles, begin_bit, stream);
  *keys_result = kin;
  if (vals_result) *vals_result = vin;
  return hipGetLastError();
}

inline size_t dev_tile(size_t cap) { return cap <= (1u << 20) ? 2048 : cap <= (1u << 24) ? 8192 : 16384; }
inline size_t ws_words_dev(size_t cap, int passes) { return kHeadWords + (size_t)passes * ((cap + dev_tile(cap) - 1) / dev_tile(cap)) * 256; }
template <typename K>
inline hipError_t sort_dev(uint32_t* ws, size_t ws_words, K* keys_a, K* keys_b, uint32_t* vals_a, uint32_t* vals_b,
                           const unsigned long long* n_dev, size_t cap, unsigned begin_bit, unsigned end_bit, hipStream_t stream,
                           K** keys_result, uint32_t** vals_result) {
  constexpr int RB = 8;
  constexpr int kBins = 1 << RB;
  const int passes = (int)((end_bit - begin_bit + RB - 1) / RB);
  const size_t tile = dev_tile(cap);
  const uint32_t tiles = (uint32_t)((cap + tile - 1) / tile);
  if (kHeadWords + (size_t)passes * tiles * kBins > ws_words) return hipErrorInvalidValue;
  hipError_t e = hipMemsetAsync(ws, 0, (kHeadWords + (size_t)passes * tiles * kBins) * sizeof(uint32_t), stream);
  if (e != hipSuccess) return e;
  uint32_t* hist = ws;
  uint32_t* tickets = ws + (size_t)kMaxPasses * kMaxBins;
  uint32_t* status = ws + kHeadWords;
  hipLaunchKernelGGL((k_rs_hist<K, RB>), dim3((uint32_t)std::min<size_t>((cap + 2047) / 2048, kHistBlocks)), dim3(256),
                     (size_t)passes * kBins * sizeof(uint32_t), stream, (const K*)keys_a, (uint32_t)cap, passes, (int)begin_bit, hist,
                     (uint32_t*)nullptr, 0u, n_dev);
  K* kin = keys_a;
  K* kout = keys_b;
  uint32_t* vin = vals_a;
  uint32_t* vout = vals_b;
  for (int p = 0; p < passes; ++p) {
#define KS_RS_DEV_PASS(THREADS, ITEMS)                                                                                                 \
  hipLaunchKernelGGL((k_rs_pass<K, true, THREADS, ITEMS, RB>), dim3(tiles), dim3(THREADS), 0, stream, (const K*)kin, kout,             \
                     (const uint32_t*)vin, vout, (uint32_t)cap, (int)begin_bit + p * RB, (const uint32_t*)(hist + (size_t)p * kMaxBins), \
                     status + (size_t)p * tiles * kBins, tickets + p, n_dev)
    if (tile == 2048) KS_RS_DEV_PASS(256, 8);
    else if (tile == 8192) KS_RS_DEV_PASS(512, 16);
    else KS_RS_DEV_PASS(512, 32);
#undef KS_RS_DEV_PASS
    K* tk = kin; kin = kout; kout = tk;
    uint32_t* tv = vin; vin = vout; vout = tv;
  }
  *keys_result = kin;
  *vals_result = vin;
  return hipGetLastError();
}

template <typename K>
inline hipError_t sort_dev_batch(const DevBatch<K>& B, int nb, size_t ws_words, size_t cap, unsigned begin_bit, unsigned end_bit, hipStream_t stream) {
  constexpr int RB = 8;
  constexpr int kBins = 1 << RB;
  const int passes = (int)((end_bit - begin_bit + RB - 1) / RB);
  const size_t tile = dev_tile(cap);
  const uint32_t tiles = (uint32_t)((cap + tile - 1) / tile);
  if (kHeadWords + (size_t)passes * tiles * kBins > ws_words || nb < 1 || nb > kRsBatch) return hipErrorInvalidValue;
  for (int y = 0; y < nb; ++y) {
    hipError_t e = hipMemsetAsync(B.ws[y], 0, (kHeadWords + (size_t)passes * tiles * kBins) * sizeof(uint32_t), stream);
    if (e != hipSuccess) return e;
  }
  hipLaunchKernelGGL((k_rs_hist_b<K, RB>), dim3((uint32_t)std::min<size_t>((cap + 2047) / 2048, kHistBlocks), (uint32_t)nb), dim3(256),
                     (size_t)passes * kBins * sizeof(uint32_t), stream, B, (uint32_t)cap, passes, (int)begin_bit);
  for (int p = 0; p < passes; ++p) {
    if (tile == 2048) hipLaunchKernelGGL((k_rs_pass_b<K, 256, 8, RB>), dim3(tiles, (uint32_t)nb), dim3(256), 0, stream, B, (uint32_t)cap, (int)begin_bit, p, tiles);
    else if (tile == 8192) hipLaunchKernelGGL((k_rs_pass_b<K, 512, 16, RB>), dim3(tiles, (uint32_t)nb), dim3(512), 0, stream, B, (uint32_t)cap, (int)begin_bit, p, tiles);
    else hipLaunchKernelGGL((k_rs_pass_b<K, 512, 32, RB>), dim3(tiles, (uint32_t)nb), dim3(512), 0, stream, B, (uint32_t)cap, (int)begin_bit, p, tiles);
  }
  return hipGetLastError();
}

template <typename K, bool HAS_VALUES>
inline hipError_t sort(Workspace& w, K* keys_a, K* keys_b, uint32_t* vals_a, uint32_t* vals_b, size_t n,
                       unsigned end_bit, hipStream_t stream, K** keys_result, uint32_t** vals_result,
                       unsigned begin_bit = 0) {
  *keys_result = keys_a;
  if (vals_result) *vals_result = vals_a;
  if (end_bit > sizeof(K) * 8) end_bit = (unsigned)(sizeof(K) * 8);
  if (n == 0 || end_bit <= begin_bit) return hipSuccess;
  return sort_rb<K, HAS_VALUES, 8>(w, keys_a, keys_b, vals_a, vals_b, n, begin_bit, end_bit, stream, keys_result, vals_result);
}

}
```

Baseline: 1009 Mvoxel-updates/s.

## Batch stage-A point sorts and seed lists across frames in one launch

Splits fast-path stage A so each frame's points kernel writes into its own per-batch-position point set, and the key sorts for all frames in a batch run as one batched radix sort with host-known sizes. Seed list generation also becomes a single batched launch, and workspace memsets for contiguous batch slices are merged. The intent is to cut per-frame launch and memset overhead and expose more parallelism per sort. In exchange it allocates extra per-position point buffers and delays dedup until the batch is launched, which changes frame-level overlap.

```diff
diff --git a/include/ks_hip.h b/include/ks_hip.h
--- a/include/ks_hip.h
+++ b/include/ks_hip.h
@@ -179,6 +179,7 @@
                              int freespace_points, ks_round_stats* stats);
 
 int ks_debug_radix_sort(ks_ctx* ctx, void* keys, uint32_t* vals, size_t n, int key_bits, unsigned end_bit);
+int ks_debug_radix_sort_batch(ks_ctx* ctx, uint32_t* const* keys, uint32_t* const* vals, const size_t* n, int nb, unsigned end_bit);
 
 int ks_synchronize(ks_ctx* ctx);
 void* ks_stream(ks_ctx* ctx);
diff --git a/kimera_semantics_amd/binding.py b/kimera_semantics_amd/binding.py
--- a/kimera_semantics_amd/binding.py
+++ b/kimera_semantics_amd/binding.py
@@ -28,7 +28,7 @@
     "ks_default_config", "ks_create", "ks_destroy", "ks_last_error", "ks_set_color_to_label",
     "ks_integrate_points", "ks_integrate_points_device", "ks_integrate_depth", "ks_integrate_depth_device", "ks_num_blocks", "ks_get_block_indices",
     "ks_get_updated_block_indices", "ks_count_updated_voxels", "ks_download_updated_voxels", "ks_download_blocks", "ks_upload_blocks", "ks_host_alloc", "ks_host_free", "ks_get_tile_keys", "ks_export_tiles_device", "ks_merge_tiles_device", "ks_clear", "ks_clear_voxels", "ks_reset_tiles", "ks_tile_owner", "ks_reduce",
-    "ks_debug_radix_sort", "ks_synchronize", "ks_flush", "ks_stream",
+    "ks_debug_radix_sort", "ks_debug_radix_sort_batch", "ks_synchronize", "ks_flush", "ks_stream",
     "ks_profile_enable", "ks_profile_get", "ks_early_out_iterations", "ks_early_out_stats", "ks_pipeline_shape", "ks_stream_plan", "ks_seed_launch_shape", "ks_update_stats", "ks_integrate_round_exact",
     "ks_mesh_default_config", "ks_mesh_update", "ks_mesh_size", "ks_mesh_download", "ks_mesh_changed_blocks",
     "ks_esdf_default_config", "ks_esdf_update", "ks_esdf_download_blocks", "ks_esdf_query",
@@ -156,6 +156,7 @@
         L.ks_tile_owner.argtypes = [C.c_uint64, C.c_int]
         L.ks_reduce.argtypes = [vp, vp, C.c_int, C.c_int, C.POINTER(KsReduceStats)]
         L.ks_debug_radix_sort.argtypes = [vp, vp, vp, C.c_size_t, C.c_int, C.c_uint]
+        L.ks_debug_radix_sort_batch.argtypes = [vp, vp, vp, vp, C.c_int, C.c_uint]
         L.ks_synchronize.argtypes = [vp]
         L.ks_flush.argtypes = [vp, C.POINTER(KsFrameStats)]
         L.ks_stream.argtypes = [vp]
@@ -441,6 +442,17 @@
                                             bits if end_bit is None else end_bit))
         return keys, vals
 
+    def debug_radix_sort_batch(self, keys, vals, end_bit=32):
+        keys = [np.ascontiguousarray(k, dtype=np.uint32).copy() for k in keys]
+        vals = [np.ascontiguousarray(v, dtype=np.uint32).copy() for v in vals]
+        assert len(keys) == len(vals) and all(k.shape == v.shape for k, v in zip(keys, vals))
+        nb = len(keys)
+        kp = (C.c_void_p * nb)(*[k.ctypes.data for k in keys])
+        vp_ = (C.c_void_p * nb)(*[v.ctypes.data for v in vals])
+        ns = (C.c_size_t * nb)(*[k.shape[0] for k in keys])
+        self._chk(lib().ks_debug_radix_sort_batch(self._h, kp, vp_, ns, nb, end_bit))
+        return keys, vals
+
     def synchronize(self):
         self._chk(lib().ks_synchronize(self._h))
 
diff --git a/kimera_semantics_amd/csrc/ks_hip.hip b/kimera_semantics_amd/csrc/ks_hip.hip
--- a/kimera_semantics_amd/csrc/ks_hip.hip
+++ b/kimera_semantics_amd/csrc/ks_hip.hip
@@ -101,7 +101,7 @@
   DevBuf<uint32_t> d_eo_cnt_b, d_eo_ux, d_eo_dirty, d_eo_list[2], d_eo_chg, d_eo_consulted, d_eo_lp;
   DevBuf<unsigned long long> d_eo_bt;
   DevBuf<EoCtl> d_eo_ctl;
-  DevBuf<uint32_t> d_eo_sort_ws;
+  uint32_t* d_eo_sort_ws = nullptr;
   DevBuf<uint32_t> d_eo_hseq, d_eo_where;
   DevBuf<uint4> d_eo_rinfo, d_eo_ckpt;
   DevBuf<uint8_t> d_eo_hitb;
@@ -261,6 +261,10 @@
   uint32_t key_bits = 0;
   DevBuf<uint64_t> d_pkeys, d_pkeys2;
   DevBuf<uint32_t> d_pvals, d_pvals2;
+  struct PointSet {
+    DevBuf<uint32_t> d_hash, d_keys, d_keys_b, d_vals, d_vals_b;
+  } a_sets[kBatchMax - 1];
+  DevBuf<uint32_t> d_a_sort_ws;
   DevBuf<uint32_t> d_order;
   DevBuf<uint32_t> d_inv_order;
   DevBuf<uint32_t> d_okeys, d_okeys2, d_ovals;
@@ -289,6 +293,7 @@
   hipEvent_t eo_last_commit = nullptr;
   std::atomic<size_t> eo_want_marks{0}, eo_want_x{0};
   size_t eo_cap_marks = 0, eo_cap_x = 0;
+  DevBuf<uint32_t> d_eo_sort_ws_all;
   std::atomic<uint64_t> eo_fallbacks{0};
   uint64_t eo_fallbacks_seen = 0;
   std::atomic<int> eo_hopeless{0};
@@ -542,6 +547,13 @@
   return (size_t)std::ceil(1.7321 * max_len * (double)voxel_size_inv) + 8;
 }
 int ensure_exact_points(ks_ctx* c, size_t cap);
+constexpr int kStageASortPasses = ((int)kSetBits + 1 + 7) / 8;
+inline size_t stage_a_sort_words(size_t cap) {
+  size_t w = ksrs::ws_words_dev(cap, kStageASortPasses);
+  for (size_t edge : {(size_t)1 << 20, (size_t)1 << 24})
+    if (cap > edge) w = std::max(w, ksrs::ws_words_dev(edge, kStageASortPasses));
+  return w;
+}
 int ensure_points(ks_ctx* c, size_t n) {
   if (n <= c->cap_points) return KS_OK;
   const size_t cap = std::max<size_t>(c->cap_points ? n + n / 8 : n, 1024);
@@ -595,6 +607,15 @@
   if ((rc = c->d_pkeys2.alloc(c, cap))) return rc;
   if ((rc = c->d_pvals.alloc(c, cap))) return rc;
   if ((rc = c->d_pvals2.alloc(c, cap))) return rc;
+  if (c->cfg.method == KS_METHOD_FAST) {
+    for (int k = 1; k < c->batch; ++k) {
+      ks_ctx::PointSet& P = c->a_sets[k - 1];
+      if ((rc = P.d_hash.alloc(c, cap)) || (rc = P.d_keys.alloc(c, cap)) || (rc = P.d_keys_b.alloc(c, cap)) || (rc = P.d_vals.alloc(c, cap)) ||
+          (rc = P.d_vals_b.alloc(c, cap)))
+        return rc;
+    }
+    if ((rc = c->d_a_sort_ws.alloc(c, (size_t)c->batch * stage_a_sort_words(cap)))) return rc;
+  }
   if ((rc = c->d_order.alloc(c, cap))) return rc;
   if ((rc = c->d_inv_order.alloc(c, cap))) return rc;
   if ((rc = c->d_okeys.alloc(c, cap))) return rc;
@@ -885,7 +906,7 @@
         if ((rc = S.d_eo_keys[b].alloc(c, cap_marks))) return rc;
         if ((rc = S.d_eo_vals[b].alloc(c, cap_marks))) return rc;
       }
-      if ((rc = S.d_eo_sort_ws.alloc(c, ksrs::ws_words_dev(cap_marks, 3)))) return rc;
+      S.d_eo_sort_ws = nullptr;
       if ((rc = S.d_eo_hitb.alloc(c, cap_marks))) return rc;
       if ((rc = S.d_eo_hseq.alloc(c, cap_marks))) return rc;
       if ((rc = S.d_eo_where.alloc(c, cap_marks))) return rc;
@@ -894,6 +915,14 @@
       S.eo_cap_marks = cap_marks;
     }
     if ((rc = S.d_eo_xnode.reserve(c, 2 * cap_x, 2 * cap_x))) return rc;
+  }
+  const size_t ws_words = ksrs::ws_words_dev(c->slot[0].eo_cap_marks, 3);
+  bool carved = c->d_eo_sort_ws_all.size() >= (size_t)n_slots * ws_words;
+  for (int i = 0; i < n_slots; ++i) carved = carved && c->slot[i].d_eo_sort_ws != nullptr;
+  if (!carved) {
+    for (int i = 0; i < n_slots; ++i) c->slot[i].d_eo_sort_ws = nullptr;
+    if ((rc = c->d_eo_sort_ws_all.alloc(c, (size_t)n_slots * ws_words))) return rc;
+    for (int i = 0; i < n_slots; ++i) c->slot[i].d_eo_sort_ws = c->d_eo_sort_ws_all + (size_t)i * ws_words;
   }
   c->eo_cap_marks = cap_marks;
   c->eo_cap_x = cap_x;
@@ -989,7 +1018,7 @@
     hipLaunchKernelGGL(k_eo2_full, dim3(gn, nb), dim3(256), 0, st, Bt);
     hipLaunchKernelGGL(k_eo2_scan, dim3(nb4k, nb), dim3(1024), 0, st, Bt);
     hipLaunchKernelGGL(k_eo2_emit<8>, dim3((uint32_t)((n + 31) / 32), nb), dim3(256), lds, st, Bt);
-    HIPCHK(c, ksrs::sort_dev_batch<uint64_t>(Rs, (int)nb, S0.d_eo_sort_ws.size(), S0.eo_cap_marks, 44, 64, st));
+    HIPCHK(c, ksrs::sort_dev_batch<uint64_t>(Rs, (int)nb, ksrs::ws_words_dev(S0.eo_cap_marks, 3), S0.eo_cap_marks, 44, 64, st));
     hipLaunchKernelGGL(k_eo2_bits, dim3(gm, nb), dim3(256), 0, st, Bt, 0u);
     hipLaunchKernelGGL(k_eo2_where, dim3(gm, nb), dim3(256), 0, st, Bt);
     enqueue_sweeps(c, Bt, nb, c->eo_sweeps, st);
@@ -997,7 +1026,7 @@
   } else {
     hipLaunchKernelGGL(k_eo2_scan, dim3(nb4k, nb), dim3(1024), 0, st, Bt);
     hipLaunchKernelGGL(k_eo2_emit<64>, dim3((uint32_t)((n + 255) / 256), nb), dim3(256), lds, st, Bt);
-    HIPCHK(c, ksrs::sort_dev_batch<uint64_t>(Rs, (int)nb, S0.d_eo_sort_ws.size(), S0.eo_cap_marks, 44, 64, st));
+    HIPCHK(c, ksrs::sort_dev_batch<uint64_t>(Rs, (int)nb, ksrs::ws_words_dev(S0.eo_cap_marks, 3), S0.eo_cap_marks, 44, 64, st));
     hipLaunchKernelGGL(k_eo2_hits, dim3(gm, nb), dim3(256), 0, st, Bt);
     hipLaunchKernelGGL(k_eo2_stop0, dim3(gn, nb), dim3(256), 0, st, Bt);
     hipLaunchKernelGGL(k_eo2_bits, dim3(gm, nb), dim3(256), 0, st, Bt, 1u);
@@ -1113,12 +1142,16 @@
   }
 };
 
+int stage_a2_fast(ks_ctx* c, FrameSlot* const* slots, uint32_t nb);
 int launch_batch(ks_ctx* c) {
   if (c->batch_slots.empty()) return KS_OK;
   std::vector<FrameSlot*> slots;
   slots.swap(c->batch_slots);
   const uint32_t nb = (uint32_t)slots.size();
   FrameSlot& S0 = *slots[0];
+  if (c->cfg.method == KS_METHOD_FAST) {
+    if (int rc = stage_a2_fast(c, slots.data(), nb)) return rc;
+  }
   hipStream_t sm = c->batch > 1 ? c->stream_march_[(S0.frame_no / (uint64_t)c->batch) % (uint64_t)c->n_march] : march_stream(c, S0.frame_no);
   c->prof_march_stream = sm;
   if (sm != c->stream) HIPCHK(c, hipStreamWaitEvent(sm, slots[nb - 1]->a_done, 0));
@@ -1208,26 +1241,75 @@
   P.n_pairs = 0;
   S.prof_set = set;
 }
-int stage_a_fast(ks_ctx* c, FrameSlot& S, const float* d_xyz, const uint8_t* d_rgba, const uint8_t* d_labels, size_t n) {
-  const FrameParams& F = S.F;
+struct PointSetView {
+  uint32_t *hash, *keys, *keys_b, *vals, *vals_b;
+};
+inline PointSetView point_set(ks_ctx* c, uint32_t k) {
+  if (k == 0) return {c->d_hash, c->d_skeys32, c->d_skeys32b, c->d_pvals, c->d_pvals2};
+  const ks_ctx::PointSet& P = c->a_sets[k - 1];
+  return {P.d_hash, P.d_keys, P.d_keys_b, P.d_vals, P.d_vals_b};
+}
+int stage_a1_fast(ks_ctx* c, FrameSlot& S, const float* d_xyz, const uint8_t* d_rgba, const uint8_t* d_labels, size_t n) {
+  const uint32_t k = (uint32_t)c->batch_slots.size();
+  if (k >= (uint32_t)std::max(c->batch, 1) || (k > 0 && !c->a_sets[k - 1].d_hash)) {
+    c->err = "stage A: no point set for this position of the batch";
+    return KS_ERR_INVALID_ARG;
+  }
+  const PointSetView P = point_set(c, k);
+  hipLaunchKernelGGL(k_points_fast, dim3((uint32_t)((n + 1023) / 1024)), dim3(1024), 0, c->stream, S.F, d_xyz, d_rgba, d_labels, c->d_color_lut,
+                     S.d_rays, P.hash, P.keys, P.vals, S.d_cnt, S.d_live, S.d_counters);
+  stage_mark(c, S.prof_set, 1);
+  return KS_OK;
+}
+int stage_a2_fast(ks_ctx* c, FrameSlot* const* slots, uint32_t nb) {
   hipStream_t st = c->stream;
-  const uint32_t nb1k = (uint32_t)((n + 1023) / 1024);
-  hipLaunchKernelGGL(k_points_fast, dim3(nb1k), dim3(1024), 0, st, F, d_xyz, d_rgba, d_labels, c->d_color_lut,
-                     S.d_rays, c->d_hash, c->d_skeys32, c->d_pvals, S.d_cnt, S.d_live, S.d_counters);
-  stage_mark(c, S.prof_set, 1);
-  uint32_t *sk = nullptr, *sv = nullptr;
-  if (int rc = sort_pairs(c, c->d_skeys32.get(), c->d_skeys32b.get(), c->d_pvals.get(), c->d_pvals2.get(), n, kSetBits + 1, &sk, &sv)) return rc;
-  stage_mark(c, S.prof_set, 2);
-  hipLaunchKernelGGL(k_dedup, dim3(nb1k), dim3(1024), 0, st, F, sk, sv, c->d_hash, c->d_start_set, S.d_ray_list, S.d_rays, S.d_cnt, S.d_live, S.d_counters);
-  if (c->uses_early_out && n > 0) {
-    const uint32_t n_gen = (uint32_t)((n + F.chains - 1) / F.chains);
-    uint32_t n_ph = 0;
-    while (n_ph < c->seed_phases.size() && c->seed_phases[n_ph].g0 < n_gen) ++n_ph;
-    HIPCHK(c, hipMemsetAsync(S.d_seed_n, 0, c->seed_phases.size() * sizeof(uint32_t), st));
-    hipLaunchKernelGGL(k_seed_list, dim3((F.chains + 63u) / 64u, n_ph), dim3(64 * kSeedSegs), 0, st, F, (const SeedPhase*)c->d_seed_phases,
-                       (const uint8_t*)S.d_live, S.d_seed_gen, S.d_seed_items, S.d_seed_n, S.d_counters);
-  }
-  hipLaunchKernelGGL(k_dedup_commit, dim3(nb1k), dim3(1024), 0, st, F, sk, sv, c->d_hash, c->d_start_set, S.d_counters);
+  ksrs::DevBatch<uint32_t> Rs{};
+  size_t n_max = 0;
+  for (uint32_t k = 0; k < nb; ++k) n_max = std::max(n_max, slots[k]->n);
+  const size_t ws_words = ksrs::ws_words_dev(n_max, kStageASortPasses);
+  if ((size_t)nb * ws_words > c->d_a_sort_ws.size()) {
+    c->err = "stage A: the batch's sorts do not fit their workspace";
+    return KS_ERR_INVALID_ARG;
+  }
+  for (uint32_t k = 0; k < nb; ++k) {
+    const PointSetView P = point_set(c, k);
+    Rs.keys_a[k] = P.keys;
+    Rs.keys_b[k] = P.keys_b;
+    Rs.vals_a[k] = P.vals;
+    Rs.vals_b[k] = P.vals_b;
+    Rs.n[k] = (uint32_t)slots[k]->n;
+    Rs.ws[k] = c->d_a_sort_ws + (size_t)k * ws_words;
+  }
+  HIPCHK(c, ksrs::sort_dev_batch<uint32_t>(Rs, (int)nb, ws_words, n_max, 0, kSetBits + 1, st));
+  if (nb == 1) stage_mark(c, slots[0]->prof_set, 2);
+  for (uint32_t k = 0; k < nb; ++k) {
+    FrameSlot& S = *slots[k];
+    const PointSetView P = point_set(c, k);
+    const uint32_t nb1k = (uint32_t)((S.n + 1023) / 1024);
+    hipLaunchKernelGGL(k_dedup, dim3(nb1k), dim3(1024), 0, st, S.F, (const uint32_t*)P.keys_b, (const uint32_t*)P.vals_b, (const uint32_t*)P.hash, c->d_start_set,
+                       S.d_ray_list, S.d_rays, S.d_cnt, S.d_live, S.d_counters);
+    hipLaunchKernelGGL(k_dedup_commit, dim3(nb1k), dim3(1024), 0, st, S.F, (const uint32_t*)P.keys_b, (const uint32_t*)P.vals_b, (const uint32_t*)P.hash,
+                       c->d_start_set, S.d_counters);
+  }
+  if (c->uses_early_out) {
+    SeedBatch SB{};
+    uint32_t gx = 0, gy = 0;
+    for (uint32_t k = 0; k < nb; ++k) {
+      FrameSlot& S = *slots[k];
+      const FrameParams& F = S.F;
+      const uint32_t n_gen = (uint32_t)((S.n + F.chains - 1) / F.chains);
+      uint32_t n_ph = 0;
+      while (n_ph < c->seed_phases.size() && c->seed_phases[n_ph].g0 < n_gen) ++n_ph;
+      SB.f[k] = SeedFrame{F.n, F.chains, n_ph, S.d_live, S.d_seed_gen, S.d_seed_items, S.d_seed_n, S.d_counters};
+      gx = std::max(gx, (F.chains + 63u) / 64u);
+      gy = std::max(gy, n_ph);
+    }
+    hipLaunchKernelGGL(k_seed_clear, dim3(nb), dim3(64), 0, st, SB, (uint32_t)c->seed_phases.size());
+    if (gx && gy)
+      hipLaunchKernelGGL(k_seed_list, dim3(gx, gy, nb), dim3(64 * kSeedSegs), 0, st, SB, (const SeedPhase*)c->d_seed_phases);
+  }
+  if (nb == 1) stage_mark(c, slots[0]->prof_set, 3);
+  if (c->stream_march_[0] != st) HIPCHK(c, hipEventRecord(slots[nb - 1]->a_done, st));
   return KS_OK;
 }
 void enqueue_bundle_order(ks_ctx* c, hipStream_t st, size_t n, const uint64_t* sk, const uint32_t* sv) {
@@ -1320,10 +1402,12 @@
     hipLaunchKernelGGL(k_invert, dim3(nb), dim3(256), 0, st, (uint32_t)n, order_ptr, c->d_inv_order);
     F.order = order_ptr;
   }
-  if ((rc = c->cfg.method == KS_METHOD_FAST ? stage_a_fast(c, S, d_xyz, d_rgba, d_labels, n) : stage_a_merged(c, S, d_xyz, d_rgba, d_labels, n, order_ptr)))
-    return rc;
-  stage_mark(c, S.prof_set, 3);
-  if (c->stream_march_[0] != st) HIPCHK(c, hipEventRecord(S.a_done, st));
+  const bool fast = c->cfg.method == KS_METHOD_FAST;
+  if ((rc = fast ? stage_a1_fast(c, S, d_xyz, d_rgba, d_labels, n) : stage_a_merged(c, S, d_xyz, d_rgba, d_labels, n, order_ptr))) return rc;
+  if (!fast) {
+    stage_mark(c, S.prof_set, 3);
+    if (c->stream_march_[0] != st) HIPCHK(c, hipEventRecord(S.a_done, st));
+  }
   S.steps_max = steps_max;
   S.b_launched = false;
   S.pending = true;
@@ -3025,6 +3109,44 @@
   HIPCHK(c, hipStreamSynchronize(c->stream));
   HIPCHK(c, hipMemcpy(keys, kres, n * kb, hipMemcpyDeviceToHost));
   if (vals) HIPCHK(c, hipMemcpy(vals, vres, n * 4, hipMemcpyDeviceToHost));
+  return KS_OK;
+}
+
+int ks_debug_radix_sort_batch(ks_ctx* c, uint32_t* const* keys, uint32_t* const* vals, const size_t* n, int nb, unsigned end_bit) {
+  if (!c || !keys || !vals || !n || nb < 1 || nb > ksrs::kRsBatch || end_bit < 1 || end_bit > 32) return KS_ERR_INVALID_ARG;
+  size_t n_max = 0;
+  for (int k = 0; k < nb; ++k) {
+    if (n[k] && (!keys[k] || !vals[k])) return KS_ERR_INVALID_ARG;
+    if (n[k] > ((size_t)1 << 30)) return KS_ERR_INVALID_ARG;
+    n_max = std::max(n_max, n[k]);
+  }
+  if (n_max == 0) return KS_OK;
+  const int passes = (int)((end_bit + 7) / 8);
+  const size_t ws_words = ksrs::ws_words_dev(n_max, passes);
+  DevBuf<uint32_t> ka[ksrs::kRsBatch], kb[ksrs::kRsBatch], va[ksrs::kRsBatch], vb[ksrs::kRsBatch], ws;
+  ksrs::DevBatch<uint32_t> Rs{};
+  int rc;
+  if ((rc = ws.alloc(c, (size_t)nb * ws_words))) return rc;
+  for (int k = 0; k < nb; ++k) {
+    if ((rc = ka[k].alloc(c, n[k])) || (rc = kb[k].alloc(c, n[k])) || (rc = va[k].alloc(c, n[k])) || (rc = vb[k].alloc(c, n[k]))) return rc;
+    if (n[k]) {
+      HIPCHK(c, hipMemcpy(ka[k], keys[k], n[k] * 4, hipMemcpyHostToDevice));
+      HIPCHK(c, hipMemcpy(va[k], vals[k], n[k] * 4, hipMemcpyHostToDevice));
+    }
+    Rs.keys_a[k] = ka[k];
+    Rs.keys_b[k] = kb[k];
+    Rs.vals_a[k] = va[k];
+    Rs.vals_b[k] = vb[k];
+    Rs.n[k] = (uint32_t)n[k];
+    Rs.ws[k] = ws + (size_t)k * ws_words;
+  }
+  HIPCHK(c, ksrs::sort_dev_batch<uint32_t>(Rs, nb, ws_words, n_max, 0, end_bit, c->stream));
+  HIPCHK(c, hipStreamSynchronize(c->stream));
+  for (int k = 0; k < nb; ++k) {
+    if (!n[k]) continue;
+    HIPCHK(c, hipMemcpy(keys[k], (passes & 1) ? kb[k] : ka[k], n[k] * 4, hipMemcpyDeviceToHost));
+    HIPCHK(c, hipMemcpy(vals[k], (passes & 1) ? vb[k] : va[k], n[k] * 4, hipMemcpyDeviceToHost));
+  }
   return KS_OK;
 }
 
diff --git a/kimera_semantics_amd/csrc/ks_k_march.h b/kimera_semantics_amd/csrc/ks_k_march.h
--- a/kimera_semantics_amd/csrc/ks_k_march.h
+++ b/kimera_semantics_amd/csrc/ks_k_march.h
@@ -214,12 +214,32 @@
 };
 constexpr uint32_t kSeedChainBits = 16, kSeedSubBits = 11;
 constexpr uint32_t kSeedSegs = 4;
-__global__ void __launch_bounds__(64 * kSeedSegs) k_seed_list(FrameParams F, const SeedPhase* __restrict__ phases,
-                                                              const uint8_t* __restrict__ live, uint32_t* __restrict__ gens,
-                                                              uint32_t* __restrict__ items, uint32_t* __restrict__ n_items, Counters* C) {
+struct SeedFrame {
+  uint32_t n, chains;
+  uint32_t n_phases;
+  const uint8_t* live;
+  uint32_t* gens;
+  uint32_t* items;
+  uint32_t* n_items;
+  Counters* C;
+};
+struct SeedBatch {
+  SeedFrame f[kBatchMax];
+};
+__global__ void __launch_bounds__(64) k_seed_clear(SeedBatch B, uint32_t n_phases) {
+  for (uint32_t i = threadIdx.x; i < n_phases; i += 64u) B.f[blockIdx.x].n_items[i] = 0u;
+}
+__global__ void __launch_bounds__(64 * kSeedSegs) k_seed_list(SeedBatch B, const SeedPhase* __restrict__ phases) {
   __shared__ uint32_t s_cnt[kSeedSegs][64];
+  const SeedFrame& Fr = B.f[blockIdx.z];
+  const uint32_t n = Fr.n, n_chains = Fr.chains;
+  if (blockIdx.y >= Fr.n_phases || blockIdx.x * 64u >= n_chains) return;
+  const uint8_t* __restrict__ live = Fr.live;
+  uint32_t* __restrict__ gens = Fr.gens;
+  uint32_t* __restrict__ items = Fr.items;
+  uint32_t* __restrict__ n_items = Fr.n_items;
+  Counters* C = Fr.C;
   const SeedPhase P = phases[blockIdx.y];
-  const uint32_t n = F.n, n_chains = F.chains;
   const uint32_t n_gen = (n + n_chains - 1u) / n_chains;
   const uint32_t g0 = P.g0, g1 = P.g1 < n_gen ? P.g1 : n_gen;
   if (g0 >= g1 || blockIdx.x * 64u >= n_chains) return;
diff --git a/kimera_semantics_amd/csrc/ks_radix_sort.h b/kimera_semantics_amd/csrc/ks_radix_sort.h
--- a/kimera_semantics_amd/csrc/ks_radix_sort.h
+++ b/kimera_semantics_amd/csrc/ks_radix_sort.h
@@ -91,14 +91,16 @@
   uint32_t* vals_b[kRsBatch];
   const unsigned long long* n_dev[kRsBatch];
   uint32_t* ws[kRsBatch];
+  uint32_t n[kRsBatch];
 };
 template <typename K, int RB>
 __global__ void __launch_bounds__(256) k_rs_hist_b(DevBatch<K> B, uint32_t cap, int passes, int begin_bit) {
   extern __shared__ uint32_t s_hist[];
-  rs_hist_body<K, RB>(B.keys_a[blockIdx.y], cap, passes, begin_bit, B.ws[blockIdx.y], nullptr, 0u, B.n_dev[blockIdx.y], s_hist);
-}
-
-template <typename K, bool HAS_VALUES, int THREADS, int ITEMS, int RB, bool REORDER = false>
+  const unsigned long long* n_dev = B.n_dev[blockIdx.y];
+  rs_hist_body<K, RB>(B.keys_a[blockIdx.y], n_dev ? cap : B.n[blockIdx.y], passes, begin_bit, B.ws[blockIdx.y], nullptr, 0u, n_dev, s_hist);
+}
+
+template <typename K, bool HAS_VALUES, int THREADS, int ITEMS, int RB, bool REORDER = false, bool PAST_END = false>
 __device__ __forceinline__ void rs_pass_body(const K* __restrict__ keys_in, K* __restrict__ keys_out,
                                              const uint32_t* __restrict__ vals_in,
                                              uint32_t* __restrict__ vals_out, uint32_t n, int shift,
@@ -122,7 +124,7 @@
   for (int i = tid; i < kWaves * kBins; i += THREADS) (&s_cnt[0][0])[i] = 0;
   __syncthreads();
   const uint32_t tile = s_tile;
-  if (n_dev && (unsigned long long)tile * kTile >= (unsigned long long)n) return;
+  if ((PAST_END || n_dev) && (unsigned long long)tile * kTile >= (unsigned long long)n) return;
   const uint32_t wbase = tile * kTile + wave * (ITEMS * 64);
 
   K key[ITEMS];
@@ -267,10 +269,11 @@
   const uint32_t y = blockIdx.y;
   uint32_t* ws = B.ws[y];
   const bool odd = (p & 1) != 0;
-  rs_pass_body<K, true, THREADS, ITEMS, RB, false>(odd ? B.keys_b[y] : B.keys_a[y], odd ? B.keys_a[y] : B.keys_b[y], odd ? B.vals_b[y] : B.vals_a[y],
-                                                   odd ? B.vals_a[y] : B.vals_b[y], cap, begin_bit + p * RB, ws + (size_t)p * kMaxBins,
+  const unsigned long long* n_dev = B.n_dev[y];
+  rs_pass_body<K, true, THREADS, ITEMS, RB, false, true>(odd ? B.keys_b[y] : B.keys_a[y], odd ? B.keys_a[y] : B.keys_b[y], odd ? B.vals_b[y] : B.vals_a[y],
+                                                   odd ? B.vals_a[y] : B.vals_b[y], n_dev ? cap : B.n[y], begin_bit + p * RB, ws + (size_t)p * kMaxBins,
                                                    ws + ((size_t)kMaxPasses * kMaxBins + kMaxPasses) + (size_t)p * tiles * (1 << RB),
-                                                   ws + (size_t)kMaxPasses * kMaxBins + p, B.n_dev[y]);
+                                                   ws + (size_t)kMaxPasses * kMaxBins + p, n_dev);
 }
 
 struct Workspace {
@@ -394,10 +397,14 @@
   const int passes = (int)((end_bit - begin_bit + RB - 1) / RB);
   const size_t tile = dev_tile(cap);
   const uint32_t tiles = (uint32_t)((cap + tile - 1) / tile);
-  if (kHeadWords + (size_t)passes * tiles * kBins > ws_words || nb < 1 || nb > kRsBatch) return hipErrorInvalidValue;
-  for (int y = 0; y < nb; ++y) {
-    hipError_t e = hipMemsetAsync(B.ws[y], 0, (kHeadWords + (size_t)passes * tiles * kBins) * sizeof(uint32_t), stream);
+  const size_t used = kHeadWords + (size_t)passes * tiles * kBins;
+  if (used > ws_words || nb < 1 || nb > kRsBatch || cap == 0) return hipErrorInvalidValue;
+  for (int y = 0; y < nb;) {
+    int z = y + 1;
+    while (z < nb && B.ws[z] == B.ws[y] + (size_t)(z - y) * used) ++z;
+    hipError_t e = hipMemsetAsync(B.ws[y], 0, (size_t)(z - y) * used * sizeof(uint32_t), stream);
     if (e != hipSuccess) return e;
+    y = z;
   }
   hipLaunchKernelGGL((k_rs_hist_b<K, RB>), dim3((uint32_t)std::min<size_t>((cap + 2047) / 2048, kHistBlocks), (uint32_t)nb), dim3(256),
                      (size_t)passes * kBins * sizeof(uint32_t), stream, B, (uint32_t)cap, passes, (int)begin_bit);
```

Result: no change. 1006 Mvoxel-updates/s (-0.3%).
